# Tejasvanvekar/Sparse-optimal-control-of-Viscous-Chan-hilliard-via-Gradient-descent--1D-2D

Measured on AMD Instinct MI355X. Metric: PGD iterations/sec (fwd Newton + adjoint + prox), 2D 512^2 grid, higher is better.
Workload: dtype f64; 1 GPU; 2D 512x512, 1000 time steps, batch 8 trajectories per GPU (8 total), seeds 42+i, targets build_targets 1/1, u0 = 0; grid=512, batch_per_gpu=8, contexts_per_gpu=2, parallelism=batch-shard x1, collective=cabi-rccl

## Files before the change

sparse-optimal-control-of-viscous-chan-hilliard-via-gradient-descent--1d-2d_amd/csrc/vch_engine2d.hip:

```cpp
#include "vch_common.h"
#include "vch_kernels2d.h"
#include "vch_gemm.h"
#include "vch_fft.h"
#include <algorithm>
#include <atomic>
#include <chrono>
#include <cmath>

thread_local char g_vch_err[512] = "";

extern "C" const char *vch_last_error(void) { return g_vch_err; }
extern "C" int vch_abi_version(void) { return 3; }
extern "C" int vch_device_count(void) {
    int n = 0;
    if (hipGetDeviceCount(&n) != hipSuccess) return -1;
    return n;
}

constexpr int J_RING = 64;

struct GuessPolicy {
    static constexpr int PROBE_EVERY = 8;
    int order, probe, since, next_dir;
    bool climbing;
    double r_base;
    void reset() { order = 1; probe = 0; since = 0; next_dir = 1; climbing = true; r_base = 1e300; }
    int choose(int avail, int cap) const { return std::max(0, std::min(std::min(order + probe, cap), avail)); }
    void report(double r, int used, int cap) {
        if (used < 1) return;
        if (climbing) {
            if (r > 0.7) {
                order = std::max(1, used - 1);
                r_base = 1e300;
                if (used > 1) climbing = false;
                return;
            }
            if (r_base < 1e299 && r > 0.5 * r_base) {
                order = std::max(1, used - 1);
                climbing = false;
                return;
            }
            r_base = r;
            order = used;
            if (used >= cap) climbing = false;
            else order = used + 1;
            return;
        }
        if (probe == 0) {
            r_base = r;
            if (r > 0.7 && order > 1) { --order; since = 0; return; }
            if (++since >= PROBE_EVERY) {
                since = 0;
                probe = next_dir;
                next_dir = -next_dir;
                if (order + probe < 1 || order + probe > cap) probe = 0;
            }
            return;
        }
        if (probe > 0 ? r < 0.5 * r_base : r <= r_base) order = used;
        probe = 0;
    }
};

struct vch2d_ctx {
    vch2d_params prm;
    int B, Mmax, device;
    Geom G;
    Phys P;
    double hx, hy;
    hipStream_t stream;
    hipEvent_t ev0, ev1;
    dim3 grid;
    int nblk;
    long slot_stride;
    double *phi_s, *mu_s, *Rphi_s, *rhs_s, *D_s;
    double *w, *wnew, *mu0, *cphi, *cmu, *x, *r, *dmu, *t1, *t2;
    double *cg_p[2], *cg_v, *cg_q;
    double *cg_z2;
    double *xf;
    int cg_last;
    bool cheb_on;
    int spec_form[4];
    bool debug_guess;
    bool adj_guess_off, adj_safe;
    long redo_iters;
    bool fused_on;
    int fused_mode;
    unsigned *fin_counter;
    int cheb_enq, spec_chn[4], cheb_margin, cheb_max;
    double pgd_adj_tol;
    double eta1_factor;
    double cg_scale_ratio;
    double *dprev[GUESS_RING], *x0g;
    bool guess_on;
    int guess_wr, guess_step;
    int guess_max;
    std::vector<GuessPolicy> pol1, pol2;
    std::vector<int> used1, used2, run2;
    GuessPolicy pol1_all, pol2_all;
    int run2_all;
    GuessArgs gtab1, gtab2;
    unsigned gmask1, gmask2;
    double *dprev2[GUESS_RING];
    bool guess2_on;
    double *gpart2;
    double *gpart3;
    double *gpart;
    int gnblk;
    double *tmp[6];
    double *wts_mass, *W_cost;
    double *part;
    double *part_mass;
    bool post_fold;
    bool post_pending;
    double *post_hist;
    TrajState *st, *st_host;
    TrajState *st_pub;
    unsigned long long *seq_pub, seq_next;
    bool look_spin;
    int *frozen_dev;
    double *hist_dev, *hist_host;
    double *Q1f, *Q2f, *Q1s, *Q2s, *mf, *ms;
    bool use_fft;
    int cols_c;
    FftAxis fax, sax;
    FftAxis fax_h, sax_h;
    double2 *tw_fh = nullptr, *tw_sh = nullptr;
    bool half_f = false, half_s = false;
    double2 *tw_f, *tw_s;
    double *phi_hist, *u_hist, *u_trial, *phi_trial, *phiQ, *r_hist, *p_hist, *q_hist;
    double *phiT, *phi0;
    double *cost_part, *cost_lvl;
    double *cost_lvl_host;
    double *alpha_dev;
    int M_res;
    int u_rows_res;
    bool pgd_ready;
    bool ramp;
    double rampT;
    std::vector<double> t_hist, dt, xg, yg, tfrac;
    double *tfrac_dev;
    std::vector<vch_opt_params> opts;
    double *opt_tab, *seam_tab;
    std::vector<double> tab_host;
    bool pgd_r_valid;
    unsigned long long *kkt_dev;
    std::vector<double> pgd_cost, pgd_alpha_prev, pgd_J;
    std::vector<int> pgd_plateau, pgd_done, pgd_k;
    std::vector<std::vector<double>> pgd_cost_hist;
    std::vector<double> pgd_denQ2, pgd_denT2, pgd_trk, pgd_trm;
    double pgd_rms;
    int pgd_err_n;
    double *J_dev;
    double *J_ring_dev, *J_ring_host;
    std::atomic<long> pgd_iter_total;
    long tot_launch, tot_sync;
    bool prof_on;
    std::vector<hipEvent_t> prof_ev;
    std::vector<int> prof_cls;
    size_t prof_used;
    int lin_maxit;
    double lin_tol;
    double lin_eta;
    bool spec;
    int spec_slots, spec_cgb[4];
    long n_launch, n_sync;
};

enum { PC_SCHUR_P = 0, PC_GEMM = 1, PC_RESIDUAL = 2, PC_ADJ_Q = 3, PC_CG_UPDATE = 4, PC_ADJ_RHS = 5, PC_COST = 6,
       PC_PROX = 7, PC_DCT_R0 = 8, PC_DCT_C = 9, PC_DCT_R3 = 10, PC_SCHUR_P1 = 11, PC_CG_ROWS = 12, PC_CG_ROWS1 = 13,
       PC_NOOP = 14, PC_GUESS = 15, PC_ADJ_GUESS = 16, PC_CHEB_ROWS = 17, PC_CHEB_ROWS0 = 18, PC_RESIDUAL0 = 19,
       PC_NCLS = 20 };

__global__ void k_noop() {}

static bool launch_begin(vch2d_ctx *c, int cls) {
    const bool rec = cls >= 0 && c->prof_on && c->prof_used + 2 <= c->prof_ev.size();
    if (rec) hipEventRecord(c->prof_ev[c->prof_used], c->stream);
    return rec;
}
static void launch_end(vch2d_ctx *c, int cls, bool rec) {
    c->n_launch++;
    if (rec) {
        hipEventRecord(c->prof_ev[c->prof_used + 1], c->stream);
        c->prof_cls.push_back(cls);
        c->prof_used += 2;
    }
}
#define LAUNCHC(cls, kern, grid, block, ...) LAUNCH_LDS(cls, kern, grid, block, 0, __VA_ARGS__)

static int dalloc(double **p, size_t n, hipStream_t s) {
    *p = nullptr;
    HIPCHK(hipMalloc((void **)p, n * sizeof(double)));
    HIPCHK(hipMemsetAsync(*p, 0, n * sizeof(double), s));
    return 0;
}

static int h2d(vch2d_ctx *c, double *dev, const double *host, long nplanes) {
    HIPCHK(hipMemcpy2DAsync(dev, (size_t)c->G.pitch * 8, host, (size_t)c->G.nf * 8, (size_t)c->G.nf * 8,
                            (size_t)c->G.ns * nplanes, hipMemcpyHostToDevice, c->stream));
    return 0;
}
static int d2h(vch2d_ctx *c, double *host, const double *dev, long nplanes) {
    HIPCHK(hipMemcpy2DAsync(host, (size_t)c->G.nf * 8, dev, (size_t)c->G.pitch * 8, (size_t)c->G.nf * 8,
                            (size_t)c->G.ns * nplanes, hipMemcpyDeviceToHost, c->stream));
    HIPCHK(hipStreamSynchronize(c->stream));
    return 0;
}
static int h2d_hist(vch2d_ctx *c, double *dev, const double *host, int rows) {
    const long hs = (long)(c->Mmax + 1) * c->G.plane;
    for (int b = 0; b < c->B; ++b)
        VCHCHK(h2d(c, dev + b * hs, host + (long)b * rows * c->G.nf * c->G.ns, rows));
    return 0;
}
static int d2h_hist(vch2d_ctx *c, double *host, const double *dev, int rows) {
    const long hs = (long)(c->Mmax + 1) * c->G.plane;
    for (int b = 0; b < c->B; ++b) {
        HIPCHK(hipMemcpy2DAsync(host + (long)b * rows * c->G.nf * c->G.ns, (size_t)c->G.nf * 8, dev + b * hs,
                                (size_t)c->G.pitch * 8, (size_t)c->G.nf * 8, (size_t)c->G.ns * rows,
                                hipMemcpyDeviceToHost, c->stream));
    }
    HIPCHK(hipStreamSynchronize(c->stream));
    return 0;
}
static int ensure_hist(vch2d_ctx *c, double **p) {
    if (*p) return 0;
    size_t n = (size_t)c->B * (c->Mmax + 1) * c->G.plane;
    hipError_t e = hipMalloc((void **)p, n * sizeof(double));
    if (e != hipSuccess) {
        *p = nullptr;
        return vch_fail(VCH_ERR_NOMEM, "hipMalloc of a %.2f GB history failed: %s", n * 8e-9, hipGetErrorString(e));
    }
    HIPCHK(hipMemsetAsync(*p, 0, n * sizeof(double), c->stream));
    return 0;
}
static inline long hist_stride(const vch2d_ctx *c) { return (long)(c->Mmax + 1) * c->G.plane; }

__global__ void k_publish_state(const unsigned *__restrict__ st, int nwords, unsigned *__restrict__ dst,
                                unsigned long long *seq, unsigned long long val) {
    for (int i = threadIdx.x; i < nwords; i += blockDim.x) dst[i] = st[i];
    __threadfence_system();
    __syncthreads();
    if (threadIdx.x == 0) __hip_atomic_store(seq, val, __ATOMIC_RELEASE, __HIP_MEMORY_SCOPE_SYSTEM);
}

static int sync_state(vch2d_ctx *c, bool full = true) {
    c->n_sync++;
    if (full || !c->look_spin) {
        HIPCHK(hipMemcpyAsync(c->st_host, c->st, sizeof(TrajState) * c->B, hipMemcpyDeviceToHost, c->stream));
        HIPCHK(hipStreamSynchronize(c->stream));
        return 0;
    }
    const unsigned long long want = ++c->seq_next;
    static_assert(sizeof(TrajState) % 4 == 0, "TrajState is copied in 32-bit words");
    hipLaunchKernelGGL(k_publish_state, dim3(1), dim3(256), 0, c->stream, (const unsigned *)c->st,
                       (int)(sizeof(TrajState) / 4 * c->B), (unsigned *)c->st_pub, c->seq_pub, want);
    HIPCHK(hipGetLastError());
    const auto t0 = std::chrono::steady_clock::now();
    for (unsigned spins = 1; __atomic_load_n(c->seq_pub, __ATOMIC_ACQUIRE) != want; ++spins) {
        __builtin_ia32_pause();
        if ((spins & 0x3fff) == 0) {
            const hipError_t q = hipStreamQuery(c->stream);
            if (q != hipSuccess && q != hipErrorNotReady) return vch_fail(VCH_ERR_HIP, "sync_state: %s", hipGetErrorString(q));
            if (q == hipSuccess && __atomic_load_n(c->seq_pub, __ATOMIC_ACQUIRE) != want)
                return vch_fail(VCH_ERR_STATE, "sync_state: stream drained but the state was not published");
            if (std::chrono::steady_clock::now() - t0 > std::chrono::seconds(120))
                return vch_fail(VCH_ERR_STATE, "sync_state: no state from the device after 120 s");
        }
    }
    memcpy(c->st_host, c->st_pub, sizeof(TrajState) * c->B);
    return 0;
}

static void dct_tables(int N, double h, std::vector<double> &Q1, std::vector<double> &Q2, std::vector<double> &m) {
    const int n = N + 1;
    Q1.assign((size_t)n * n, 0.0);
    Q2.assign((size_t)n * n, 0.0);
    m.assign(n, 0.0);
    const long double pi = 3.14159265358979323846264338327950288L;
    const long double sc = sqrtl(2.0L / N), is2 = 1.0L / sqrtl(2.0L);
    for (int j = 0; j < n; ++j) {
        long double sj = (j == 0 || j == N) ? is2 : 1.0L;
        for (int k = 0; k < n; ++k) {
            long double sk = (k == 0 || k == N) ? is2 : 1.0L;
            long long jk = ((long long)j * k) % (2LL * N);
            long double cv = cosl(pi * (long double)jk / (long double)N);
            Q1[(size_t)j * n + k] = (double)(sc * sj * sj * sk * cv);
            Q2[(size_t)j * n + k] = (double)(sc * sj * cv);
        }
        m[j] = (double)((2.0L - 2.0L * cosl(pi * j / (long double)N)) / ((long double)h * h));
    }
}

extern "C" vch2d_ctx *vch2d_create(const vch2d_params *p, int batch, int max_steps, int device) {
    if (!p || p->Nx < 2 || p->Ny < 2 || batch < 1 || max_steps < 1 || !(p->Lx > 0) || !(p->Ly > 0)) {
        vch_fail(VCH_ERR_ARG, "vch2d_create: bad arguments (Nx,Ny >= 2, batch >= 1, max_steps >= 1)");
        return nullptr;
    }
    if (hipSetDevice(device) != hipSuccess) {
        (void)hipGetLastError();
        vch_fail(VCH_ERR_HIP, "hipSetDevice(%d) failed", device);
        return nullptr;
    }
    vch2d_ctx *c = new vch2d_ctx();
    c->prm = *p;
    c->B = batch;
    c->Mmax = max_steps;
    c->device = device;
    c->hx = p->Lx / p->Nx;
    c->hy = p->Ly / p->Ny;
    Geom &G = c->G;
    G.nf = p->Nx + 1;
    G.ns = p->Ny + 1;
    G.pitch = (G.nf + 7) / 8 * 8;
    G.plane = (long)G.ns * G.pitch;
    G.tiles_f = (G.nf + TX - 1) / TX;
    G.tiles_s = (G.ns + TY - 1) / TY;
    G.ax = 1.0 / (c->hx * c->hx);
    G.ay = 1.0 / (c->hy * c->hy);
    c->P = Phys{p->tau, p->gamma, p->c1, p->c2, p->kappa, p->Lx * p->Ly};
    c->grid = dim3(G.tiles_f, G.tiles_s, batch);
    c->nblk = G.tiles_f * G.tiles_s;
    c->slot_stride = (long)batch * G.plane;
    c->M_res = -1;
    c->u_rows_res = 0;
    c->pgd_ready = false;
    c->prof_on = false;
    c->prof_used = 0;
    c->lin_maxit = 4000;
    c->lin_tol = 1e-15;
    if (const char *e = getenv("VCH_LIN_TOL")) c->lin_tol = atof(e);
    c->lin_eta = 0.05 * NEWTON_TOL;
    if (const char *e = getenv("VCH_LIN_ETA")) c->lin_eta = atof(e);
    c->cols_c = 1024;
    if (const char *e = getenv("VCH_COLS_C")) c->cols_c = atoi(e);
    c->spec = getenv("VCH_NO_SPEC") == nullptr;
    c->spec_slots = 2;
    for (int &n : c->spec_cgb) n = 12;
    c->cheb_on = !(getenv("VCH_CHEB") && atoi(getenv("VCH_CHEB")) == 0);
    for (int &f : c->spec_form) f = 3;
    c->debug_guess = getenv("VCH_DEBUG_GUESS") != nullptr;
    c->adj_guess_off = c->adj_safe = false;
    c->redo_iters = 0;
    c->cheb_enq = -1;
    c->fused_mode = getenv("VCH_FUSED") ? atoi(getenv("VCH_FUSED")) : 2;
    c->fused_on = c->fused_mode != 0;
    c->post_fold = true;
    if (const char *e = getenv("VCH_POST_FOLD")) c->post_fold = atoi(e) != 0;
    c->post_pending = false;
    c->post_hist = nullptr;
    c->fin_counter = nullptr;
    for (int &n : c->spec_chn) n = 2;
    c->cheb_margin = 1;
    if (const char *e = getenv("VCH_CHEB_MARGIN")) c->cheb_margin = std::max(0, atoi(e));
    c->cheb_max = 6;
    if (const char *e = getenv("VCH_CHEB_MAX")) c->cheb_max = std::max(0, atoi(e));
    c->pgd_adj_tol = 1e-12;
    if (const char *e = getenv("VCH_ADJ_TOL")) c->pgd_adj_tol = atof(e);
    c->eta1_factor = 1e-2;
    if (const char *e = getenv("VCH_ETA1")) c->eta1_factor = atof(e);
    c->cg_scale_ratio = 4.0;
    if (const char *e = getenv("VCH_CG_SCALE")) c->cg_scale_ratio = atof(e);
    c->n_launch = c->n_sync = 0;
    auto fail = [&](const char *what) {
        vch_fail(VCH_ERR_HIP, "vch2d_create: %s failed: %s", what, hipGetErrorString(hipGetLastError()));
        return (vch2d_ctx *)nullptr;
    };
    if (hipStreamCreate(&c->stream) != hipSuccess) return fail("hipStreamCreate");
    hipEventCreate(&c->ev0);
    hipEventCreate(&c->ev1);
    const size_t bp = (size_t)batch * G.plane;
    double **two[] = {&c->phi_s, &c->mu_s, &c->Rphi_s, &c->rhs_s, &c->D_s};
    for (auto q : two)
        if (dalloc(q, 2 * bp, c->stream)) return fail("hipMalloc");
    double **one[] = {&c->w, &c->wnew, &c->mu0, &c->cphi, &c->cmu, &c->x, &c->r, &c->dmu, &c->t1, &c->t2,
                      &c->cg_p[0], &c->cg_p[1], &c->cg_v, &c->cg_q, &c->cg_z2, &c->xf, &c->dprev[0], &c->dprev[1], &c->dprev[2], &c->dprev[3], &c->dprev[4], &c->dprev[5], &c->dprev[6], &c->dprev[7], &c->dprev2[0], &c->dprev2[1], &c->dprev2[2], &c->dprev2[3], &c->dprev2[4], &c->dprev2[5], &c->dprev2[6], &c->dprev2[7], &c->x0g, &c->tmp[0], &c->tmp[1], &c->tmp[2], &c->tmp[3], &c->tmp[4], &c->tmp[5], &c->phiT, &c->phi0};
    for (auto q : one)
        if (dalloc(q, bp, c->stream)) return fail("hipMalloc");
    if (dalloc(&c->wts_mass, G.plane, c->stream) || dalloc(&c->W_cost, G.plane, c->stream)) return fail("hipMalloc");
    if (dalloc(&c->part, (size_t)batch * c->nblk * NPART, c->stream)) return fail("hipMalloc");
    if (dalloc(&c->part_mass, (size_t)batch * c->nblk * NPART, c->stream)) return fail("hipMalloc");
    c->gnblk = ((G.nf + GN - 1) / GN) * ((G.ns + GM - 1) / GM);
    if (dalloc(&c->gpart, 2 * (size_t)batch * (c->gnblk + G.ns), c->stream)) return fail("hipMalloc");
    c->gpart2 = c->gpart + (size_t)batch * (c->gnblk + G.ns);
    if (dalloc(&c->gpart3, 4 * (size_t)batch * (c->gnblk + G.ns), c->stream)) return fail("hipMalloc");
    if (dalloc(&c->hist_dev, (size_t)batch * HIST_CAP, c->stream)) return fail("hipMalloc");
    if (dalloc(&c->alpha_dev, batch, c->stream) || dalloc(&c->J_dev, 5 * (size_t)batch, c->stream)) return fail("hipMalloc");
    if (dalloc(&c->opt_tab, (size_t)OPT_STRIDE * batch, c->stream) || dalloc(&c->seam_tab, (size_t)OPT_STRIDE * batch, c->stream))
        return fail("hipMalloc");
    if (hipMalloc((void **)&c->kkt_dev, sizeof(unsigned long long) * 3 * batch * (max_steps + 2)) != hipSuccess)
        return fail("hipMalloc");
    c->pgd_r_valid = false;
    if (dalloc(&c->J_ring_dev, (size_t)J_RING * 5 * batch, c->stream)) return fail("hipMalloc");
    if (hipHostMalloc((void **)&c->J_ring_host, sizeof(double) * J_RING * 5 * batch) != hipSuccess) return fail("hipHostMalloc");
    c->pgd_iter_total = 0;
    c->tot_launch = c->tot_sync = 0;
    if (hipMalloc((void **)&c->st, sizeof(TrajState) * batch) != hipSuccess) return fail("hipMalloc");
    hipMemsetAsync(c->st, 0, sizeof(TrajState) * batch, c->stream);
    if (hipMalloc((void **)&c->frozen_dev, sizeof(int) * batch) != hipSuccess) return fail("hipMalloc");
    if (hipMalloc((void **)&c->fin_counter, sizeof(unsigned) * batch) != hipSuccess) return fail("hipMalloc");
    hipMemsetAsync(c->fin_counter, 0, sizeof(unsigned) * batch, c->stream);
    if (hipHostMalloc((void **)&c->st_host, sizeof(TrajState) * batch) != hipSuccess) return fail("hipHostMalloc");
    c->st_pub = nullptr;
    c->seq_pub = nullptr;
    c->seq_next = 0;
    c->look_spin = !(getenv("VCH_LOOK_SPIN") && atoi(getenv("VCH_LOOK_SPIN")) == 0);
    if (c->look_spin) {
        if (hipHostMalloc((void **)&c->st_pub, sizeof(TrajState) * batch, hipHostMallocMapped | hipHostMallocCoherent) != hipSuccess ||
            hipHostMalloc((void **)&c->seq_pub, 64, hipHostMallocMapped | hipHostMallocCoherent) != hipSuccess) {
            (void)hipGetLastError();
            if (c->st_pub) hipHostFree(c->st_pub);
            c->st_pub = nullptr;
            c->seq_pub = nullptr;
            c->look_spin = false;
        } else {
            *c->seq_pub = 0;
        }
    }
    if (hipHostMalloc((void **)&c->hist_host, sizeof(double) * batch * HIST_CAP) != hipSuccess) return fail("hipHostMalloc");
    c->phi_hist = c->u_hist = c->u_trial = c->phi_trial = c->phiQ = c->r_hist = c->p_hist = c->q_hist = nullptr;
    c->cost_part = c->cost_lvl = nullptr;
    c->cost_lvl_host = nullptr;
    c->tfrac_dev = nullptr;
    {
        std::vector<double> wm((size_t)G.plane, 0.0);
        const int nx1 = p->Nx + 1, ny1 = p->Ny + 1;
        for (int i = 0; i < nx1; ++i)
            for (int j = 0; j < ny1; ++j) {
                long f = (long)i * ny1 + j;
                double wi = (i == 0 || i == nx1 - 1) ? 0.5 : 1.0, wj = (j == 0 || j == ny1 - 1) ? 0.5 : 1.0;
                wm[(f / G.nf) * G.pitch + (f % G.nf)] = c->hx * c->hy * (wi * wj);
            }
        if (hipMemcpy(c->wts_mass, wm.data(), wm.size() * 8, hipMemcpyHostToDevice) != hipSuccess) return fail("hipMemcpy");
    }
    {
        std::vector<double> Q1, Q2, m;
        auto up = [&](double **d, const std::vector<double> &v) {
            if (hipMalloc((void **)d, v.size() * 8) != hipSuccess) return false;
            return hipMemcpy(*d, v.data(), v.size() * 8, hipMemcpyHostToDevice) == hipSuccess;
        };
        dct_tables(p->Nx, c->hx, Q1, Q2, m);
        if (!up(&c->Q1f, Q1) || !up(&c->Q2f, Q2) || !up(&c->mf, m)) return fail("DCT table upload");
        dct_tables(p->Ny, c->hy, Q1, Q2, m);
        if (!up(&c->Q1s, Q1) || !up(&c->Q2s, Q2) || !up(&c->ms, m)) return fail("DCT table upload");
    }
    {
        auto pow2 = [](int n) { return n >= 16 && n <= 2048 && (n & (n - 1)) == 0; };
        c->use_fft = pow2(p->Nx) && pow2(p->Ny) && getenv("VCH_FORCE_GEMM_DCT") == nullptr;
        c->tw_f = c->tw_s = nullptr;
        if (c->use_fft) {
            auto mk = [&](int N, double2 **tw, FftAxis &ax) {
                const int L = 2 * N;
                std::vector<double2> t(L);
                const long double pi = 3.14159265358979323846264338327950288L;
                for (int m = 0; m < L; ++m) {
                    long double a = -2.0L * pi * m / L;
                    t[m] = make_double2((double)cosl(a), (double)sinl(a));
                }
                if (hipMalloc((void **)tw, sizeof(double2) * L) != hipSuccess) return false;
                if (hipMemcpy(*tw, t.data(), sizeof(double2) * L, hipMemcpyHostToDevice) != hipSuccess) return false;
                int lg = 0;
                while ((1 << lg) < L) ++lg;
                ax = FftAxis{N, L, lg, *tw};
                return true;
            };
            if (!mk(p->Nx, &c->tw_f, c->fax) || !mk(p->Ny, &c->tw_s, c->sax)) return fail("FFT twiddle upload");
            const bool want_half = getenv("VCH_DCT_HALF") != nullptr;
            if (want_half && p->Nx == HN) {
                if (!mk(HN / 2, &c->tw_fh, c->fax_h)) return fail("FFT twiddle upload");
                c->half_f = true;
            }
            if (want_half && p->Ny == HN) {
                if (!mk(HN / 2, &c->tw_sh, c->sax_h)) return fail("FFT twiddle upload");
                c->half_s = true;
            }
            if (c->half_f) {
                c->gnblk = (G.ns + 3) / 4;
            } else {
                const int Cc = c->fax.L <= 1024 ? 1024 : c->fax.L;
                const int rpw = 2 * (Cc >> c->fax.logL);
                c->gnblk = (G.ns + rpw - 1) / rpw;
            }
        }
    }
    c->guess_on = c->use_fft && !c->half_f && !c->half_s && !(getenv("VCH_GUESS") && atoi(getenv("VCH_GUESS")) == 0);
    memset(&c->gtab1, 0, sizeof(c->gtab1));
    memset(&c->gtab2, 0, sizeof(c->gtab2));
    c->gmask1 = c->gmask2 = 0;
    c->pol1.resize(batch);
    c->pol2.resize(batch);
    c->used1.assign(batch, 0);
    c->used2.assign(batch, 0);
    c->run2.assign(batch, 0);
    c->run2_all = 0;
    c->guess2_on = !(getenv("VCH_GUESS2") && atoi(getenv("VCH_GUESS2")) == 0);
    c->guess_wr = -1;
    c->guess_step = 0;
    c->guess_max = 6;
    if (const char *e = getenv("VCH_GUESS_MAX")) c->guess_max = std::max(1, std::min(GUESS_ORD, atoi(e)));
    if (hipStreamSynchronize(c->stream) != hipSuccess) return fail("hipStreamSynchronize");
    return c;
}

extern "C" void vch2d_destroy(vch2d_ctx *c) {
    if (!c) return;
    hipSetDevice(c->device);
    hipStreamSynchronize(c->stream);
    double *all[] = {c->phi_s, c->mu_s, c->Rphi_s, c->rhs_s, c->D_s, c->w, c->wnew, c->mu0, c->cphi, c->cmu, c->x,
                     c->r, c->dmu, c->t1, c->t2, c->cg_p[0], c->cg_p[1], c->cg_v, c->cg_q, c->cg_z2, c->xf, c->dprev[0], c->dprev[1], c->dprev[2], c->dprev[3], c->dprev[4], c->dprev[5], c->dprev[6], c->dprev[7], c->dprev2[0], c->dprev2[1], c->dprev2[2], c->dprev2[3], c->dprev2[4], c->dprev2[5], c->dprev2[6], c->dprev2[7], c->x0g, c->gpart, c->gpart3, c->tmp[0], c->tmp[1], c->tmp[2], c->tmp[3], c->tmp[4], c->tmp[5],
                     c->phiT, c->phi0, c->wts_mass, c->W_cost, c->part, c->part_mass, c->hist_dev, c->alpha_dev, c->opt_tab, c->seam_tab, c->J_dev, c->Q1f,
                     c->Q2f, c->Q1s, c->Q2s, c->mf, c->ms, c->phi_hist, c->u_hist, c->u_trial, c->phi_trial, c->phiQ,
                     c->r_hist, c->p_hist, c->q_hist, c->cost_part, c->cost_lvl, c->tfrac_dev};
    for (double *q : all)
        if (q) hipFree(q);
    hipFree(c->st);
    hipFree(c->frozen_dev);
    if (c->kkt_dev) hipFree(c->kkt_dev);
    if (c->fin_counter) hipFree(c->fin_counter);
    if (c->tw_fh) hipFree(c->tw_fh);
    if (c->tw_sh) hipFree(c->tw_sh);
    if (c->tw_f) hipFree(c->tw_f);
    if (c->tw_s) hipFree(c->tw_s);
    hipHostFree(c->st_host);
    if (c->st_pub) hipHostFree(c->st_pub);
    if (c->seq_pub) hipHostFree(c->seq_pub);
    hipHostFree(c->hist_host);
    hipHostFree(c->J_ring_host);
    hipFree(c->J_ring_dev);
    if (c->cost_lvl_host) hipHostFree(c->cost_lvl_host);
    for (hipEvent_t e : c->prof_ev) hipEventDestroy(e);
    hipEventDestroy(c->ev0);
    hipEventDestroy(c->ev1);
    hipStreamDestroy(c->stream);
    delete c;
}

extern "C" int vch2d_batch(const vch2d_ctx *c) { return c ? c->B : VCH_ERR_ARG; }

template <class F>
static int with_plan(const FftAxis &ax, F &&f) {
    using std::integral_constant;
    if (ax.logL == 10) return f(integral_constant<int, 1024>(), integral_constant<int, 10>());
    if (ax.logL == 9) return f(integral_constant<int, 1024>(), integral_constant<int, 9>());
    if (ax.logL < 10) return f(integral_constant<int, 1024>(), integral_constant<int, 0>());
    if (ax.logL == 11) return f(integral_constant<int, 2048>(), integral_constant<int, 11>());
    return f(integral_constant<int, 4096>(), integral_constant<int, 0>());
}

template <int EPI>
static int dct_rows(vch2d_ctx *c, const double *in, long in_slot_stride, double *out, const SpecArgs &sp, int gate) {
    return with_plan(c->fax, [&](auto C, auto LG) {
        const int rpw = 2 * (C >> c->fax.logL);
        LAUNCHC(EPI >= 3 ? PC_DCT_R3 : PC_DCT_R0, (k_dct_rows<EPI, C, LG>), dim3((c->G.ns + rpw - 1) / rpw, 1, c->B),
                dim3(FftThreads<C, LG>::T), c->G, c->fax, in, in_slot_stride, out, 1.0, sp, c->st, gate);
        return 0;
    });
}

template <int C, int LOGL>
static int dct_cols_plan(vch2d_ctx *c, const SpecArgs &sp, double scale, int gate) {
    const int cpw = 2 * (C >> c->sax.logL);
    LAUNCHC(PC_DCT_C, (k_dct_cols<C, LOGL>), dim3((c->G.nf + cpw - 1) / cpw, 1, c->B), dim3(FftThreads<C, LOGL>::T), c->G,
            c->sax, (const double *)c->t1, c->t2, scale, sp, c->st, gate);
    return 0;
}
static int dct_cols(vch2d_ctx *c, const SpecArgs &sp, double scale, int gate) {
    const int wide = c->sax.logL == 10 ? c->cols_c : 0;
    if (wide == 4096) return dct_cols_plan<4096, 10>(c, sp, scale, gate);
    if (wide == 2048) return dct_cols_plan<2048, 10>(c, sp, scale, gate);
    return with_plan(c->sax, [&](auto C, auto LG) { return dct_cols_plan<C, LG>(c, sp, scale, gate); });
}

static int cg_rows(vch2d_ctx *c, const CgSweepArgs &a, bool first) {
    return with_plan(c->fax, [&](auto C, auto LG) {
        const int rpw = 2 * (C >> c->fax.logL);
        auto k_rows = first ? k_cg_rows_fwd<1, C, LG> : k_cg_rows_fwd<0, C, LG>;
        LAUNCHC(first ? PC_CG_ROWS1 : PC_CG_ROWS, k_rows, dim3((c->G.ns + rpw - 1) / rpw, 1, c->B), dim3(FftThreads<C, LG>::T),
                c->G, c->fax, a, c->t1, c->st);
        return 0;
    });
}

static int cheb_rows(vch2d_ctx *c, const ChebSweepArgs &a, bool first) {
    return with_plan(c->fax, [&](auto C, auto LG) {
        const int rpw = 2 * (C >> c->fax.logL);
        auto k_rows = first ? k_cheb_rows<C, LG, 1> : k_cheb_rows<C, LG, 0>;
        LAUNCHC(first ? PC_CHEB_ROWS0 : PC_CHEB_ROWS, k_rows, dim3((c->G.ns + rpw - 1) / rpw, 1, c->B), dim3(FftThreads<C, LG>::T),
                c->G, c->fax, a, (const double *)c->t2, c->t1, (const TrajState *)c->st);
        return 0;
    });
}

static int adj_rows(vch2d_ctx *c, const AdjSweepArgs &a, bool first) {
    return with_plan(c->fax, [&](auto C, auto LG) {
        const int rpw = 2 * (C >> c->fax.logL);
        auto k_rows = first ? k_adj_rows_fwd<1, C, LG> : k_adj_rows_fwd<0, C, LG>;
        LAUNCHC(PC_ADJ_Q, k_rows, dim3((c->G.ns + rpw - 1) / rpw, 1, c->B), dim3(FftThreads<C, LG>::T), c->G, c->fax, a, c->t1,
                c->st);
        return 0;
    });
}

static int precond(vch2d_ctx *c, const double *in, long in_slot_stride, double *out, int last, const double *other,
                   double c0, double c1a, double c1b, double c2, int gate) {
    const Geom &G = c->G;
    const int ns = G.ns, nf = G.nf;
    dim3 g((nf + GN - 1) / GN, (ns + GM - 1) / GM, c->B);
    SpecArgs sp{c0, c1a, c1b, c2, c->ms, c->mf, other, c->D_s, c->slot_stride, c->gpart, c->gpart2, 0};
    if (c->use_fft) {
        const double scale = 1.0 / (4.0 * (double)c->fax.N * (double)c->sax.N);
#define DCTH_ROWS(EPI_, in_, iss_, out_)                                                                        \
    LAUNCHC(((EPI_) == 3 ? PC_DCT_R3 : PC_DCT_R0), (k_dcth_rows<EPI_>), dim3((ns + 3) / 4, 1, c->B), dim3(HT), G, c->fax, c->fax_h, in_, iss_, out_, 1.0, sp, \
            c->st, gate)
        if (c->half_f) DCTH_ROWS(0, in, in_slot_stride, c->t1);
        else VCHCHK(dct_rows<0>(c, in, in_slot_stride, c->t1, sp, gate));
        if (c->half_s)
            LAUNCHC(PC_DCT_C, k_dcth_cols, dim3((nf + 3) / 4, 1, c->B), dim3(HT), G, c->sax, c->sax_h, (const double *)c->t1, c->t2,
                    scale, sp, c->st, gate);
        else VCHCHK(dct_cols(c, sp, scale, gate));
        if (c->half_f) {
            if (last == 3) DCTH_ROWS(3, (const double *)c->t2, 0L, out);
            else DCTH_ROWS(0, (const double *)c->t2, 0L, out);
        } else if (last == 3) VCHCHK(dct_rows<3>(c, c->t2, 0L, out, sp, gate));
        else if (last == 4) VCHCHK(dct_rows<4>(c, c->t2, 0L, out, sp, gate));
        else VCHCHK(dct_rows<0>(c, c->t2, 0L, out, sp, gate));
        return 0;
    }
    LAUNCHC(PC_GEMM, (k_gemm<false, 0>), g, dim3(256), ns, nf, nf, in, (long)G.pitch, G.plane, in_slot_stride, c->Q1f, (long)nf, 0L,
           c->t1, (long)G.pitch, G.plane, sp, c->st, gate);
    LAUNCHC(PC_GEMM, (k_gemm<true, 1>), g, dim3(256), ns, nf, ns, c->Q1s, (long)ns, 0L, 0L, c->t1, (long)G.pitch, G.plane, c->t2,
           (long)G.pitch, G.plane, sp, c->st, gate);
    LAUNCHC(PC_GEMM, (k_gemm<true, 0>), g, dim3(256), ns, nf, ns, c->Q2s, (long)ns, 0L, 0L, c->t2, (long)G.pitch, G.plane, c->t1,
           (long)G.pitch, G.plane, sp, c->st, gate);
    if (last == 3)
        LAUNCHC(PC_GEMM, (k_gemm<false, 3>), g, dim3(256), ns, nf, nf, c->t1, (long)G.pitch, G.plane, 0L, c->Q2f, (long)nf, 0L, out,
               (long)G.pitch, G.plane, sp, c->st, gate);
    else
        LAUNCHC(PC_GEMM, (k_gemm<false, 0>), g, dim3(256), ns, nf, nf, c->t1, (long)G.pitch, G.plane, 0L, c->Q2f, (long)nf, 0L, out,
               (long)G.pitch, G.plane, sp, c->st, gate);
    return 0;
}

static int sweep_tail(vch2d_ctx *c, const double *p, double *q, double c0, double c2, int gate) {
    const SpecArgs sp{c0, 0.0, 1.0, c2, c->ms, c->mf, p, c->D_s, c->slot_stride, c->gpart, c->gpart2, 1};
    VCHCHK(dct_cols(c, sp, 1.0 / (4.0 * (double)c->fax.N * (double)c->sax.N), gate));
    return dct_rows<4>(c, c->t2, 0L, q, sp, gate);
}

static int cg_budget(const vch2d_ctx *c, bool only_newton_active) {
    int n = 0;
    for (int b = 0; b < c->B; ++b) {
        const TrajState &S = c->st_host[b];
        if (!S.lin_active) continue;
        if (only_newton_active && !S.newton_active) continue;
        n = std::max(n, S.lin_budget);
    }
    return std::min(n, c->lin_maxit);
}
static bool any_lin_active(const vch2d_ctx *c) {
    for (int b = 0; b < c->B; ++b)
        if (c->st_host[b].lin_active) return true;
    return false;
}
constexpr int CG_CHUNK = 24;

static int schur_solve(vch2d_ctx *c, double dt, int budget, bool look) {
    c->cg_last = -1;
    if (budget <= 0) return 0;
    const double c0 = 1.0 / dt, c2 = 0.5 * c->P.kappa;
    double *zb[2] = {c->r, c->cg_z2};
    VCHCHK(precond(c, c->rhs_s, c->slot_stride, zb[0], 3, nullptr, c0, 0.0, 1.0, c2, 5));
    const bool spectral = c->use_fft && !c->half_f && !c->half_s;
    if (!spectral) LAUNCH(k_fin_cg_init, dim3(c->B), dim3(64), c->st, c->gpart, c->gnblk);
    int done = 0;
    while (done < budget) {
        const int chunk = look ? std::min(budget - done, CG_CHUNK) : budget - done;
        for (int j = 0; j < chunk; ++j, ++done) {
            double *pn = c->cg_p[done & 1], *po = c->cg_p[(done + 1) & 1];
            if (spectral) {
                CgSweepArgs a{done == 0 ? zb[0] : zb[(done + 1) & 1], c->cg_q, po, c->x, zb[done & 1], pn, c->D_s, c->slot_stride,
                              c->gpart, c->gpart2, c->gpart3, done, c->lin_maxit, c->B, c->x0g};
                VCHCHK(cg_rows(c, a, done == 0));
                VCHCHK(sweep_tail(c, pn, c->cg_q, c0, c2, 2 + (done & 1)));
                continue;
            }
            if (done == 0) {
                LAUNCHC(PC_SCHUR_P1, (k_schur_p<1>), c->grid, dim3(NTH), c->G, c->P, c->st, c->slot_stride, zb[0], c->cg_q, po, c->D_s, dt,
                        c->x, zb[1], pn, c->cg_v, c->part, (const double *)c->gpart, (const double *)c->gpart2, c->gnblk, 0,
                        c->lin_tol, c->lin_maxit);
            } else {
                LAUNCHC(PC_SCHUR_P, (k_schur_p<0>), c->grid, dim3(NTH), c->G, c->P, c->st, c->slot_stride, zb[(done + 1) & 1], c->cg_q, po,
                        c->D_s, dt, c->x, zb[done & 1], pn, c->cg_v, c->part, (const double *)c->gpart, (const double *)c->gpart2,
                        c->gnblk, done, c->lin_tol, c->lin_maxit);
            }
            VCHCHK(precond(c, c->cg_v, 0, c->cg_q, 3, pn, c0, 0.0, 1.0, c2, 2 + (done & 1)));
        }
        if (done < budget) {
            LAUNCH(k_cg_publish, dim3((c->B + 63) / 64), dim3(64), c->st, (done - 1) & 1, c->B);
            VCHCHK(sync_state(c, false));
            if (!any_lin_active(c)) break;
        }
    }
    c->cg_last = done - 1;
    if (!spectral) {
        LAUNCH(k_fin_cg_step, dim3(c->B), dim3(192), c->st, c->gpart, c->gpart2, c->gnblk, c->part, c->nblk, (done - 1) & 1,
               done - 1 >= 1 ? 1 : 0, (done - 1) & 1, (done - 1) & 1, c->lin_tol, c->lin_maxit);
        LAUNCHC(PC_CG_UPDATE, k_cg_finish, c->grid, dim3(NTH), c->G, c->st, c->cg_p[0], c->cg_p[1], c->x);
    }
    return 0;
}

static int cheb_solve(vch2d_ctx *c, double dt, int n_enq) {
    c->cheb_enq = n_enq;
    const double c0 = 1.0 / dt, c2 = 0.5 * c->P.kappa;
    const double scale = 1.0 / (4.0 * (double)c->fax.N * (double)c->sax.N);
    {
        const SpecArgs sp{c0, 0.0, 1.0, c2, c->ms, c->mf, nullptr, c->D_s, c->slot_stride, c->gpart, c->gpart2, 0};
        VCHCHK(dct_rows<0>(c, c->rhs_s, c->slot_stride, c->t1, sp, 8));
        VCHCHK(dct_cols(c, sp, 1.0, 8));
    }
    for (int j = 0; j <= n_enq; ++j) {
        ChebSweepArgs a{c->r, c->r, c->cg_p[j & 1], c->cg_p[(j + 1) & 1], c->cg_p[(j + 1) & 1], c->xf, c->x0g, c->D_s, c->slot_stride,
                        j == 0 ? c->gpart : c->gpart2, j, scale, c->phi_s, c->gpart3,
                        c->guess_wr >= 0 ? c->dprev[c->guess_wr] : (double *)nullptr,
                        (c->guess_wr >= 0 && c->guess2_on) ? c->dprev2[c->guess_wr] : (double *)nullptr};
        VCHCHK(cheb_rows(c, a, j == 0));
        if (j < n_enq) {
            const SpecArgs sp{c0, 0.0, 1.0, c2, c->ms, c->mf, nullptr, c->D_s, c->slot_stride, c->gpart, c->gpart2, 1};
            VCHCHK(dct_cols(c, sp, 1.0, 16 + j + 1));
        }
    }
    return 0;
}

static int dmu_ceiling(vch2d_ctx *c, int strict) {
    const bool spectral = c->use_fft && !c->half_f && !c->half_s;
    const ChebFin nocheb{-1, 0, nullptr, nullptr, nullptr};
    if (spectral && c->cheb_enq >= 0) {
        LAUNCH(k_fin_ceiling, dim3(c->B), dim3(64), c->st, c->part, c->nblk, strict, -1,
               ChebFin{c->cheb_enq, c->gnblk, c->gpart, c->gpart2, c->gpart3});
    }
    if (spectral && c->cg_last >= 0) {
        const int last = c->cg_last, rd = last & 1;
        FinSolveArgs f{c->gpart, c->gpart2, c->gpart3 + (size_t)rd * c->B * c->gnblk, c->gnblk, last >= 1 ? 1 : 0, rd, c->lin_maxit,
                       c->cg_p[last & 1], -1};
        LAUNCH(k_dmu_ceiling_fin, c->grid, dim3(NTH), c->G, c->P, c->st, c->slot_stride, (const double *)c->x, f, (const double *)c->phi_s,
               (const double *)c->D_s, (const double *)c->Rphi_s, c->dmu, c->xf, c->part,
               c->guess_wr >= 0 ? c->dprev[c->guess_wr] : (double *)nullptr,
               (c->guess_wr >= 0 && c->guess2_on) ? c->dprev2[c->guess_wr] : (double *)nullptr);
        LAUNCH(k_fin_ceiling, dim3(c->B), dim3(64), c->st, c->part, c->nblk, strict, rd ^ 1, nocheb);
    } else if (!spectral) {
        LAUNCH(k_dmu_ceiling, c->grid, dim3(NTH), c->G, c->P, c->st, c->slot_stride, c->x, c->phi_s, c->D_s, c->Rphi_s, c->dmu, c->xf,
               c->part);
        LAUNCH(k_fin_ceiling, dim3(c->B), dim3(64), c->st, c->part, c->nblk, strict, -1, nocheb);
    }
    c->cg_last = -1;
    c->cheb_enq = -1;
    return 0;
}

static int residual_trial(vch2d_ctx *c, double dt, bool inline_dmu, bool fused, bool fin_inside, bool guess, double eta,
                          const SolveOpts &so, const EvalFin &efin) {
    if (inline_dmu && fused) {
        GuessArgs gt = c->gtab2;
        if (!guess) memset(gt.c, 0, sizeof(gt.c));
        auto k_trial = fin_inside ? k_eval<2, true> : k_eval<2, false>;
        LAUNCHC(PC_RESIDUAL, k_trial, c->grid, dim3(NTH), c->G, c->P, c->st, c->slot_stride, c->phi_s, c->mu_s, c->Rphi_s, c->rhs_s,
                c->D_s, (const double *)c->xf, c->cphi, c->cmu, dt, c->part, (const double *)nullptr, (const double *)nullptr,
                (const double *)nullptr, 0L, (double *)nullptr, gt, c->x0g, efin, PostArgs{nullptr, nullptr, 0});
        if (!fin_inside)
            LAUNCH((k_fin_residual<1>), dim3(c->B), dim3(64), c->st, c->part, c->nblk, c->hist_dev, c->P.kappa, dt, c->lin_tol, eta,
                   guess ? (int)c->gmask2 : 0, so);
        return 0;
    }
    if (inline_dmu)
        LAUNCHC(PC_RESIDUAL, k_residual2, c->grid, dim3(NTH), c->G, c->P, c->st, c->slot_stride, c->phi_s, c->mu_s, c->Rphi_s,
                c->rhs_s, c->D_s, (const double *)c->xf, c->cphi, c->cmu, dt, c->part);
    else
        LAUNCHC(PC_RESIDUAL, (k_residual<1>), c->grid, dim3(NTH), c->G, c->P, c->st, c->slot_stride, c->phi_s, c->mu_s, c->Rphi_s,
                c->rhs_s, c->D_s, c->mu0, c->xf, c->dmu, c->cphi, c->cmu, dt, c->part);
    if (guess)
        LAUNCHC(PC_GUESS, k_guess, c->grid, dim3(NTH), c->G, c->P, c->st, c->slot_stride, c->gtab2, (const double *)c->D_s, dt,
                c->rhs_s, c->x0g, c->part, 1);
    LAUNCH((k_fin_residual<1>), dim3(c->B), dim3(64), c->st, c->part, c->nblk, c->hist_dev, c->P.kappa, dt, c->lin_tol, eta,
           guess ? (int)c->gmask2 : 0, so);
    return 0;
}

static int newton_level(vch2d_ctx *c, double dt, const double *un, const double *unp1, long u_stride,
                        const double *wnew_in, bool in_march) {
    const double eta_ = in_march ? c->lin_eta : 0.0;
    const bool spectral = c->use_fft && !c->half_f && !c->half_s;
    const bool fused = in_march && c->fused_on && spectral && !wnew_in;
    const bool inline_dmu = in_march && spectral;
    const int cheb_max_ = (in_march && spectral && c->cheb_on && eta_ > 0.0) ? c->cheb_max : -1;
    const bool fin_inside = c->fused_mode == 1;
    const SolveOpts so_{cheb_max_, spectral ? c->cg_scale_ratio : 0.0, in_march ? c->eta1_factor : 0.0};
    const EvalFin efin_{fin_inside ? c->fin_counter : (unsigned *)nullptr, c->hist_dev, c->P.kappa, c->lin_tol, eta_, so_};
    const bool guess = in_march && c->guess_on && c->gmask1 != 0;
    const bool guess2 = in_march && c->guess_on && c->guess2_on && c->gmask2 != 0;
    if (fused) {
        GuessArgs g1_ = c->gtab1;
        if (!guess) memset(g1_.c, 0, sizeof(g1_.c));
        const PostArgs post_{c->post_pending ? (const double *)c->part_mass : (const double *)nullptr, c->post_hist, hist_stride(c)};
        c->post_pending = false;
        auto k_start = fin_inside ? k_eval<0, true> : k_eval<0, false>;
        LAUNCHC(PC_RESIDUAL0, k_start, c->grid, dim3(NTH), c->G, c->P, c->st, c->slot_stride, c->phi_s, c->mu_s, c->Rphi_s, c->rhs_s,
                c->D_s, (const double *)nullptr, c->cphi, c->cmu, dt, c->part, (const double *)c->w, un, unp1, u_stride, c->wnew, g1_,
                c->x0g, efin_, post_);
        if (!fin_inside)
            LAUNCH((k_fin_residual<2>), dim3(c->B), dim3(64), c->st, c->part, c->nblk, c->hist_dev, c->P.kappa, dt, c->lin_tol, eta_,
                   guess ? (int)c->gmask1 : 0, so_);
    } else {
        LAUNCH(k_prepare, c->grid, dim3(NTH), c->G, c->P, c->st, c->slot_stride, c->phi_s, c->mu_s, c->w, un, unp1, u_stride,
               wnew_in, dt, c->wnew, c->mu0, c->cphi, c->cmu);
        LAUNCHC(PC_RESIDUAL0, (k_residual<0>), c->grid, dim3(NTH), c->G, c->P, c->st, c->slot_stride, c->phi_s, c->mu_s, c->Rphi_s, c->rhs_s,
               c->D_s, c->mu0, c->x, c->dmu, c->cphi, c->cmu, dt, c->part);
        if (guess)
            LAUNCHC(PC_GUESS, k_guess, c->grid, dim3(NTH), c->G, c->P, c->st, c->slot_stride, c->gtab1, (const double *)c->D_s, dt, c->rhs_s,
                   c->x0g, c->part, 0);
        LAUNCH((k_fin_residual<0>), dim3(c->B), dim3(64), c->st, c->part, c->nblk, c->hist_dev, c->P.kappa, dt, c->lin_tol, eta_,
               guess ? (int)c->gmask1 : 0, so_);
    }
    if (c->spec) {
        for (int s = 0; s < c->spec_slots; ++s) {
            if (cheb_max_ >= 0 && (c->spec_form[s] & 1)) VCHCHK(cheb_solve(c, dt, c->spec_chn[s]));
            if (cheb_max_ < 0 || (c->spec_form[s] & 2)) VCHCHK(schur_solve(c, dt, c->spec_cgb[s], false));
            VCHCHK(dmu_ceiling(c, 1));
            VCHCHK(residual_trial(c, dt, inline_dmu, fused, fin_inside, guess2, eta_, so_, efin_));
        }
    }
    VCHCHK(sync_state(c, false));
    auto any_active = [&]() {
        for (int b = 0; b < c->B; ++b)
            if (c->st_host[b].newton_active) return true;
        return false;
    };
    auto any_trial = [&]() {
        for (int b = 0; b < c->B; ++b)
            if (c->st_host[b].newton_active && c->st_host[b].need_trial) return true;
        return false;
    };
    if (c->debug_guess) {
        const TrajState &S = c->st_host[0];
        fprintf(stderr, "guess order %d / %d (run %d) | traj 0: ratio %.3e / %.3e solves %d sweeps %d %d %d normR %.3e active %d "
                "tol %.3e %.3e %.3e kT %.6f %.6f %.6f form %d %d %d | norms %d total sweeps %ld newton %ld trials %d lastform %d lastn %d R %.3e %.3e %.3e r0 %.3e\n",
                c->used1[0], c->used2[0], c->run2[0], S.guess_ratio, S.guess_ratio2, S.step_solves, S.step_lin[0],
                S.step_lin[1], S.step_lin[2], S.normR, S.newton_active, S.step_tol[0], S.step_tol[1], S.step_tol[2],
                S.step_kT[0], S.step_kT[1], S.step_kT[2], S.step_form[0], S.step_form[1], S.step_form[2], S.iters, S.lin_total,
                S.newton_total, S.ntrials, S.use_cheb, S.cheb_n, S.step_R[0], S.step_R[1], S.step_R[2], S.lin_r0);
    }
    int guard = 0;
    while (any_active()) {
        if (++guard > NEWTON_MAXIT + 2) return vch_fail(VCH_ERR_STATE, "newton_level: state machine did not terminate");
        int need = -1, budget = 0;
        for (int b = 0; b < c->B; ++b) {
            const TrajState &S = c->st_host[b];
            if (!S.newton_active || !S.lin_active) continue;
            if (S.use_cheb) need = std::max(need, S.cheb_n);
            else budget = std::max(budget, S.lin_budget);
        }
        if (need >= 0) VCHCHK(cheb_solve(c, dt, need));
        if (budget > 0) VCHCHK(schur_solve(c, dt, std::min(budget, c->lin_maxit), true));
        VCHCHK(dmu_ceiling(c, 0));
        int tguard = 0;
        do {
            VCHCHK(residual_trial(c, dt, inline_dmu, fused, fin_inside, guess2, eta_, so_, efin_));
            VCHCHK(sync_state(c, false));
            if (++tguard > ARMIJO_TRIALS + 2) return vch_fail(VCH_ERR_STATE, "newton_level: Armijo loop did not terminate");
        } while (any_trial());
    }
    {
        int solves = 1, sweeps[4] = {1, 1, 1, 1}, chn[4] = {0, 0, 0, 0}, form[4] = {0, 0, 0, 0}, longest = 1, bound = 1, chmax = 0,
            form_any = 0;
        for (int b = 0; b < c->B; ++b) {
            const TrajState &S = c->st_host[b];
            if (S.frozen) continue;
            solves = std::max(solves, S.step_solves);
            bound = std::max(bound, S.lin_budget);
            for (int s = 0; s < 4 && s < S.step_solves; ++s) {
                if (S.step_form[s]) {
                    chn[s] = std::max(chn[s], S.step_chn[s]);
                    chmax = std::max(chmax, S.step_chn[s]);
                    form[s] |= 1;
                } else {
                    sweeps[s] = std::max(sweeps[s], S.step_lin[s]);
                    longest = std::max(longest, S.step_lin[s]);
                    form[s] |= 2;
                }
                form_any |= form[s];
            }
        }
        if (!form_any) form_any = cheb_max_ >= 0 ? 1 : 2;
        c->spec_slots = std::min(solves, 4);
        for (int s = 0; s < 4; ++s) {
            const bool seen = s < solves && form[s] != 0;
            c->spec_form[s] = seen ? form[s] : form_any;
            const int want = ((seen && (form[s] & 2)) ? sweeps[s] : longest) + 1;
            c->spec_cgb[s] = std::max(2, std::min(std::min(want, bound), 64));
            c->spec_chn[s] = ((seen && (form[s] & 1)) ? chn[s] : chmax) + c->cheb_margin;
        }
    }
    return 0;
}

static void fill_stats(vch2d_ctx *c, vch_stats *s, float ms) {
    if (!s) return;
    memset(s, 0, sizeof(*s));
    for (int b = 0; b < c->B; ++b) {
        const TrajState &S = c->st_host[b];
        s->newton_iters += S.newton_total;
        s->linear_solves += S.nsolves;
        s->linear_iters += S.lin_total;
        s->armijo_trials += S.ntrials;
        s->max_lin_relres = std::max(s->max_lin_relres, S.lin_maxrel);
        s->max_lin_absres = std::max(s->max_lin_absres, S.lin_maxabs);
        s->unconverged_solves += S.lin_unconv;
    }
    s->linear_iters += c->redo_iters;
    s->host_syncs += 0;
    s->host_syncs = c->n_sync;
    s->launches = c->n_launch;
    s->seconds = ms * 1e-3;
}

static int reset_counters(vch2d_ctx *c) {
    HIPCHK(hipMemsetAsync(c->st, 0, sizeof(TrajState) * c->B, c->stream));
    c->tot_launch += c->n_launch;
    c->tot_sync += c->n_sync;
    c->n_launch = c->n_sync = 0;
    return 0;
}

static int freeze(vch2d_ctx *c, const std::vector<int> &flags) {
    HIPCHK(hipMemcpyAsync(c->frozen_dev, flags.data(), sizeof(int) * c->B, hipMemcpyHostToDevice, c->stream));
    LAUNCH(k_set_frozen, dim3((c->B + 63) / 64), dim3(64), c->st, (const int *)c->frozen_dev, c->B);
    return 0;
}

extern "C" int vch2d_apply_laplacian(vch2d_ctx *c, const double *v, double *out) {
    CTXCHK(c);
    ARGCHK(v && out, "NULL array");
    VCHCHK(h2d(c, c->tmp[0], v, c->B));
    LAUNCH(k_lap, c->grid, dim3(NTH), c->G, c->tmp[0], c->tmp[1]);
    return d2h(c, out, c->tmp[1], c->B);
}

extern "C" int vch2d_initialize_mu(vch2d_ctx *c, const double *phi, const double *w, double *mu_out) {
    CTXCHK(c);
    ARGCHK(phi && w && mu_out, "NULL array");
    VCHCHK(h2d(c, c->tmp[0], phi, c->B));
    VCHCHK(h2d(c, c->tmp[1], w, c->B));
    LAUNCH(k_init_mu, c->grid, dim3(NTH), c->G, c->P, c->tmp[0], c->tmp[1], c->tmp[2]);
    return d2h(c, mu_out, c->tmp[2], c->B);
}

extern "C" int vch2d_solve_w(vch2d_ctx *c, const double *w_old, double dt, const double *u_n, const double *u_np1,
                             double *w_out) {
    CTXCHK(c);
    ARGCHK(w_old && w_out && dt > 0, "NULL array or dt <= 0");
    VCHCHK(h2d(c, c->tmp[0], w_old, c->B));
    if (u_n) VCHCHK(h2d(c, c->tmp[1], u_n, c->B));
    if (u_np1) VCHCHK(h2d(c, c->tmp[2], u_np1, c->B));
    LAUNCH(k_solve_w, c->grid, dim3(NTH), c->G, c->tmp[0], u_n ? c->tmp[1] : nullptr, u_np1 ? c->tmp[2] : nullptr,
           c->P.gamma / dt, c->tmp[3]);
    return d2h(c, w_out, c->tmp[3], c->B);
}

static int read_norms(vch2d_ctx *c, int slot, double *norm_out) {
    std::vector<double> hp((size_t)c->B * c->nblk * NPART);
    HIPCHK(hipMemcpyAsync(hp.data(), c->part, hp.size() * 8, hipMemcpyDeviceToHost, c->stream));
    HIPCHK(hipStreamSynchronize(c->stream));
    for (int b = 0; b < c->B; ++b) {
        double s = 0.0;
        for (int t = 0; t < c->nblk; ++t) s += hp[((size_t)b * c->nblk + t) * NPART + slot];
        norm_out[b] = std::sqrt(s);
    }
    return 0;
}

extern "C" int vch2d_residuals(vch2d_ctx *c, const double *pn, const double *po, const double *mn, const double *mo,
                               const double *wn, const double *wo, double dt, double *Rp, double *Rm, double *norm_out) {
    CTXCHK(c);
    ARGCHK(pn && po && mn && mo && wn && wo && Rp && Rm && dt > 0, "NULL array or dt <= 0");
    const double *src[6] = {pn, po, mn, mo, wn, wo};
    for (int k = 0; k < 6; ++k) VCHCHK(h2d(c, c->tmp[k], src[k], c->B));
    LAUNCH(k_residual_plain, c->grid, dim3(NTH), c->G, c->P, c->tmp[0], c->tmp[1], c->tmp[2], c->tmp[3], c->tmp[4],
           c->tmp[5], dt, c->t1, c->t2, c->part);
    VCHCHK(d2h(c, Rp, c->t1, c->B));
    VCHCHK(d2h(c, Rm, c->t2, c->B));
    if (norm_out) VCHCHK(read_norms(c, 0, norm_out));
    return 0;
}

extern "C" int vch2d_jacobian_apply(vch2d_ctx *c, const double *phi_new, double dt, const double *dphi, const double *dmu,
                                    double *out_phi, double *out_mu) {
    CTXCHK(c);
    ARGCHK(phi_new && dphi && dmu && out_phi && out_mu && dt > 0, "NULL array or dt <= 0");
    VCHCHK(h2d(c, c->tmp[0], phi_new, c->B));
    VCHCHK(h2d(c, c->tmp[1], dphi, c->B));
    VCHCHK(h2d(c, c->tmp[2], dmu, c->B));
    LAUNCH(k_jac_apply, c->grid, dim3(NTH), c->G, c->P, c->tmp[0], c->tmp[1], c->tmp[2], dt, c->tmp[3], c->tmp[4]);
    VCHCHK(d2h(c, out_phi, c->tmp[3], c->B));
    return d2h(c, out_mu, c->tmp[4], c->B);
}

extern "C" int vch2d_schur_apply(vch2d_ctx *c, const double *phi_new, double dt, const double *x, double *out) {
    CTXCHK(c);
    ARGCHK(phi_new && x && out && dt > 0, "NULL array or dt <= 0");
    VCHCHK(reset_counters(c));
    VCHCHK(h2d(c, c->tmp[0], phi_new, c->B));
    VCHCHK(h2d(c, c->tmp[1], x, c->B));
    LAUNCH(k_solve_setup, c->grid, dim3(NTH), c->G, c->P, c->tmp[1], c->tmp[1], c->tmp[0], dt, c->Rphi_s, c->rhs_s, c->D_s,
           c->part);
    LAUNCH(k_schur, c->grid, dim3(NTH), c->G, c->P, (const TrajState *)nullptr, c->slot_stride, c->tmp[1], c->D_s, dt, c->tmp[2]);
    return d2h(c, out, c->tmp[2], c->B);
}

extern "C" int vch2d_spectral_solve(vch2d_ctx *c, double c0, double c1, double c2, const double *v, double *out) {
    CTXCHK(c);
    ARGCHK(v && out, "NULL array");
    VCHCHK(h2d(c, c->tmp[0], v, c->B));
    VCHCHK(precond(c, c->tmp[0], 0, c->tmp[1], 0, nullptr, c0, c1, 0.0, c2, 0));
    return d2h(c, out, c->tmp[1], c->B);
// ... 11 lines not shown
    HIPCHK(hipMemcpyAsync(c->phi_s, c->tmp[0], sizeof(double) * c->B * c->G.plane, hipMemcpyDeviceToDevice, c->stream));
    LAUNCH(k_solve_setup, c->grid, dim3(NTH), c->G, c->P, c->tmp[1], c->tmp[2], c->tmp[0], dt, c->Rphi_s, c->rhs_s, c->D_s,
           c->part);
    LAUNCH(k_fin_lin_begin, dim3(c->B), dim3(64), c->st, c->part, c->nblk, 2, c->P.tau, c->P.kappa, dt, c->lin_tol);
    VCHCHK(sync_state(c));
    VCHCHK(schur_solve(c, dt, cg_budget(c, false), true));
    HIPCHK(hipStreamSynchronize(c->stream));
    {
        std::vector<TrajState> tmp(c->B);
        HIPCHK(hipMemcpy(tmp.data(), c->st, sizeof(TrajState) * c->B, hipMemcpyDeviceToHost));
        for (auto &S : tmp) { S.newton_active = 1; S.need_trial = 0; }
        HIPCHK(hipMemcpy(c->st, tmp.data(), sizeof(TrajState) * c->B, hipMemcpyHostToDevice));
    }
    VCHCHK(dmu_ceiling(c, 0));
    HIPCHK(hipEventRecord(c->ev1, c->stream));
    VCHCHK(d2h(c, dphi, c->xf, c->B));
    VCHCHK(d2h(c, dmu, c->dmu, c->B));
    VCHCHK(sync_state(c));
    float ms = 0;
    hipEventElapsedTime(&ms, c->ev0, c->ev1);
    fill_stats(c, stats, ms);
    return 0;
}

static int adjoint_solve_cg(vch2d_ctx *c, double dt, int budget, bool look) {
    const bool spectral = c->use_fft && !c->half_f && !c->half_s;
    LAUNCH((k_adj_op<1>), c->grid, dim3(NTH), c->G, c->P, c->st, c->x, c->cmu, c->cphi, dt, c->r, c->part);
    if (spectral) {
        if (budget <= 0) return 0;
        const double cadj = 0.5 * dt;
        double *rb[2] = {c->r, c->cg_z2}, *y = c->cg_v;
        int done = 0;
        while (done < budget) {
            const int chunk = look ? std::min(budget - done, CG_CHUNK) : budget - done;
            for (int j = 0; j < chunk; ++j, ++done) {
                double *pn = c->cg_p[done & 1], *po = c->cg_p[(done + 1) & 1];
                AdjSweepArgs a{done == 0 ? rb[0] : rb[(done + 1) & 1], c->cg_q, po, y, rb[done & 1], pn, c->cmu,
                               c->gpart, c->gpart2, c->gpart3, done, c->lin_maxit, c->B, c->part, c->nblk, c->lin_tol};
                VCHCHK(adj_rows(c, a, done == 0));
                const SpecArgs sp{1.0, c->P.tau, cadj, cadj, c->ms, c->mf, pn, c->cmu, 0L, c->gpart, c->gpart2, 1, cadj};
                const int gate = 2 + (done & 1);
                VCHCHK(dct_cols(c, sp, 1.0 / (4.0 * (double)c->fax.N * (double)c->sax.N), gate));
                VCHCHK(dct_rows<5>(c, c->t2, 0L, c->cg_q, sp, gate));
            }
            if (done < budget) {
                LAUNCH(k_cg_publish, dim3((c->B + 63) / 64), dim3(64), c->st, (done - 1) & 1, c->B);
                VCHCHK(sync_state(c, false));
                if (!any_lin_active(c)) break;
            }
        }
        LAUNCH(k_fin_adj_step, dim3(c->B), dim3(192), c->st, (const double *)c->gpart, (const double *)c->gpart2,
               (const double *)(c->gpart3 + (size_t)((done - 1) & 1) * c->B * c->gnblk * 2), c->gnblk, done - 1 >= 1 ? 1 : 0,
               (done - 1) & 1, (done - 1) & 1, c->lin_maxit);
        LAUNCHC(PC_CG_UPDATE, k_cg_finish, c->grid, dim3(NTH), c->G, c->st, c->cg_p[0], c->cg_p[1], y);
        VCHCHK(precond(c, y, 0, c->x, 4, c->x, 1.0, c->P.tau, cadj, cadj, 4));
        return 0;
    }
    double *ph = c->cg_p[0], *pv = c->cg_p[1], *q = c->cg_q;
    LAUNCH(k_fin_cg_beta, dim3(c->B), dim3(64), c->st, c->part, c->nblk, 1, c->lin_tol, c->lin_maxit, 1);
    int done = 0;
    while (done < budget) {
        const int chunk = std::min(budget - done, CG_CHUNK);
        for (int j = 0; j < chunk; ++j, ++done) {
            if (done == 0) LAUNCH((k_cg_dir<1>), c->grid, dim3(NTH), c->G, c->st, c->r, ph);
            else LAUNCH((k_cg_dir<0>), c->grid, dim3(NTH), c->G, c->st, c->r, ph);
            VCHCHK(precond(c, ph, 0, pv, 0, nullptr, 1.0, c->P.tau, 0.5 * dt, 0.5 * dt, 1));
            LAUNCHC(PC_ADJ_Q, k_adj_q, c->grid, dim3(NTH), c->G, c->P, c->st, pv, c->cmu, ph, dt, q, c->part);
            LAUNCH(k_fin_cg_alpha, dim3(c->B), dim3(64), c->st, c->part, c->nblk, NPART, 0);
            LAUNCHC(PC_CG_UPDATE, k_cg_update_adj, c->grid, dim3(NTH), c->G, c->st, pv, q, c->cmu, c->x, c->r, c->part);
            LAUNCH(k_fin_cg_beta, dim3(c->B), dim3(64), c->st, c->part, c->nblk, 1, c->lin_tol, c->lin_maxit, 0);
        }
        if (done < budget && look) {
            VCHCHK(sync_state(c, false));
            if (!any_lin_active(c)) break;
        }
    }
    return 0;
}

extern "C" int vch2d_adjoint_apply(vch2d_ctx *c, int which, const double *phi, double dt, const double *v, double *out) {
    CTXCHK(c);
    ARGCHK(phi && v && out && (which == 0 || which == 1), "NULL array or which not in {0,1}");
    VCHCHK(h2d(c, c->tmp[0], phi, c->B));
    VCHCHK(h2d(c, c->tmp[1], v, c->B));
    LAUNCH(k_adj_setup, c->grid, dim3(NTH), c->G, c->P, c->tmp[0], (const double *)nullptr, c->cmu, c->part);
    if (which == 0)
        LAUNCH((k_adj_op<0>), c->grid, dim3(NTH), c->G, c->P, c->st, c->tmp[1], c->cmu, c->cphi, dt, c->tmp[2], c->part);
    else
        LAUNCH((k_adj_op<2>), c->grid, dim3(NTH), c->G, c->P, c->st, c->tmp[1], c->cmu, c->cphi, dt, c->tmp[2], c->part);
    return d2h(c, out, c->tmp[2], c->B);
}

extern "C" int vch2d_adjoint_solve(vch2d_ctx *c, const double *phi_n, double dt, const double *rhs, double *p_out,
                                   vch_stats *stats) {
    CTXCHK(c);
    ARGCHK(rhs && p_out && dt >= 0 && (phi_n || dt == 0), "NULL array or dt < 0");
    VCHCHK(reset_counters(c));
    HIPCHK(hipEventRecord(c->ev0, c->stream));
    if (phi_n) VCHCHK(h2d(c, c->tmp[0], phi_n, c->B));
    VCHCHK(h2d(c, c->cphi, rhs, c->B));
    LAUNCH(k_adj_setup, c->grid, dim3(NTH), c->G, c->P, (dt > 0 ? c->tmp[0] : (const double *)nullptr), c->cphi, c->cmu,
           c->part);
    LAUNCH(k_fin_lin_begin, dim3(c->B), dim3(64), c->st, c->part, c->nblk, 0, c->P.tau, c->P.kappa, dt, c->lin_tol);
    LAUNCH(k_fill, c->grid, dim3(NTH), c->G, c->x, 0.0);
    VCHCHK(sync_state(c));
    VCHCHK(adjoint_solve_cg(c, dt, cg_budget(c, false), true));
    HIPCHK(hipEventRecord(c->ev1, c->stream));
    VCHCHK(d2h(c, p_out, c->x, c->B));
    VCHCHK(sync_state(c));
    float ms = 0;
    hipEventElapsedTime(&ms, c->ev0, c->ev1);
    fill_stats(c, stats, ms);
    return 0;
}

extern "C" int vch2d_newton_raphson(vch2d_ctx *c, const double *phi_old, const double *mu_old, const double *w_old,
                                    const double *w_new, double dt, double *phi_new, double *mu_new, double *hist,
                                    int hist_cap, int32_t *n_hist, vch_stats *stats) {
    CTXCHK(c);
    ARGCHK(phi_old && mu_old && w_old && w_new && phi_new && mu_new && dt > 0, "NULL array or dt <= 0");
    VCHCHK(reset_counters(c));
    VCHCHK(h2d(c, c->phi_s, phi_old, c->B));
    VCHCHK(h2d(c, c->mu_s, mu_old, c->B));
    VCHCHK(h2d(c, c->w, w_old, c->B));
    VCHCHK(h2d(c, c->tmp[0], w_new, c->B));
    HIPCHK(hipEventRecord(c->ev0, c->stream));
    VCHCHK(newton_level(c, dt, nullptr, nullptr, 0, c->tmp[0], false));
    HIPCHK(hipEventRecord(c->ev1, c->stream));
    HIPCHK(hipStreamSynchronize(c->stream));
    for (int b = 0; b < c->B; ++b) {
        const int slot = c->st_host[b].slot;
        VCHCHK(d2h(c, phi_new + (long)b * c->G.nf * c->G.ns, c->phi_s + slot * c->slot_stride + b * c->G.plane, 1));
        VCHCHK(d2h(c, mu_new + (long)b * c->G.nf * c->G.ns, c->mu_s + slot * c->slot_stride + b * c->G.plane, 1));
    }
    if (hist || n_hist) {
        HIPCHK(hipMemcpy(c->hist_host, c->hist_dev, sizeof(double) * c->B * HIST_CAP, hipMemcpyDeviceToHost));
        for (int b = 0; b < c->B; ++b) {
            int n = std::min(c->st_host[b].iters, HIST_CAP);
            if (n_hist) n_hist[b] = n;
            if (hist)
                for (int k = 0; k < std::min(n, hist_cap); ++k) hist[(long)b * hist_cap + k] = c->hist_host[(long)b * HIST_CAP + k];
        }
    }
    float ms = 0;
    hipEventElapsedTime(&ms, c->ev0, c->ev1);
    fill_stats(c, stats, ms);
    return 0;
}

static int forward_core(vch2d_ctx *c, const double *u_dev, int u_rows, const double *dt, int M, double *hist_out) {
    const long hs = hist_stride(c);
    HIPCHK(hipMemsetAsync(c->w, 0, sizeof(double) * c->B * c->G.plane, c->stream));
    LAUNCH(k_init_mu, c->grid, dim3(NTH), c->G, c->P, c->phi_s, c->w, c->mu_s);
    LAUNCH(k_mass, c->grid, dim3(NTH), c->G, c->st, c->slot_stride, c->phi_s, c->wts_mass, 0, c->part);
    LAUNCH(k_fin_mass, dim3(c->B), dim3(64), c->st, c->part, c->nblk, 1);
    c->post_pending = false;
    const bool fold_post = c->post_fold && c->fused_on && c->use_fft && !c->half_f && !c->half_s;
    if (hist_out) LAUNCH(k_copy_plane, c->grid, dim3(NTH), c->G, c->phi_s, c->G.plane, hist_out, hs);
    const bool per_traj = c->B <= GUESS_BMAX;
    for (auto &q : c->pol1) q.reset();
    for (auto &q : c->pol2) q.reset();
    std::fill(c->run2.begin(), c->run2.end(), 0);
    c->pol1_all.reset();
    c->pol2_all.reset();
    c->run2_all = 0;
    for (int &f : c->spec_form) f = 3;
    for (int step = 0; step < M; ++step) {
        const double *un = nullptr, *unp1 = nullptr;
        if (u_dev && step < u_rows - 1) {
            un = u_dev + (long)step * c->G.plane;
            unp1 = u_dev + (long)(step + 1) * c->G.plane;
        }
        memset(c->gtab1.c, 0, sizeof(c->gtab1.c));
        memset(c->gtab2.c, 0, sizeof(c->gtab2.c));
        c->gtab1.per_traj = c->gtab2.per_traj = per_traj ? 1 : 0;
        c->gmask1 = c->gmask2 = 0;
        c->guess_wr = -1;
        c->guess_step = step;
        if (c->guess_on) {
            c->guess_wr = step & (GUESS_RING - 1);
            for (int j = 0; j < GUESS_ORD; ++j) {
                c->gtab1.d[j] = c->dprev[(step - 1 - j) & (GUESS_RING - 1)];
                c->gtab2.d[j] = c->dprev2[(step - 1 - j) & (GUESS_RING - 1)];
            }
            auto weights = [&](int m, double *cf) -> int {
                for (; m >= 1; --m) {
                    double mid[GUESS_ORD + 1];
                    mid[0] = 0.5 * dt[step];
                    double t0 = 0.0, mag = 0.0;
                    for (int j = 1; j <= m; ++j) {
                        t0 -= dt[step - j];
                        mid[j] = t0 + 0.5 * dt[step - j];
                    }
                    for (int j = 0; j < GUESS_ORD; ++j) cf[j] = 0.0;
                    for (int j = 1; j <= m; ++j) {
                        double w = 1.0;
                        for (int k = 1; k <= m; ++k)
                            if (k != j) w *= (mid[0] - mid[k]) / (mid[j] - mid[k]);
                        cf[j - 1] = w * dt[step] / dt[step - j];
                        mag += std::fabs(cf[j - 1]);
                    }
                    if (std::isfinite(mag) && mag <= 64.0) return m;
                }
                for (int j = 0; j < GUESS_ORD; ++j) cf[j] = 0.0;
                return 0;
            };
            if (per_traj) {
                for (int b = 0; b < c->B; ++b) {
                    c->used1[b] = weights(c->pol1[b].choose(step, c->guess_max), c->gtab1.c[b]);
                    c->used2[b] = weights(c->guess2_on ? c->pol2[b].choose(std::min(step, c->run2[b]), c->guess_max) : 0, c->gtab2.c[b]);
                    if (c->used1[b] >= 1) c->gmask1 |= 1u << b;
                    if (c->used2[b] >= 1) c->gmask2 |= 1u << b;
                }
            } else {
                const int u1 = weights(c->pol1_all.choose(step, c->guess_max), c->gtab1.c[0]);
                const int u2 = weights(c->guess2_on ? c->pol2_all.choose(std::min(step, c->run2_all), c->guess_max) : 0, c->gtab2.c[0]);
                std::fill(c->used1.begin(), c->used1.end(), u1);
                std::fill(c->used2.begin(), c->used2.end(), u2);
                c->gmask1 = u1 >= 1 ? ~0u : 0u;
                c->gmask2 = u2 >= 1 ? ~0u : 0u;
            }
        }
        VCHCHK(newton_level(c, dt[step], un, unp1, hs, nullptr, true));
        LAUNCH(k_mass, c->grid, dim3(NTH), c->G, c->st, c->slot_stride, c->phi_s, c->wts_mass, 1, c->part_mass);
        double *const lvl = hist_out ? hist_out + (long)(step + 1) * c->G.plane : (double *)nullptr;
        if (fold_post && step + 1 < M) {
            c->post_pending = true;
            c->post_hist = lvl;
        } else {
            LAUNCH(k_post, c->grid, dim3(NTH), c->G, c->P, c->st, c->slot_stride, c->phi_s, lvl, hs, (const double *)c->part_mass);
        }
        std::swap(c->w, c->wnew);
        if (c->guess_on) {
            auto fin = [](double r) { return std::isfinite(r) ? r : 1e300; };
            if (per_traj) {
                for (int b = 0; b < c->B; ++b) {
                    const TrajState &S = c->st_host[b];
                    if (S.frozen) continue;
                    if (c->used1[b] >= 1 && S.step_solves >= 1) c->pol1[b].report(fin(S.guess_ratio), c->used1[b], c->guess_max);
                    if (!c->guess2_on) continue;
                    if (S.step_solves >= 2) {
                        c->run2[b]++;
                        if (c->used2[b] >= 1) c->pol2[b].report(fin(S.guess_ratio2), c->used2[b], c->guess_max);
                    } else {
                        c->run2[b] = 0;
                        c->pol2[b].reset();
                    }
                }
            } else {
                double worst = 0.0, worst2 = 0.0;
                bool any = false, anyb = false, all2 = true;
                for (int b = 0; b < c->B; ++b) {
                    const TrajState &S = c->st_host[b];
                    if (S.frozen) continue;
                    anyb = true;
                    if (S.step_solves >= 1) { any = true; worst = std::max(worst, fin(S.guess_ratio)); }
                    if (S.step_solves < 2) all2 = false;
                    worst2 = std::max(worst2, fin(S.guess_ratio2));
                }
                if (any && c->used1[0] >= 1) c->pol1_all.report(worst, c->used1[0], c->guess_max);
                if (c->guess2_on) {
                    if (anyb && all2) {
                        c->run2_all++;
                        if (c->used2[0] >= 1) c->pol2_all.report(worst2, c->used2[0], c->guess_max);
                    } else {
                        c->run2_all = 0;
                        c->pol2_all.reset();
                    }
                }
            }
        }
    }
    memset(c->gtab1.c, 0, sizeof(c->gtab1.c));
    memset(c->gtab2.c, 0, sizeof(c->gtab2.c));
    c->gmask1 = c->gmask2 = 0;
    c->guess_wr = -1;
    return 0;
}

extern "C" int vch2d_forward(vch2d_ctx *c, const double *phi0, const double *u, int u_rows, const double *dt, int M,
                             double *phi_hist_out, vch_stats *stats) {
    CTXCHK(c);
    ARGCHK(phi0 && dt && M >= 1 && M <= c->Mmax, "NULL array or M out of range (1..max_steps)");
    for (int k = 0; k < M; ++k) ARGCHK(dt[k] > 0, "dt must be positive");
    VCHCHK(ensure_hist(c, &c->phi_hist));
    const double *u_dev = nullptr;
    if (u == VCH_RESIDENT) {
        ARGCHK(c->u_hist && c->u_rows_res > 0, "no resident control");
        u_dev = c->u_hist;
        u_rows = c->u_rows_res;
    } else if (u) {
        ARGCHK(u_rows >= 1 && u_rows <= c->Mmax + 1, "control rows out of range (1..max_steps+1)");
        VCHCHK(ensure_hist(c, &c->u_hist));
        VCHCHK(h2d_hist(c, c->u_hist, u, u_rows));
        c->u_rows_res = u_rows;
        u_dev = c->u_hist;
    }
    VCHCHK(reset_counters(c));
    VCHCHK(h2d(c, c->phi_s, phi0, c->B));
    HIPCHK(hipEventRecord(c->ev0, c->stream));
    VCHCHK(forward_core(c, u_dev, u_rows, dt, M, c->phi_hist));
    HIPCHK(hipEventRecord(c->ev1, c->stream));
    VCHCHK(sync_state(c));
    c->M_res = M;
    if (phi_hist_out) VCHCHK(d2h_hist(c, phi_hist_out, c->phi_hist, M + 1));
    float ms = 0;
    hipEventElapsedTime(&ms, c->ev0, c->ev1);
    fill_stats(c, stats, ms);
    return 0;
}

static int write_opt_tab(vch2d_ctx *c, double *tab_dev, const vch_opt_params *o, int n_o) {
    c->tab_host.assign((size_t)OPT_STRIDE * c->B, 0.0);
    for (int b = 0; b < c->B; ++b) {
        const vch_opt_params &s = o[n_o == 1 ? 0 : b];
        double *t = c->tab_host.data() + (size_t)OPT_STRIDE * b;
        t[OPT_B1] = s.b1; t[OPT_B2] = s.b2; t[OPT_B3] = s.b3;
        t[OPT_KS] = s.kappa_sparsity; t[OPT_UMIN] = s.u_min; t[OPT_UMAX] = s.u_max;
    }
    HIPCHK(hipMemcpyAsync(tab_dev, c->tab_host.data(), sizeof(double) * OPT_STRIDE * c->B, hipMemcpyHostToDevice, c->stream));
    return 0;
}

constexpr int ADJ_LOOK = 8, ADJ_SETTLE = 16;
static int backward_pass(vch2d_ctx *c, const double *phi_hist_dev, int M, const double *t_hist, const double *opt_tab,
                         const double *phiQ_dev, const double *phiT_dev, double *r_out, double *p_out, double *q_out, bool safe) {
    const long hs = hist_stride(c);
    const Geom &G = c->G;
    double *rhs = c->cphi, *Dn = c->cmu, *rcur = c->wnew;
    double *qa = c->mu0, *qb = c->dmu;
    LAUNCH(k_scaled_diff, c->grid, dim3(NTH), G, phi_hist_dev + (long)M * G.plane, hs, phiT_dev, G.plane, opt_tab + OPT_B2, OPT_STRIDE, rhs,
           c->part);
    LAUNCH(k_adj_setup, c->grid, dim3(NTH), G, c->P, (const double *)nullptr, (const double *)rhs, Dn, c->part);
    LAUNCH(k_fin_lin_begin, dim3(c->B), dim3(64), c->st, c->part, c->nblk, 0, c->P.tau, c->P.kappa, 0.0, c->lin_tol);
    LAUNCH(k_fill, c->grid, dim3(NTH), G, c->x, 0.0);
    VCHCHK(adjoint_solve_cg(c, 0.0, 3, false));
    int sweeps = -1, steps_since_look = 0;
    bool first_solve = true;
    const bool guess = c->guess_on && !safe && !c->adj_guess_off;
    const bool per_traj = c->B <= GUESS_BMAX;
    std::vector<int> order(per_traj ? c->B : 1, 1);
    int kept = 0;
    LAUNCH(k_adj_finish, c->grid, dim3(NTH), G, c->x, (const double *)nullptr, qa, rcur, 0.0, 0.0,
           r_out ? r_out + (long)M * G.plane : (double *)nullptr, p_out ? p_out + (long)M * G.plane : (double *)nullptr,
           q_out ? q_out + (long)M * G.plane : (double *)nullptr, hs);
    for (int n = M - 1; n >= 0; --n) {
        const double dtn = t_hist[n + 1] - t_hist[n];
        double *rl = r_out ? r_out + (long)n * G.plane : nullptr;
        double *pl = p_out ? p_out + (long)n * G.plane : nullptr;
        double *ql = q_out ? q_out + (long)n * G.plane : nullptr;
        if (dtn <= 1e-14) {
            if (rl) LAUNCH(k_copy_plane, c->grid, dim3(NTH), G, r_out + (long)(n + 1) * G.plane, hs, rl, hs);
            if (pl) LAUNCH(k_copy_plane, c->grid, dim3(NTH), G, p_out + (long)(n + 1) * G.plane, hs, pl, hs);
            if (ql) LAUNCH(k_copy_plane, c->grid, dim3(NTH), G, q_out + (long)(n + 1) * G.plane, hs, ql, hs);
            kept = 0;
            continue;
        }
        LAUNCHC(PC_ADJ_RHS, k_adj_rhs, c->grid, dim3(NTH), G, c->P, c->x, qa, phi_hist_dev + (long)n * G.plane,
               phi_hist_dev + (long)(n + 1) * G.plane, phiQ_dev ? phiQ_dev + (long)n * G.plane : (const double *)nullptr,
               phiQ_dev ? phiQ_dev + (long)(n + 1) * G.plane : (const double *)nullptr, hs, dtn, opt_tab, rhs, Dn, c->part);
        LAUNCH(k_fin_lin_begin, dim3(c->B), dim3(64), c->st, c->part, c->nblk, 0, c->P.tau, c->P.kappa, dtn, c->lin_tol);
        if (safe || steps_since_look >= ((guess && M - 1 - n < ADJ_SETTLE) ? 1 : ADJ_LOOK) || sweeps < 0) {
            VCHCHK(sync_state(c, false));
            steps_since_look = 0;
            int longest = 0;
            for (int b = 0; b < c->B; ++b) longest = std::max(longest, c->st_host[b].step_lin_max);
            const int bound = cg_budget(c, false);
            int margin = 1;
            if (guess && !first_solve) {
                bool changed = false;
                auto adapt = [&](int &ord, double ratio) {
                    const int before = ord;
                    if (ratio < 0.25) ord = std::min(ord + 1, GUESS_ORD / 2);
                    else if (ratio > 0.7) ord = std::max(ord - 1, 1);
                    changed |= ord != before;
                };
                auto fin = [](double r) { return std::isfinite(r) ? r : 1e300; };
// ... 719 lines not shown
```

sparse-optimal-control-of-viscous-chan-hilliard-via-gradient-descent--1d-2d_amd/csrc/vch_fft.h:

```cpp
#pragma once
#include "vch_common.h"
#include "vch_kernels2d.h"
#include "vch_gemm.h"

struct FftAxis {
    int N, L, logL;
    const double2 *tw;
};


__device__ __forceinline__ double2 cmul(double2 a, double2 b) {
    return make_double2(a.x * b.x - a.y * b.y, a.x * b.y + a.y * b.x);
}

struct SpecArgs;
template <class SP>
__device__ __forceinline__ void spec_mult2(const SP &sp, double c1, double scale, double ma, double mb, double &fa, double &fb,
                                           int mode) {
    const double pa = sp.c0 + ma * (c1 + sp.c2 * ma), pb = sp.c0 + mb * (c1 + sp.c2 * mb);
    const double na = scale * (mode == 2 ? -(sp.c0 + sp.c2 * ma * ma) : (mode ? ma : 1.0));
    const double nb = scale * (mode == 2 ? -(sp.c0 + sp.c2 * mb * mb) : (mode ? mb : 1.0));
    const double d = pa * pb;
    double r = __builtin_amdgcn_rcp(d);
    r = fma(fma(-d, r, 1.0), r, r);
// ... 422 lines not shown
            if (active)
                for (int t = tid; t < (int)gridDim.x; t += 64) g += a.gpart[(long)b * gridDim.x + t];
            g = wave_sum(g);
            if (tid == 0) {
                TrajState &S = st[b];
                S.cg_pending = 0;
                if (!active) {
                    S.ci_active[0] = 0;
                } else {
                    S.cg_gamma = S.cg_gamma0 = g;
                    S.cg_beta = 0.0;
                    S.lin_it = 0;
                    S.lin_rel = 1.0;
                    S.ci_active[0] = 1;
                    S.ci_it[0] = 0;
                    S.ci_gamma[0] = g;
                }
            }
        }
        if (!active) return;
    } else {
        if (!st[b].ci_active[rd]) {
            if (blockIdx.x == 0 && tid == 0) {
                st[b].ci_active[wr] = 0;
                st[b].ci_it[wr] = st[b].ci_it[rd];
                st[b].ci_gamma[wr] = st[b].ci_gamma[rd];
            }
            return;
        }
        const double gamma0 = st[b].cg_gamma0, gamma_old = st[b].ci_gamma[rd], tol = st[b].lin_reltol;
        const int it_old = st[b].ci_it[rd], n = gridDim.x;
        cg_sums3<T>(a.gpart, a.gpart2, a.it >= 2 ? a.gpart3 + (long)rd * a.nbatch * n : nullptr, n, b, s3);
        const CgNext nx = cg_next(s3[0], s3[1], a.it >= 2 ? s3[2] : gamma_old, gamma0, it_old, tol, a.maxit);
        if (blockIdx.x == 0 && tid == 0) cg_record(st[b], nx, wr);
        alpha = nx.alpha;
        beta = nx.beta;
        if (!nx.active) {
            if (!nx.breakdown)
                for (int idx = tid; idx < 2 * nfft * n1; idx += T) {
                    const int rr = idx / n1, k = idx - rr * n1, row = row0 + rr;
                    if (row < G.ns) {
                        const long o = pb + (long)row * G.pitch + k;
                        a.x[o] += alpha * a.p_old[o];
                    }
                }
            return;
        }
    }
    const double dbar = st[b].dbar;
    const int scaled = st[b].scaled;
    const double *Dp = a.Dslot + st[b].slot * a.d_slot_stride + pb;
    const bool primed = FIRST && a.x0 && st[b].x_primed;
    double acc = 0.0;
    auto node = [&](int row, int m, bool owner) -> double {
        if (row >= G.ns) return 0.0;
        const long o = (long)row * G.pitch + m;
        const double dl = cg_weight(Dp[o], dbar, scaled);
        double pn;
        if (FIRST) {
            pn = a.z[pb + o];
            if (owner) {
                a.x[pb + o] = primed ? (scaled ? a.x0[pb + o] * (Dp[o] / dbar) : a.x0[pb + o]) : 0.0;
                a.p_new[pb + o] = pn;
            }
        } else {
            const double po = a.p_old[pb + o];
            const double zn = a.z[pb + o] - alpha * a.q[pb + o];
            pn = zn + beta * po;
            if (owner) {
                a.x[pb + o] += alpha * po;
                a.z_new[pb + o] = zn;
                a.p_new[pb + o] = pn;
                acc += wdev(row, m, G) * dl * (zn * zn);
            }
        }
        return dl * pn;
    };
    double *ob = out + pb;
    auto put = [&](int row, int k, double e) { ob[(long)row * G.pitch + k] = e; };
    constexpr bool DIRECT = LOGL >= 9 && LOGL <= 11;
    if (DIRECT) {
        struct Emit {
            enum { ACTIVE = 1, TO_LDS = 0 };
            decltype(put) &put_;
            int row0_, ns_;
            __device__ __forceinline__ void operator()(int idx, double2 v) const {
                constexpr int LL = 1 << (LOGL ? LOGL : 1);
                const int f = idx >> (LOGL ? LOGL : 1), k = idx & (LL - 1);
                if (k <= LL / 2) {
                    const int ra = row0_ + 2 * f;
                    if (ra < ns_) put_(ra, k, v.x);
                    if (ra + 1 < ns_) put_(ra + 1, k, v.y);
                }
            }
        };
        for (int idx = tid; idx < nfft * n1; idx += T) {
            const int f = nfft == 1 ? 0 : idx / n1, j = idx - f * n1;
            const int ra = row0 + 2 * f;
            const double2 v = make_double2(node(ra, j, true), node(ra + 1, j, true));
            buf[swz<LOGL>(f * L + j)] = v;
            if (j > 0 && j < N) buf[swz<LOGL>(f * L + L - j)] = v;
        }
        __syncthreads();
        fft_lds<C, LOGL>(buf, ax, Emit{put, row0, G.ns});
    } else {
        const float inv_n1 = 1.0f / (float)n1;
        for (int idx = tid; idx < nfft * n1; idx += T) {
            const int f = nfft == 1 ? 0 : (int)(((float)idx + 0.5f) * inv_n1), j = idx - f * n1;
            const int ra = row0 + 2 * f;
            const double2 v = make_double2(node(ra, j, true), node(ra + 1, j, true));
            buf[swz<LOGL>(f * L + j)] = v;
            if (j > 0 && j < N) buf[swz<LOGL>(f * L + L - j)] = v;
        }
        __syncthreads();
        fft_lds<C, LOGL>(buf, ax);
        for (int idx = tid; idx < 2 * nfft * n1; idx += T) {
            const int rr = nfft == 1 ? (idx >= n1 ? 1 : 0) : (int)(((float)idx + 0.5f) * inv_n1), k = idx - rr * n1;
            const int row = row0 + rr;
            if (row < G.ns) {
                const double2 c = buf[swz<LOGL>((rr >> 1) * L + k)];
                put(row, k, (rr & 1) ? c.y : c.x);
            }
        }
    }
    if (!FIRST) {
        acc = wave_sum(acc);
        __syncthreads();
        double *sred = reinterpret_cast<double *>(buf);
        if ((tid & 63) == 0) sred[tid >> 6] = acc;
        __syncthreads();
        if (tid == 0) {
            double tot = 0.0;
            for (int w = 0; w < T / 64; ++w) tot += sred[w];
            a.gpart3[((long)wr * a.nbatch + b) * gridDim.x + blockIdx.x] = tot;
        }
    }
}

struct ChebSweepArgs {
    const double *bt_in;
    double *bt_out;
    const double *y_cur, *y_prev;
    double *y_new;
    double *x_out;
    const double *x0;
    const double *Dslot;
    long d_slot_stride;
    double *gpart;
    int j;
    double scale;
    const double *phi_s;
    double *cmin;
    double *keep1, *keep2;
};

#ifndef CHEB_MINW
#define CHEB_MINW 1
#endif
template <int C, int LOGL, int FIRST>
__global__ __launch_bounds__((FftThreads<C, LOGL>::T), CHEB_MINW) void k_cheb_rows(Geom G, FftAxis ax, ChebSweepArgs a_, const double *__restrict__ in,
                                                                       double *__restrict__ out, const TrajState *__restrict__ st) {
    const int b = blockIdx.z;
    ChebSweepArgs a = a_;
    if (FIRST) a.j = 0;
    if (!st[b].lin_active || !st[b].use_cheb || a.j > st[b].cheb_n) return;
    const bool last = a.j == st[b].cheb_n;
    __shared__ double2 buf[C];
    constexpr int T = FftThreads<C, LOGL>::T;
    const int tid = threadIdx.x;
    const int logL = LOGL ? LOGL : ax.logL, L = 1 << logL, N = L >> 1, nfft = C >> logL;
    const int row0 = blockIdx.x * 2 * nfft, n1 = N + 1;
    const long pb = b * G.plane;
    const double theta = st[b].cheb_theta, delta = st[b].cheb_delta;
    double cj = 0.0, ej = 1.0 / theta;
    {
        double rho_prev = delta / theta;
        for (int i = 1; i <= a.j; ++i) {
            ej = 2.0 / (2.0 * theta - delta * rho_prev);
            const double rho = 0.5 * delta * ej;
            cj = rho * rho_prev;
            rho_prev = rho;
        }
    }
    const double dbar = st[b].dbar;
    const double *Dp = a.Dslot + st[b].slot * a.d_slot_stride + pb;
    const bool primed = a.x0 && st[b].x_primed;
    const bool need_norm = !(last && a.j == 0);
    double acc = 0.0, cmin = 1e300;
    const double *php = a.phi_s + st[b].slot * a.d_slot_stride + pb;
    double *const keepp = st[b].iters == 1 ? a.keep1 : (st[b].iters == 2 ? a.keep2 : nullptr);
    auto upd = [&](int row, int k, double g) -> double {
        const long o = (long)row * G.pitch + k;
        const double gg = a.scale * g;
        double z, yn, dl = 0.0;
        if (need_norm || !last) dl = Dp[o] - dbar;
        if (a.j == 0) {
            z = gg;
            yn = ej * z;
            if (!last) a.bt_out[pb + o] = gg;
        } else {
            const double yc = a.y_cur[pb + o], yp = a.j >= 2 ? a.y_prev[pb + o] : 0.0;
            z = a.bt_in[pb + o] - yc - gg;
            yn = yc + cj * (yc - yp) + ej * z;
        }
        if (need_norm) acc += wdev(row, k, G) * dl * (z * z);
        if (last) {
            const double d = primed ? a.x0[pb + o] + yn : yn, ph = php[o];
            a.x_out[pb + o] = d;
            if (keepp) keepp[pb + o] = d;
            if (d > 0.0) cmin = fmin(cmin, (1.0 - DELTA_SEP - ph) / d);
            else if (d < 0.0) cmin = fmin(cmin, (-1.0 + DELTA_SEP - ph) / d);
        } else {
            a.y_new[pb + o] = yn;
        }
        return dl * yn;
    };
    const double *ib = in + pb;
    double *ob = out + pb;
    auto put = [&](int row, int k, double e) { ob[(long)row * G.pitch + k] = e; };
    constexpr bool DIRECT = LOGL >= 9 && LOGL <= 11;
    if (DIRECT) {
        constexpr int LL = 1 << (LOGL ? LOGL : 1), LG = LOGL ? LOGL : 1;
        struct RowIngest {
            enum { ACTIVE = 1 };
            const double *ib_;
            long pitch_;
            int row0_, ns_;
            __device__ __forceinline__ double2 operator()(int idx) const {
                const int f = idx >> LG, i = idx & (LL - 1), m = i <= LL / 2 ? i : LL - i;
                const int ra = row0_ + 2 * f;
                const double *p = ib_ + (long)ra * pitch_ + m;
                return make_double2(ra < ns_ ? p[0] : 0.0, ra + 1 < ns_ ? p[pitch_] : 0.0);
            }
        };
        struct UpdEmit {
            enum { ACTIVE = 1, TO_LDS = 1 };
            decltype(upd) &upd_;
            double2 *buf_;
            int row0_, ns_;
            bool last_;
            __device__ __forceinline__ void operator()(int idx, double2 v) const {
                const int f = idx >> LG, k = idx & (LL - 1);
                if (k > LL / 2) return;
                const int ra = row0_ + 2 * f;
                double2 w = make_double2(0.0, 0.0);
                if (ra < ns_) w.x = upd_(ra, k, v.x);
                if (ra + 1 < ns_) w.y = upd_(ra + 1, k, v.y);
                if (!last_) {
                    buf_[swz<LOGL>(idx)] = w;
                    if (k > 0 && k < LL / 2) buf_[swz<LOGL>(f * LL + LL - k)] = w;
                }
            }
        };
        struct RowEmit {
            enum { ACTIVE = 1, TO_LDS = 0 };
            decltype(put) &put_;
            int row0_, ns_;
            __device__ __forceinline__ void operator()(int idx, double2 v) const {
                const int f = idx >> LG, k = idx & (LL - 1);
                if (k <= LL / 2) {
                    const int ra = row0_ + 2 * f;
                    if (ra < ns_) put_(ra, k, v.x);
                    if (ra + 1 < ns_) put_(ra + 1, k, v.y);
                }
            }
        };
        fft_lds<C, LOGL>(buf, ax, UpdEmit{upd, buf, row0, G.ns, last}, RowIngest{ib, (long)G.pitch, row0, G.ns});
        if (!last) fft_lds<C, LOGL>(buf, ax, RowEmit{put, row0, G.ns});
    } else {
        const float inv_n1 = 1.0f / (float)n1;
        for (int idx = tid; idx < nfft * n1; idx += T) {
            const int f = nfft == 1 ? 0 : (int)(((float)idx + 0.5f) * inv_n1), j = idx - f * n1;
            const int ra = row0 + 2 * f;
            const double2 v = make_double2(ra < G.ns ? ib[(long)ra * G.pitch + j] : 0.0,
                                           ra + 1 < G.ns ? ib[(long)(ra + 1) * G.pitch + j] : 0.0);
            buf[swz<LOGL>(f * L + j)] = v;
            if (j > 0 && j < N) buf[swz<LOGL>(f * L + L - j)] = v;
        }
        __syncthreads();
        fft_lds<C, LOGL>(buf, ax);
        for (int idx = tid; idx < nfft * n1; idx += T) {
            const int f = nfft == 1 ? 0 : (int)(((float)idx + 0.5f) * inv_n1), k = idx - f * n1;
            const int ra = row0 + 2 * f;
            const double2 v = buf[swz<LOGL>(f * L + k)];
            double2 w = make_double2(0.0, 0.0);
            if (ra < G.ns) w.x = upd(ra, k, v.x);
            if (ra + 1 < G.ns) w.y = upd(ra + 1, k, v.y);
            if (!last) {
                buf[swz<LOGL>(f * L + k)] = w;
                if (k > 0 && k < N) buf[swz<LOGL>(f * L + L - k)] = w;
            }
        }
        if (!last) {
            __syncthreads();
            fft_lds<C, LOGL>(buf, ax);
            for (int idx = tid; idx < 2 * nfft * n1; idx += T) {
                const int rr = nfft == 1 ? (idx >= n1 ? 1 : 0) : (int)(((float)idx + 0.5f) * inv_n1), k = idx - rr * n1;
                const int row = row0 + rr;
                if (row < G.ns) {
                    const double2 c = buf[swz<LOGL>((rr >> 1) * L + k)];
                    put(row, k, (rr & 1) ? c.y : c.x);
                }
            }
        }
    }
    if (need_norm || last) {
        acc = wave_sum(acc);
        cmin = wave_min(cmin);
        __syncthreads();
        double *sred = reinterpret_cast<double *>(buf);
        if ((tid & 63) == 0) {
            sred[tid >> 6] = acc;
            sred[T / 64 + (tid >> 6)] = cmin;
        }
        __syncthreads();
        if (tid == 0) {
            double tot = 0.0, mn = 1e300;
            for (int w = 0; w < T / 64; ++w) {
                tot += sred[w];
                mn = fmin(mn, sred[T / 64 + w]);
            }
            if (need_norm) a.gpart[(long)b * gridDim.x + blockIdx.x] = tot;
            if (last) a.cmin[(long)b * gridDim.x + blockIdx.x] = mn;
        }
    }
}

struct AdjSweepArgs {
    const double *r, *q, *p_old;
    double *y, *r_new, *p_new;
    const double *Dn;
    const double *gpart, *gpart2;
    double *gpart3;
    int it, maxit, nbatch;
    const double *part;
    int nblk;
    double tol;
};

struct CgNextAdj {
    int active, breakdown, it;
    double alpha, beta, gamma, rel;
};
__device__ __forceinline__ CgNextAdj cg_next_adj(double pq, double qq, double gamma, double r2, double rhs_norm, int it_old,
                                                 double tol, int maxit) {
    CgNextAdj n;
    n.it = it_old;
    const double rel_now = rhs_norm > 0.0 ? sqrt(fmax(r2, 0.0)) / rhs_norm : 0.0;
    if (!(pq > 0.0) || !(gamma > 0.0)) {
        n.active = 0; n.breakdown = 1; n.alpha = 0.0; n.beta = 0.0; n.gamma = fmax(gamma, 0.0); n.rel = rel_now;
        return n;
    }
    n.breakdown = 0;
    n.alpha = gamma / pq;
    double gn = n.alpha * n.alpha * qq - gamma;
    if (gn > 1e-13 * gamma) {
        n.beta = gn / gamma;
    } else {
        gn = 1e-13 * gamma;
        n.beta = 0.0;
    }
    n.gamma = gn;
    n.it = it_old + 1;
    n.rel = sqrt(gn / gamma) * rel_now;
    n.active = (n.rel > tol && n.it < maxit) ? 1 : 0;
    return n;
}
__device__ __forceinline__ void adj_record(TrajState &S, const CgNextAdj &n, int wr) {
    S.cg_alpha = n.alpha;
    S.cg_beta = n.beta;
    S.cg_gamma = n.gamma;
    S.lin_rel = n.rel;
    if (!n.breakdown) {
        S.lin_it = n.it;
        S.lin_total++;
    }
    if (!n.active && n.rel > S.lin_maxrel) S.lin_maxrel = n.rel;
    S.ci_active[wr] = n.active;
    S.ci_it[wr] = n.it;
    S.ci_gamma[wr] = n.gamma;
}

template <int T>
__device__ __forceinline__ void adj_sums4(const double *__restrict__ g1, const double *__restrict__ g2,
                                          const double *__restrict__ g3, int n, int b, double *s4) {
    const int wv = threadIdx.x >> 6, lane = threadIdx.x & 63;
    for (int k = wv; k < 4; k += T / 64) {
        double a = 0.0;
        if (k < 2) {
            const double *src = k == 0 ? g1 : g2;
            for (int t = lane; t < n; t += 64) a += src[(long)b * n + t];
        } else if (g3) {
            for (int t = lane; t < n; t += 64) a += g3[((long)b * n + t) * 2 + (k - 2)];
        }
        a = wave_sum(a);
        if (lane == 0) s4[k] = a;
    }
    __syncthreads();
}

__global__ void k_fin_adj_step(TrajState *st, const double *__restrict__ gpart, const double *__restrict__ gpart2,
                               const double *__restrict__ gpart3_rd, int gnblk, int direct, int pbuf, int rd, int maxit) {
    const int b = blockIdx.x;
    TrajState &S = st[b];
    __shared__ double s4[4];
    if (!S.lin_active) return;
    if (!S.ci_active[rd]) {
        if (threadIdx.x == 0) { S.lin_active = 0; S.cg_pending = 0; }
        return;
    }
    adj_sums4<192>(gpart, gpart2, direct ? gpart3_rd : nullptr, gnblk, b, s4);
    if (threadIdx.x != 0) return;
    const CgNextAdj n = cg_next_adj(s4[0], s4[1], direct ? s4[2] : S.ci_gamma[rd], direct ? s4[3] : S.aux[0], S.lin_r0,
                                    S.ci_it[rd], S.lin_reltol, maxit);
    adj_record(S, n, rd ^ 1);
    if (n.it > S.step_lin_max) S.step_lin_max = n.it;
    S.cg_pending = n.breakdown ? 0 : 1;
    S.cg_pbuf = pbuf;
    S.lin_active = n.active;
}

template <int FIRST, int C, int LOGL>
__global__ __launch_bounds__((FftThreads<C, LOGL>::T)) void k_adj_rows_fwd(Geom G, FftAxis ax, AdjSweepArgs a, double *__restrict__ out,
                                                                          TrajState *__restrict__ st) {
    const int b = blockIdx.z;
    __shared__ double2 buf[C];
    __shared__ double s4[4];
    constexpr int T = FftThreads<C, LOGL>::T;
    const int tid = threadIdx.x;
    const int logL = LOGL ? LOGL : ax.logL, L = 1 << logL, N = L >> 1, nfft = C >> logL;
    const int row0 = blockIdx.x * 2 * nfft, n1 = N + 1;
    const int rd = (a.it + 1) & 1, wr = a.it & 1;
    const long pb = b * G.plane;
    double alpha = 0.0, beta = 0.0;
    if (FIRST) {
        const int pending = st[b].lin_active;
        const double rhsn = st[b].lin_r0;
        double g = 0.0, r2 = 0.0;
        if (pending) {
            if (tid < 64) {
                for (int t = tid; t < a.nblk; t += 64) {
                    g += a.part[((long)b * a.nblk + t) * NPART];
                    r2 += a.part[((long)b * a.nblk + t) * NPART + 1];
                }
                g = wave_sum(g);
                r2 = wave_sum(r2);
                if (tid == 0) {
                    s4[0] = g;
                    s4[1] = r2;
                }
            }
            __syncthreads();
            g = s4[0];
            r2 = s4[1];
        }
        const double rel = rhsn > 0.0 ? sqrt(r2) / rhsn : 0.0;
        const int start = pending && (rel > a.tol) && (g > 0.0);
        if (blockIdx.x == 0 && tid == 0) {
            TrajState &S = st[b];
            S.cg_pending = 0;
            if (pending) {
                S.cg_gamma = S.cg_gamma0 = g;
                S.cg_beta = 0.0;
                S.lin_it = 0;
                S.lin_reltol = a.tol;
                S.aux[0] = r2;
                S.lin_rel = rel;
                S.guess_ratio = rel;
                if (!start) {
                    S.lin_active = 0;
                    if (rel > S.lin_maxrel) S.lin_maxrel = rel;
                }
                S.ci_it[0] = 0;
                S.ci_gamma[0] = g;
            }
            S.ci_active[0] = start;
// ... 454 lines not shown
```

sparse-optimal-control-of-viscous-chan-hilliard-via-gradient-descent--1d-2d_amd/csrc/vch_kernels2d.h:

```cpp
#pragma once
#include "vch_common.h"

struct TrajState {
    int slot;
    int newton_active;
    int need_trial;
    int trial_no;
    int force_accept;
    int iters;
    int nsolves;
    int ntrials;
    int stuck;
    int frozen;
    double normR;
    double alpha;
    double best_norm, best_alpha;
    double Dmin, Dmax, dbar;
    double rho;
    double kT;
    long newton_total;
    int lin_active, lin_it;
    long lin_total;
    double lin_r0, lin_prev, lin_rel, lin_maxrel;
    double cg_gamma, cg_gamma0, cg_alpha, cg_beta;
// ... 418 lines not shown
__host__ __device__ inline unsigned guess_bit(unsigned mask, int b) { return (mask >> (b & 31)) & 1u; }
__global__ __launch_bounds__(NTH) void k_guess(Geom G, Phys P, const TrajState *__restrict__ st, long slot_stride,
                                               GuessArgs ga, const double *__restrict__ D_s, double dt,
                                               double *__restrict__ rhs_s, double *__restrict__ x0, double *__restrict__ part,
                                               int which) {
    TILE_COORDS;
    const TrajState S = st[b];
    if (!S.newton_active || !S.need_trial) return;
    if (which == 1 && S.iters != 1) return;
    const double *gcf = ga.row(b);
    if (gcf[0] == 0.0) return;
    const int slot = which == 1 ? 1 - S.slot : S.slot;
    __shared__ double sx[(TY + 4) * (TX + 4)];
    __shared__ double stt[(TY + 2) * (TX + 2)];
    __shared__ double sred[4];
    constexpr int W2 = TX + 4, W1 = TX + 2;
    const long pb = b * G.plane;
    for (int e = threadIdx.x; e < W2 * (TY + 4); e += NTH) {
        int ly = e / W2, lxx = e - ly * W2;
        int gr = refl(r0 - 2 + ly, G.ns), gc = refl(c0 - 2 + lxx, G.nf);
        long o = pb + (long)gr * G.pitch + gc;
        double v = gcf[0] * ga.d[0][o];
#pragma unroll
        for (int j = 1; j < GUESS_ORD; ++j)
            if (gcf[j] != 0.0) v += gcf[j] * ga.d[j][o];
        sx[e] = isfinite(v) ? v : 0.0;
    }
    __syncthreads();
    const double *Dp = D_s + slot * slot_stride + pb;
    for (int e = threadIdx.x; e < (TY + 2) * W1; e += NTH) {
        int ly = e / W1, lxx = e - ly * W1;
        int gr = refl(r0 - 1 + ly, G.ns), gc = refl(c0 - 1 + lxx, G.nf);
        int p2 = (ly + 1) * W2 + lxx + 1;
        stt[e] = -0.5 * P.kappa * lap_at<W2>(sx, p2, G.ax, G.ay) + Dp[(long)gr * G.pitch + gc] * sx[p2];
    }
    __syncthreads();
    const double idt = 1.0 / dt;
    double acc = 0.0;
    for (int k = 0; k < TY / 4; ++k) {
        int ly = ly0 + 4 * k, r = r0 + ly, c = c0 + lx;
        if (r < G.ns && c < G.nf) {
            int p1 = (ly + 1) * W1 + lx + 1, p2 = (ly + 2) * W2 + lx + 2;
            long o = pb + (long)r * G.pitch + c, os = slot * slot_stride + o;
            const double rh = rhs_s[os] - (sx[p2] * idt - lap_at<W1>(stt, p1, G.ax, G.ay));
            rhs_s[os] = rh;
            x0[o] = sx[p2];
            acc += rh * rh;
        }
    }
    acc = wave_sum(acc);
    if ((threadIdx.x & 63) == 0) sred[threadIdx.x >> 6] = acc;
    __syncthreads();
    if (threadIdx.x == 0) {
        double *pp = part + ((long)b * nblk + blk) * NPART;
        pp[4] = pp[1];
        pp[1] = (sred[0] + sred[1]) + (sred[2] + sred[3]);
    }
}

__global__ __launch_bounds__(NTH) void k_dmu_ceiling(Geom G, Phys P, const TrajState *__restrict__ st,
                                                     long slot_stride, const double *__restrict__ x,
                                                     const double *__restrict__ phi_s,
                                                     const double *__restrict__ D_s,
                                                     const double *__restrict__ Rphi_s, double *__restrict__ dmu,
                                                     double *__restrict__ x_out, double *__restrict__ part) {
    TILE_COORDS;
    const TrajState S = st[b];
    if (!S.newton_active || S.need_trial) return;
    __shared__ double sx[(TY + 2) * (TX + 2)];
    __shared__ double sred[NPART * 4];
    constexpr int W = TX + 2;
    const long pb = b * G.plane;
    load_tile<1>(sx, x + pb, G, c0, r0);
    __syncthreads();
    double acc[1] = {1e300};
    for (int k = 0; k < TY / 4; ++k) {
        int ly = ly0 + 4 * k, r = r0 + ly, c = c0 + lx;
        if (r < G.ns && c < G.nf) {
            int p = (ly + 1) * W + lx + 1;
            long o = pb + (long)r * G.pitch + c, os = S.slot * slot_stride + o;
            double d = sx[p];
            x_out[o] = d;
            dmu[o] = 2.0 * ((-0.5 * P.kappa * lap_at<W>(sx, p, G.ax, G.ay) + D_s[os] * d) + Rphi_s[os]);
            double ph = phi_s[os];
            if (d > 0.0) acc[0] = fmin(acc[0], (1.0 - DELTA_SEP - ph) / d);
            else if (d < 0.0) acc[0] = fmin(acc[0], (-1.0 + DELTA_SEP - ph) / d);
        }
    }
    const int op[1] = {1};
    block_reduce_store<1>(acc, op, sred, part + ((long)b * nblk + blk) * NPART);
}

__global__ __launch_bounds__(NTH) void k_jac_apply(Geom G, Phys P, const double *__restrict__ phi,
                                                   const double *__restrict__ dphi, const double *__restrict__ dmu,
                                                   double dt, double *__restrict__ op_, double *__restrict__ om_) {
    TILE_COORDS;
    __shared__ double sa[(TY + 2) * (TX + 2)];
    __shared__ double sb[(TY + 2) * (TX + 2)];
    constexpr int W = TX + 2;
    const long pb = b * G.plane;
    load_tile<1>(sa, dphi + pb, G, c0, r0);
    load_tile<1>(sb, dmu + pb, G, c0, r0);
    __syncthreads();
    for (int k = 0; k < TY / 4; ++k) {
        int ly = ly0 + 4 * k, r = r0 + ly, c = c0 + lx;
        if (r < G.ns && c < G.nf) {
            int p = (ly + 1) * W + lx + 1;
            long o = pb + (long)r * G.pitch + c;
            double d = jac_diag(phi[o], P.tau / dt, P.c1);
            op_[o] = -0.5 * P.kappa * lap_at<W>(sa, p, G.ax, G.ay) + d * sa[p] - 0.5 * sb[p];
            om_[o] = sa[p] / dt - 0.5 * lap_at<W>(sb, p, G.ax, G.ay);
        }
    }
}

__global__ __launch_bounds__(NTH) void k_residual_plain(Geom G, Phys P, const double *__restrict__ pn,
                                                        const double *__restrict__ po, const double *__restrict__ mn,
                                                        const double *__restrict__ mo, const double *__restrict__ wn,
                                                        const double *__restrict__ wo, double dt,
                                                        double *__restrict__ Rp, double *__restrict__ Rm,
                                                        double *__restrict__ part) {
    TILE_COORDS;
    __shared__ double s[4][(TY + 2) * (TX + 2)];
    __shared__ double sred[NPART * 4];
    constexpr int W = TX + 2;
    const long pb = b * G.plane;
    load_tile<1>(s[0], pn + pb, G, c0, r0);
    load_tile<1>(s[1], po + pb, G, c0, r0);
    load_tile<1>(s[2], mn + pb, G, c0, r0);
    load_tile<1>(s[3], mo + pb, G, c0, r0);
    __syncthreads();
    double acc[1] = {0.0};
    for (int k = 0; k < TY / 4; ++k) {
        int ly = ly0 + 4 * k, r = r0 + ly, c = c0 + lx;
        if (r < G.ns && c < G.nf) {
            int p = (ly + 1) * W + lx + 1;
            long o = pb + (long)r * G.pitch + c;
            double rp = (P.tau * (s[0][p] - s[1][p]) / dt) -
                        0.5 * P.kappa * (lap_at<W>(s[0], p, G.ax, G.ay) + lap_at<W>(s[1], p, G.ax, G.ay)) +
                        (P.c1 * reglog(s[0][p]) + (-2.0 * P.c2 * s[1][p])) - 0.5 * (s[2][p] + s[3][p]) -
                        0.5 * (wn[o] + wo[o]);
            double rm = (s[0][p] - s[1][p]) / dt - 0.5 * (lap_at<W>(s[2], p, G.ax, G.ay) + lap_at<W>(s[3], p, G.ax, G.ay));
            Rp[o] = rp;
            Rm[o] = rm;
            acc[0] += rp * rp + rm * rm;
        }
    }
    const int op[1] = {0};
    block_reduce_store<1>(acc, op, sred, part + ((long)b * nblk + blk) * NPART);
}

__global__ __launch_bounds__(NTH) void k_mass(Geom G, const TrajState *__restrict__ st, long slot_stride,
                                              const double *__restrict__ phi_s, const double *__restrict__ wts,
                                              int do_clip, double *__restrict__ part) {
    TILE_COORDS;
    __shared__ double sred[NPART * 4];
    if (st[b].frozen) return;
    const int slot = st[b].slot;
    const double hi = 1.0 - DELTA_SEP;
    double acc[2] = {0.0, 0.0};
    for (int k = 0; k < TY / 4; ++k) {
        int r = r0 + ly0 + 4 * k, c = c0 + lx;
        if (r < G.ns && c < G.nf) {
            long o = (long)r * G.pitch + c;
            double ph = phi_s[slot * slot_stride + b * G.plane + o];
            if (do_clip) ph = fmin(fmax(ph, -hi), hi);
            double w = wts[o];
            acc[0] += w * ph;
            if (fabs(ph) < hi - 5e-3) acc[1] += w;
        }
    }
    const int op[2] = {0, 0};
    block_reduce_store<2>(acc, op, sred, part + ((long)b * nblk + blk) * NPART);
}

__device__ __forceinline__ void post_sums(const double *__restrict__ part, int nblk, int b, double *sm2) {
    if (threadIdx.x < 64) {
        double a0 = 0.0, a1 = 0.0;
        for (int t = threadIdx.x; t < nblk; t += 64) {
            a0 += part[((long)b * nblk + t) * NPART];
            a1 += part[((long)b * nblk + t) * NPART + 1];
        }
        a0 = wave_sum(a0);
        a1 = wave_sum(a1);
        if (threadIdx.x == 0) {
            sm2[0] = a0;
            sm2[1] = a1;
        }
    }
}
struct PostFix {
    double shift, hi;
    bool fix, interior_ok;
    __device__ __forceinline__ PostFix(const double *sm2, double mass0, double LxLy) {
        const double mass_err = sm2[0] - mass0, Wint = sm2[1];
        hi = 1.0 - DELTA_SEP;
        fix = fabs(mass_err) > 1e-16;
        interior_ok = Wint > 0.0;
        shift = fix ? (interior_ok ? mass_err / Wint : mass_err / LxLy) : 0.0;
    }
    __device__ __forceinline__ double apply(double v) const {
        double ph = fmin(fmax(v, -hi), hi);
        if (fix) {
            if (interior_ok) {
                if (fabs(ph) < hi - 5e-3) ph -= shift;
            } else {
                ph = fmin(fmax(ph - shift, -hi), hi);
            }
        }
        return ph;
    }
};
struct PostArgs {
    const double *part;
    double *hist;
    long hist_stride;
};

__global__ __launch_bounds__(NTH) void k_post(Geom G, Phys P, const TrajState *__restrict__ st, long slot_stride,
                                              double *__restrict__ phi_s, double *__restrict__ hist_level,
                                              long hist_stride, const double *__restrict__ part) {
    TILE_COORDS;
    const TrajState S = st[b];
    if (S.frozen) return;
    __shared__ double sm[2];
    post_sums(part, nblk, b, sm);
    __syncthreads();
    const PostFix pf(sm, S.mass0, P.LxLy);
    for (int k = 0; k < TY / 4; ++k) {
        int r = r0 + ly0 + 4 * k, c = c0 + lx;
        if (r < G.ns && c < G.nf) {
            long o = (long)r * G.pitch + c;
            long os = S.slot * slot_stride + b * G.plane + o;
            const double ph = pf.apply(phi_s[os]);
            phi_s[os] = ph;
            if (hist_level) hist_level[b * hist_stride + o] = ph;
        }
    }
}

constexpr int OPT_STRIDE = 8;
enum { OPT_B1 = 0, OPT_B2 = 1, OPT_B3 = 2, OPT_KS = 3, OPT_UMIN = 4, OPT_UMAX = 5 };

__global__ __launch_bounds__(NTH) void k_adj_rhs(Geom G, Phys P, const double *__restrict__ p,
                                                 const double *__restrict__ q, const double *__restrict__ phin,
                                                 const double *__restrict__ phin1, const double *__restrict__ qn,
                                                 const double *__restrict__ qn1, long hist_stride, double dt,
                                                 const double *__restrict__ opt_tab, double *__restrict__ rhs,
                                                 double *__restrict__ Dn, double *__restrict__ part) {
    TILE_COORDS;
    const double b1 = opt_tab[b * OPT_STRIDE + OPT_B1];
    __shared__ double sq[(TY + 2) * (TX + 2)];
    __shared__ double sred[NPART * 4];
    constexpr int W = TX + 2;
    const long pb = b * G.plane;
    load_tile<1>(sq, q + pb, G, c0, r0);
    __syncthreads();
    double acc[3] = {1e300, -1e300, 0.0};
    for (int k = 0; k < TY / 4; ++k) {
        int ly = ly0 + 4 * k, r = r0 + ly, c = c0 + lx;
        if (r < G.ns && c < G.nf) {
            int pp = (ly + 1) * W + lx + 1;
            long o = (long)r * G.pitch + c, oh = b * hist_stride + o;
            double f0 = phin[oh], f1 = phin1[oh];
            double t0 = qn ? qn[oh] : 0.0, t1 = qn1 ? qn1[oh] : 0.0;
            double src = 0.5 * dt * b1 * ((f0 - t0) + (f1 - t1));
            double dplus = fpp_log(f1, P.c1, P.c2), dn = fpp_log(f0, P.c1, P.c2);
            double v = p[pb + o] + (P.tau - 0.5 * dt * dplus) * sq[pp] + 0.5 * dt * lap_at<W>(sq, pp, G.ax, G.ay) + src;
            rhs[pb + o] = v;
            Dn[pb + o] = dn;
            acc[0] = fmin(acc[0], dn);
            acc[1] = fmax(acc[1], dn);
            acc[2] += v * v;
        }
    }
    const int op[3] = {1, 2, 0};
    block_reduce_store<3>(acc, op, sred, part + ((long)b * nblk + blk) * NPART);
}

template <int MODE>
__global__ __launch_bounds__(NTH) void k_adj_op(Geom G, Phys P, const TrajState *__restrict__ st,
                                                const double *__restrict__ x, const double *__restrict__ Dn,
                                                const double *__restrict__ rhs, double dt,
                                                double *__restrict__ out, double *__restrict__ part) {
    TILE_COORDS;
    if (MODE == 1 && !st[b].lin_active) return;
    const double dbar = MODE == 1 ? st[b].dbar : 0.0;
    __shared__ double sx[(TY + 4) * (TX + 4)];
    __shared__ double stt[(TY + 2) * (TX + 2)];
    __shared__ double sred[NPART * 4];
    constexpr int W2 = TX + 4, W1 = TX + 2;
    const long pb = b * G.plane;
    load_tile<2>(sx, x + pb, G, c0, r0);
    __syncthreads();
    for (int e = threadIdx.x; e < (TY + 2) * W1; e += NTH) {
        int ly = e / W1, lxx = e - ly * W1;
        stt[e] = -lap_at<W2>(sx, (ly + 1) * W2 + lxx + 1, G.ax, G.ay);
    }
    __syncthreads();
    double acc[2] = {0.0, 0.0};
    const double sgn = MODE == 2 ? -1.0 : 1.0;
    for (int k = 0; k < TY / 4; ++k) {
        int ly = ly0 + 4 * k, r = r0 + ly, c = c0 + lx;
        if (r < G.ns && c < G.nf) {
            int p1 = (ly + 1) * W1 + lx + 1, p2 = (ly + 2) * W2 + lx + 2;
            long o = pb + (long)r * G.pitch + c;
            double t = stt[p1], mt = -lap_at<W1>(stt, p1, G.ax, G.ay);
            double ax_ = sx[p2] + (P.tau + sgn * 0.5 * dt * Dn[o]) * t + sgn * 0.5 * dt * mt;
            if (MODE == 1) {
                double rr = rhs[o] - ax_;
// ... 151 lines not shown
__global__ __launch_bounds__(NTH) void k_grad_prox(Geom G, int tiles_f, const double *__restrict__ u,
                                                   const double *__restrict__ r, long hist_stride,
                                                   const double *__restrict__ alpha,
                                                   const double *__restrict__ opt_tab, double *__restrict__ uout,
                                                   double *__restrict__ part) {
    const int b = blockIdx.z, lvl = blockIdx.y;
    const double *ot = opt_tab + b * OPT_STRIDE;
    const double b3 = ot[OPT_B3], ks = ot[OPT_KS], umin = ot[OPT_UMIN], umax = ot[OPT_UMAX];
    const int tf = blockIdx.x % tiles_f, ts = blockIdx.x / tiles_f;
    const int c0 = tf * TX, r0 = ts * TY;
    const int lx = threadIdx.x & 63, ly0 = threadIdx.x >> 6;
    __shared__ double sred[NPART * 4];
    const double al = alpha[b];
    const long lb = b * hist_stride + (long)lvl * G.plane;
    double acc[2] = {0.0, 0.0};
    for (int k = 0; k < TY / 4; ++k) {
        int rr = r0 + ly0 + 4 * k, c = c0 + lx;
        if (rr < G.ns && c < G.nf) {
            long o = lb + (long)rr * G.pitch + c;
            double uu = u[o];
            double v = uu - al * (r[o] + b3 * uu);
            double sgn = v > 0.0 ? 1.0 : (v < 0.0 ? -1.0 : 0.0);
            double s = sgn * fmax(fabs(v) - al * ks, 0.0);
            double un = fmin(fmax(s, umin), umax);
            uout[o] = un;
            acc[0] += (un - uu) * (un - uu);
            acc[1] += uu * uu;
        }
    }
    if (part) {
        const int op[2] = {0, 0};
        block_reduce_store<2>(acc, op, sred, part + (((long)b * gridDim.y + lvl) * gridDim.x + blockIdx.x) * 4);
    }
}

__global__ __launch_bounds__(NTH) void k_kkt_count(Geom G, int tiles_f, const double *__restrict__ u,
                                                   const double *__restrict__ r, long hist_stride,
                                                   const double *__restrict__ opt_tab, double tol,
                                                   unsigned long long *__restrict__ part) {
    const int b = blockIdx.z, lvl = blockIdx.y;
    const int tf = blockIdx.x % tiles_f, ts = blockIdx.x / tiles_f;
    const int c0 = tf * TX, r0 = ts * TY;
    const int lx = threadIdx.x & 63, ly0 = threadIdx.x >> 6;
    const double ks = opt_tab[b * OPT_STRIDE + OPT_KS];
    const long lb = b * hist_stride + (long)lvl * G.plane;
    unsigned nz = 0, nsm = 0, nm = 0;
    for (int k = 0; k < TY / 4; ++k) {
        const int rr = r0 + ly0 + 4 * k, c = c0 + lx;
        const bool in = rr < G.ns && c < G.nf;
        bool zero = false, small = false;
        if (in) {
            const long o = lb + (long)rr * G.pitch + c;
            zero = fabs(u[o]) < tol;
            small = fabs(r[o]) <= ks;
        }
        nz += __popcll(__ballot(zero));
        nsm += __popcll(__ballot(small));
        nm += __popcll(__ballot(in && zero == small));
    }
    __shared__ unsigned sc[NTH / 64][3];
    if (lx == 0) {
        sc[ly0][0] = nz;
        sc[ly0][1] = nsm;
        sc[ly0][2] = nm;
    }
    __syncthreads();
    if (threadIdx.x < 3) {
        unsigned v = 0;
        for (int w = 0; w < NTH / 64; ++w) v += sc[w][threadIdx.x];
        if (v) atomicAdd(part + ((long)b * gridDim.y + lvl) * 3 + threadIdx.x, (unsigned long long)v);
    }
}

__global__ void k_kkt_fin(int levels, const unsigned long long *__restrict__ part, unsigned long long *__restrict__ counts) {
    const int b = blockIdx.x;
    __shared__ unsigned long long tot[3];
    if (threadIdx.x < 3) tot[threadIdx.x] = 0;
    __syncthreads();
    unsigned long long a[3] = {0, 0, 0};
    for (int l = threadIdx.x; l < levels; l += 64)
        for (int k = 0; k < 3; ++k) a[k] += part[((long)b * levels + l) * 3 + k];
    for (int k = 0; k < 3; ++k)
        if (a[k]) atomicAdd(&tot[k], a[k]);
    __syncthreads();
    if (threadIdx.x < 3) counts[3 * b + threadIdx.x] = tot[threadIdx.x];
}

__device__ __forceinline__ void fin_reduce(const double *part, int nblk, int b, double (&out)[NPART],
                                           const int (&op)[NPART], int n) {
    double a[NPART];
#pragma unroll
    for (int k = 0; k < NPART; ++k) a[k] = op[k] == 0 ? 0.0 : (op[k] == 1 ? 1e300 : -1e300);
    for (int t = threadIdx.x; t < nblk; t += 64) {
        const double *p = part + ((long)b * nblk + t) * NPART;
#pragma unroll
        for (int k = 0; k < NPART; ++k)
            if (k < n) {
                const double v = p[k];
                a[k] = op[k] == 0 ? a[k] + v : (op[k] == 1 ? fmin(a[k], v) : fmax(a[k], v));
            }
    }
#pragma unroll
    for (int k = 0; k < NPART; ++k)
        if (k < n) out[k] = op[k] == 0 ? wave_sum(a[k]) : (op[k] == 1 ? wave_min(a[k]) : wave_max(a[k]));
}

__device__ __forceinline__ void traj_copy_in(TrajState &dst, const TrajState *src) {
    const unsigned *s = reinterpret_cast<const unsigned *>(src);
    unsigned *d = reinterpret_cast<unsigned *>(&dst);
    for (int i = threadIdx.x; i < (int)(sizeof(TrajState) / 4); i += 64) d[i] = s[i];
    __syncthreads();
}
__device__ __forceinline__ void traj_copy_out(TrajState *dst, const TrajState &src) {
    __syncthreads();
    const unsigned *s = reinterpret_cast<const unsigned *>(&src);
    unsigned *d = reinterpret_cast<unsigned *>(dst);
    for (int i = threadIdx.x; i < (int)(sizeof(TrajState) / 4); i += 64) d[i] = s[i];
}

constexpr int HIST_CAP = 512;
constexpr double NEWTON_TOL = 1e-6;
constexpr int NEWTON_MAXIT = 500;
constexpr double ARMIJO_ETA = 1e-4;
constexpr int ARMIJO_TRIALS = 12;

__global__ void k_set_frozen(TrajState *st, const int *__restrict__ flags, int B) {
    int b = blockIdx.x * blockDim.x + threadIdx.x;
    if (b < B) st[b].frozen = flags[b];
}

__device__ __forceinline__ void cg_setup(TrajState &S, double g0, double cscale, double tol) {
    const double range = S.Dmax - S.Dmin;
    S.dbar = S.Dmin - fmax(1e-12, 0.05 * fmin(range, fabs(S.Dmin) + 1.0));
    const double den = cscale * S.dbar + g0;
    double kT = den > 0.0 ? 1.0 + cscale * (S.Dmax - S.dbar) / den : 1e12;
    const double sq = sqrt(kT);
    const double rate = (sq - 1.0) / (sq + 1.0);
    S.kT = kT;
    S.rho = rate;
    double k = rate > 1e-300 ? log(2.0 / tol) / -log(rate) : 1.0;
    S.lin_budget = (int)fmin(4000.0, ceil(k) + 2.0);
}

__device__ __forceinline__ double newton_lin_tol(double r0, double lin_tol, double eta) {
    if (!(eta > 0.0) || !(r0 > 0.0)) return lin_tol;
    if (r0 > 1e8) return fmax(lin_tol, 1e-12);
    return fmin(fmax(lin_tol, eta / r0), 0.5);
}

struct SolveOpts {
    int cheb_max;
    double scale_ratio;
    double eta1_factor;
};

__device__ __forceinline__ double cg_weight(double D, double dbar, int scaled) {
    const double dl = D - dbar;
    return scaled ? dl / D : dl;
}

constexpr int CHEB_NCAP = 200;
__device__ __forceinline__ void cheb_plan(TrajState &S, double tol) {
    const double kT = S.kT > 1.0 ? S.kT : 1.0;
    S.cheb_theta = 0.5 * (kT + 1.0);
    S.cheb_delta = 0.5 * (kT - 1.0);
    int n = 0;
    if (S.cheb_delta > 0.0) {
        const double sigma = S.cheb_theta / S.cheb_delta;
        double tkm1 = 1.0, tk = sigma;
        while (n < CHEB_NCAP && !(1.0 / tk <= tol)) {
            const double tn = 2.0 * sigma * tk - tkm1;
            tkm1 = tk;
            tk = tn;
            ++n;
        }
    }
    S.cheb_n = n;
}
__device__ __forceinline__ double cheb_last_factor(double theta, double delta, int n) {
    if (!(delta > 0.0)) return 0.0;
    const double sigma = theta / delta;
    double tkm1 = 1.0, tk = sigma;
    for (int k = 0; k < n; ++k) {
        const double tn = 2.0 * sigma * tk - tkm1;
        tkm1 = tk;
        tk = tn;
        if (!(tk < 1e280)) return 1.0 / (2.0 * sigma);
    }
    return tkm1 / tk;
}

template <int MODE>
__device__ __forceinline__ void fin_residual_update(TrajState &S, const double (&v)[NPART], bool primed, double *__restrict__ hist,
                                                    double kappa, double dt, double lin_tol, double eta, SolveOpts so);

template <int MODE>
__global__ void k_fin_residual(TrajState *st, const double *__restrict__ part, int nblk,
                               double *__restrict__ hist, double kappa, double dt, double lin_tol, double eta, int guess,
                               SolveOpts so) {
    const int b = blockIdx.x;
    __shared__ TrajState S;
    traj_copy_in(S, st + b);
    if (MODE == 2) {
        if (S.frozen) return;
        if (threadIdx.x == 0) {
            newton_begin(S);
            S.slot = 1 - S.slot;
        }
        __syncthreads();
    }
    if (!S.newton_active || !S.need_trial) return;
    double v[NPART];
    const int op[NPART] = {0, 0, 1, 2, 0, 0};
    const bool primed = guess_bit((unsigned)guess, b) && (MODE != 1 || S.iters == 1);
    fin_reduce(part, nblk, b, v, op, primed ? 5 : 4);
    if (threadIdx.x == 0)
        fin_residual_update<(MODE == 1 ? 1 : 0)>(S, v, primed, hist + (long)b * HIST_CAP, kappa, dt, lin_tol, eta, so);
    traj_copy_out(st + b, S);
}

template <int MODE>
__device__ __forceinline__ void fin_residual_update(TrajState &S, const double (&v)[NPART], bool primed, double *__restrict__ hist,
                                                    double kappa, double dt, double lin_tol, double eta, SolveOpts so) {
    const double nt = sqrt(v[0]);
    bool accept;
    if (MODE == 0) {
        accept = true;
    } else {
        S.ntrials++;
        if (S.force_accept) {
            accept = true;
        } else {
            if (nt < S.best_norm) { S.best_norm = nt; S.best_alpha = S.alpha; }
            accept = nt <= (1.0 - ARMIJO_ETA * S.alpha) * S.normR;
        }
    }
    if (accept) {
        if (MODE == 1) S.slot = 1 - S.slot;
        S.normR = nt;
        S.need_trial = 0;
        S.force_accept = 0;
        if (S.iters < HIST_CAP) hist[S.iters] = nt;
        if (S.iters < 4) S.step_R[S.iters] = nt;
        if (S.iters == 1) {
            S.R1_hist[2] = S.R1_hist[1];
            S.R1_hist[1] = S.R1_hist[0];
            S.R1_hist[0] = nt;
        }
        S.iters++;
        S.newton_total++;
        if (!(nt >= NEWTON_TOL) || S.iters > NEWTON_MAXIT) {
            if (S.iters > NEWTON_MAXIT) S.iters = NEWTON_MAXIT;
            S.newton_active = 0;
            return;
        }
        S.Dmin = v[2];
        S.Dmax = v[3];
        S.lin_r0 = sqrt(v[1]);
        S.x_primed = primed ? 1 : 0;
        S.lin_rscale = (primed && v[4] > 0.0) ? fmin(1.0, sqrt(v[1] / v[4])) : 1.0;
        if (MODE == 0) S.guess_ratio = (primed && v[4] > 0.0) ? sqrt(v[1] / v[4]) : 1.0;
        else if (primed) S.guess_ratio2 = v[4] > 0.0 ? sqrt(v[1] / v[4]) : 1.0;
        double eta_eff = eta;
        if (MODE == 0 && eta > 0.0 && so.eta1_factor > 0.0 && S.R1_hist[0] > 0.0 && S.R1_hist[1] > 0.0 && S.R1_hist[2] > 0.0)
            eta_eff = fmax(eta, so.eta1_factor * fmin(S.R1_hist[0], fmin(S.R1_hist[1], S.R1_hist[2])));
        S.lin_reltol = newton_lin_tol(S.lin_r0, lin_tol, eta_eff);
        cg_setup(S, 2.0 * sqrt(0.5 * kappa / dt), 1.0, S.lin_reltol);
        cheb_plan(S, S.lin_reltol);
        S.use_cheb = (so.cheb_max >= 0 && S.cheb_n <= so.cheb_max) ? 1 : 0;
        S.scaled = (!S.use_cheb && so.scale_ratio > 0.0 && S.Dmax > so.scale_ratio * S.Dmin) ? 1 : 0;
        S.lin_active = 1;
        S.lin_it = 0;
        S.lin_prev = 1e300;
        S.lin_rel = 1.0;
        S.nsolves++;
        S.step_solves++;
        if (S.step_solves <= 4) {
            S.step_tol[S.step_solves - 1] = S.lin_reltol;
            S.step_kT[S.step_solves - 1] = S.kT;
            S.step_chn[S.step_solves - 1] = S.cheb_n;
            S.step_form[S.step_solves - 1] = S.use_cheb;
        }
    } else {
        S.alpha *= 0.5;
        S.trial_no++;
        if (S.trial_no >= ARMIJO_TRIALS) {
            if (S.best_norm < S.normR) {
                S.alpha = S.best_alpha;
                S.force_accept = 1;
            } else {
                S.stuck = 1;
                S.need_trial = 0;
                while (S.iters < NEWTON_MAXIT) {
                    if (S.iters < HIST_CAP) hist[S.iters] = S.normR;
                    S.iters++;
                }
                S.newton_active = 0;
            }
        }
    }
}

struct EvalFin {
    unsigned *counter;
    double *hist;
    double kappa, lin_tol, eta;
    SolveOpts so;
};

__device__ __forceinline__ void store_agent(double *p, double v) { __hip_atomic_store(p, v, __ATOMIC_RELAXED, __HIP_MEMORY_SCOPE_AGENT); }
__device__ __forceinline__ double load_agent(const double *p) {
    return __hip_atomic_load(p, __ATOMIC_RELAXED, __HIP_MEMORY_SCOPE_AGENT);
}

__device__ __forceinline__ void fin_reduce_agent(const double *part, int nblk, int b, double (&out)[NPART], const int (&op)[NPART], int n) {
    double a[NPART];
#pragma unroll
    for (int k = 0; k < NPART; ++k) a[k] = op[k] == 0 ? 0.0 : (op[k] == 1 ? 1e300 : -1e300);
    for (int t = threadIdx.x; t < nblk; t += 64) {
        const double *p = part + ((long)b * nblk + t) * NPART;
#pragma unroll
        for (int k = 0; k < NPART; ++k)
            if (k < n) {
                const double v = load_agent(p + k);
                a[k] = op[k] == 0 ? a[k] + v : (op[k] == 1 ? fmin(a[k], v) : fmax(a[k], v));
            }
    }
#pragma unroll
    for (int k = 0; k < NPART; ++k)
        if (k < n) out[k] = op[k] == 0 ? wave_sum(a[k]) : (op[k] == 1 ? wave_min(a[k]) : wave_max(a[k]));
}

#ifndef EVAL_MINBLK
#define EVAL_MINBLK 5
#endif
template <int MODE, bool FIN_INSIDE>
__global__ __launch_bounds__(NTH, EVAL_MINBLK) void k_eval(Geom G, Phys P, TrajState *st, long slot_stride, double *phi_s, double *mu_s,
                                              double *Rphi_s, double *rhs_s, double *D_s, const double *dphi, double *cphi,
                                              double *cmu, double dt, double *part, const double *w, const double *un,
                                              const double *unp1, long u_stride, double *wnew, GuessArgs ga, double *x0,
                                              EvalFin fin, PostArgs post) {
    TILE_COORDS;
    const int S_slot = st[b].slot, S_iters = MODE == 0 ? 0 : st[b].iters;
    const double S_alpha = MODE == 0 ? 0.0 : st[b].alpha;
    if (MODE == 0) {
        if (st[b].frozen) {
            if (blk == 0 && threadIdx.x == 0) st[b].newton_active = st[b].need_trial = st[b].lin_active = 0;
            return;
        }
    } else {
        if (!st[b].newton_active || !st[b].need_trial) return;
    }
    __shared__ double sp[(TY + 4) * (TX + 4)];
    __shared__ double sd[MODE == 2 ? (TY + 4) * (TX + 4) : 1];
    __shared__ double sm[(TY + 2) * (TX + 2)];
    __shared__ double sr[MODE == 0 ? (TY + 2) * (TX + 2) : 1];
    __shared__ double sred[NPART * 4];
    __shared__ int s_last;
    constexpr int W2 = TX + 4, W1 = TX + 2;
    const long pb = b * G.plane;
    const int src = S_slot, dst = 1 - S_slot;
    const double tdt = P.tau / dt;
    const double *gcf = ga.row(b);
    const bool do_guess = gcf[0] != 0.0 && (MODE == 0 || S_iters == 1);
    double rm[TY / 4], rh[TY / 4];
    double acc[5] = {0.0, 0.0, 1e300, -1e300, 0.0};
    if (MODE == 0) {
        constexpr int N1 = (TY + 2) * W1, I1 = (N1 + NTH - 1) / NTH;
        if (post.part) {
            __shared__ double s_post[2];
            constexpr int I2 = (W2 * (TY + 4) + NTH - 1) / NTH;
            double raw[I2];
#pragma unroll
            for (int i = 0; i < I2; ++i) {
                const int e = threadIdx.x + i * NTH;
                raw[i] = 0.0;
                if (e < W2 * (TY + 4)) {
                    int ly = e / W2, lxx = e - ly * W2;
                    int gr = refl(r0 - 2 + ly, G.ns), gc = refl(c0 - 2 + lxx, G.nf);
                    raw[i] = phi_s[src * slot_stride + pb + (long)gr * G.pitch + gc];
                }
            }
            post_sums(post.part, nblk, (int)b, s_post);
            __syncthreads();
            const PostFix pf(s_post, st[b].mass0, P.LxLy);
#pragma unroll
            for (int i = 0; i < I2; ++i) {
                const int e = threadIdx.x + i * NTH;
                if (e < W2 * (TY + 4)) sp[e] = pf.apply(raw[i]);
            }
        } else {
            load_tile<2>(sp, phi_s + src * slot_stride + pb, G, c0, r0);
        }
        load_tile<1>(sm, mu_s + src * slot_stride + pb, G, c0, r0);
        double vW[I1], vU0[I1], vU1[I1];
#pragma unroll
        for (int i = 0; i < I1; ++i) {
            const int e = threadIdx.x + i * NTH;
            vW[i] = vU0[i] = vU1[i] = 0.0;
            if (e < N1) {
                int ly = e / W1, lxx = e - ly * W1;
                int gr = refl(r0 - 1 + ly, G.ns), gc = refl(c0 - 1 + lxx, G.nf);
                long o = (long)gr * G.pitch + gc;
                vW[i] = w[pb + o];
                vU0[i] = un ? un[b * u_stride + o] : 0.0;
                vU1[i] = unp1 ? unp1[b * u_stride + o] : 0.0;
            }
        }
        __syncthreads();
        for (int k = 0; k < TY / 4; ++k) {
            int ly = ly0 + 4 * k, r = r0 + ly, c = c0 + lx;
            rm[k] = 0.0;
            if (r < G.ns && c < G.nf) {
                int p1 = (ly + 1) * W1 + lx + 1, p2 = (ly + 2) * W2 + lx + 2;
                const double cm = -sp[p2] / dt - 0.5 * lap_at<W1>(sm, p1, G.ax, G.ay);
                cmu[pb + (long)r * G.pitch + c] = cm;
                rm[k] = cm;
            }
        }
        __syncthreads();
        const double gdt = P.gamma / dt;
#pragma unroll
        for (int i = 0; i < I1; ++i) {
            const int e = threadIdx.x + i * NTH;
            if (e >= N1) continue;
            int ly = e / W1, lxx = e - ly * W1;
            int rr = r0 - 1 + ly, cc = c0 - 1 + lxx;
            int gr = refl(rr, G.ns), gc = refl(cc, G.nf);
            int p2 = (ly + 1) * W2 + lxx + 1;
            long o = (long)gr * G.pitch + gc, ob = pb + o;
            const double u0 = vU0[i], u1 = vU1[i], wo = vW[i];
            const double wn = ((gdt - 0.5) * wo + 0.5 * (u1 + u0)) / (gdt + 0.5);
            const double ph = sp[p2], lp = lap_at<W2>(sp, p2, G.ax, G.ay);
            const double m0 = -P.kappa * lp + (P.c1 * reglog(ph) - 2.0 * P.c2 * ph) - wn;
            const double cp = -(P.tau / dt) * ph - 0.5 * P.kappa * lp - 2.0 * P.c2 * ph - 0.5 * sm[e] - 0.5 * (wn + wo);
            sr[e] = tdt * ph - 0.5 * P.kappa * lp + P.c1 * reglog(ph) - 0.5 * m0 + cp;
            sm[e] = m0;
            if (ly >= 1 && ly <= TY && lxx >= 1 && lxx <= TX && rr < G.ns && cc < G.nf) {
                wnew[ob] = wn;
                cphi[ob] = cp;
            }
        }
        __syncthreads();
        for (int k = 0; k < TY / 4; ++k) {
            int ly = ly0 + 4 * k, r = r0 + ly, c = c0 + lx;
            rh[k] = 0.0;
            if (r < G.ns && c < G.nf) {
                int p1 = (ly + 1) * W1 + lx + 1, p2 = (ly + 2) * W2 + lx + 2;
                long od = dst * slot_stride + pb + (long)r * G.pitch + c;
                const double ph = sp[p2], rp = sr[p1];
                const double rmv = ph / dt - 0.5 * lap_at<W1>(sm, p1, G.ax, G.ay) + rm[k];
                const double rhv = -rmv + lap_at<W1>(sr, p1, G.ax, G.ay);
                const double d = jac_diag(ph, tdt, P.c1);
                phi_s[od] = ph;
                if (post.part && post.hist) post.hist[b * post.hist_stride + (long)r * G.pitch + c] = ph;
                mu_s[od] = sm[p1];
                Rphi_s[od] = rp;
                D_s[od] = d;
                rh[k] = rhv;
                acc[0] += rp * rp + rmv * rmv;
                acc[2] = fmin(acc[2], d);
                acc[3] = fmax(acc[3], d);
            }
        }
    } else {
        const double *phi_o = phi_s + src * slot_stride + pb, *mu_o = mu_s + src * slot_stride + pb;
        const double *D_o = D_s + src * slot_stride + pb, *R_o = Rphi_s + src * slot_stride + pb;
        constexpr int N1 = (TY + 2) * W1, I1 = (N1 + NTH - 1) / NTH;
        double pd[(W2 * (TY + 4) + NTH - 1) / NTH], pp[(W2 * (TY + 4) + NTH - 1) / NTH];
        {
            int i = 0;
#pragma unroll
            for (int e = threadIdx.x; e < W2 * (TY + 4); e += NTH, ++i) {
                int ly = e / W2, lxx = e - ly * W2;
                int gr = refl(r0 - 2 + ly, G.ns), gc = refl(c0 - 2 + lxx, G.nf);
                long o = (long)gr * G.pitch + gc;
                pd[i] = dphi[pb + o];
                pp[i] = phi_o[o];
            }
        }
        double vD[I1], vR[I1], vM[I1], vC[I1], vcm[TY / 4];
#pragma unroll
        for (int i = 0; i < I1; ++i) {
            const int e = threadIdx.x + i * NTH;
            vD[i] = vR[i] = vM[i] = vC[i] = 0.0;
            if (e < N1) {
                int ly = e / W1, lxx = e - ly * W1;
                int gr = refl(r0 - 1 + ly, G.ns), gc = refl(c0 - 1 + lxx, G.nf);
                long o = (long)gr * G.pitch + gc;
                vD[i] = D_o[o];
                vR[i] = R_o[o];
                vM[i] = mu_o[o];
                vC[i] = cphi[pb + o];
            }
        }
#pragma unroll
        for (int k = 0; k < TY / 4; ++k) {
            int r = r0 + ly0 + 4 * k, c = c0 + lx;
            vcm[k] = (r < G.ns && c < G.nf) ? cmu[pb + (long)r * G.pitch + c] : 0.0;
        }
        {
            int i = 0;
#pragma unroll
            for (int e = threadIdx.x; e < W2 * (TY + 4); e += NTH, ++i) {
// ... 2 lines not shown
            }
        }
        __syncthreads();
#pragma unroll
        for (int i = 0; i < I1; ++i) {
            const int e = threadIdx.x + i * NTH;
            if (e < N1) {
                int ly = e / W1, lxx = e - ly * W1;
                int p2 = (ly + 1) * W2 + lxx + 1;
                const double Dv = vD[i], Rv = vR[i], Mv = vM[i];
                const double dm = 2.0 * ((-0.5 * P.kappa * lap_at<W2>(sd, p2, G.ax, G.ay) + Dv * sd[p2]) + Rv);
                sm[e] = Mv + S_alpha * dm;
            }
        }
        __syncthreads();
        double mt[TY / 4];
        for (int k = 0; k < TY / 4; ++k) {
            int ly = ly0 + 4 * k, r = r0 + ly, c = c0 + lx;
            rm[k] = mt[k] = 0.0;
            if (r < G.ns && c < G.nf) {
                int p1 = (ly + 1) * W1 + lx + 1, p2 = (ly + 2) * W2 + lx + 2;
                const double cm = vcm[k];
                rm[k] = sp[p2] / dt - 0.5 * lap_at<W1>(sm, p1, G.ax, G.ay) + cm;
                mt[k] = sm[p1];
            }
        }
        __syncthreads();
#pragma unroll
        for (int i = 0; i < I1; ++i) {
            const int e = threadIdx.x + i * NTH;
            if (e < N1) {
                int ly = e / W1, lxx = e - ly * W1;
                int p2 = (ly + 1) * W2 + lxx + 1;
                const double cp = vC[i];
                double ph = sp[p2];
                sm[e] = tdt * ph - 0.5 * P.kappa * lap_at<W2>(sp, p2, G.ax, G.ay) + P.c1 * reglog(ph) - 0.5 * sm[e] + cp;
            }
        }
        __syncthreads();
        for (int k = 0; k < TY / 4; ++k) {
            int ly = ly0 + 4 * k, r = r0 + ly, c = c0 + lx;
            rh[k] = 0.0;
            if (r < G.ns && c < G.nf) {
                int p1 = (ly + 1) * W1 + lx + 1, p2 = (ly + 2) * W2 + lx + 2;
                long od = dst * slot_stride + pb + (long)r * G.pitch + c;
                double ph = sp[p2], rp = sm[p1];
                double rhv = -rm[k] + lap_at<W1>(sm, p1, G.ax, G.ay);
                double d = jac_diag(ph, tdt, P.c1);
                phi_s[od] = ph;
                mu_s[od] = mt[k];
                Rphi_s[od] = rp;
                D_s[od] = d;
                rh[k] = rhv;
                acc[0] += rp * rp + rm[k] * rm[k];
                acc[2] = fmin(acc[2], d);
                acc[3] = fmax(acc[3], d);
            }
        }
    }
    if (do_guess) {
        double *X = MODE == 0 ? sp : sd;
        double *STT = MODE == 0 ? sr : sp;
        __syncthreads();
        for (int e = threadIdx.x; e < (TY + 2) * W1; e += NTH) {
            int ly = e / W1, lxx = e - ly * W1;
            sm[e] = jac_diag(sp[(ly + 1) * W2 + lxx + 1], tdt, P.c1);
        }
        __syncthreads();
        for (int e = threadIdx.x; e < W2 * (TY + 4); e += NTH) {
            int ly = e / W2, lxx = e - ly * W2;
            int gr = refl(r0 - 2 + ly, G.ns), gc = refl(c0 - 2 + lxx, G.nf);
            long o = pb + (long)gr * G.pitch + gc;
            double v = gcf[0] * ga.d[0][o];
#pragma unroll
            for (int j = 1; j < GUESS_ORD; ++j)
                if (gcf[j] != 0.0) v += gcf[j] * ga.d[j][o];
            X[e] = isfinite(v) ? v : 0.0;
        }
        __syncthreads();
        for (int e = threadIdx.x; e < (TY + 2) * W1; e += NTH) {
            int ly = e / W1, lxx = e - ly * W1;
            int p2 = (ly + 1) * W2 + lxx + 1;
            STT[e] = -0.5 * P.kappa * lap_at<W2>(X, p2, G.ax, G.ay) + sm[e] * X[p2];
        }
        double xv[TY / 4];
        for (int k = 0; k < TY / 4; ++k) xv[k] = X[(ly0 + 4 * k + 2) * W2 + lx + 2];
        __syncthreads();
        const double idt = 1.0 / dt;
        for (int k = 0; k < TY / 4; ++k) {
            int ly = ly0 + 4 * k, r = r0 + ly, c = c0 + lx;
            if (r < G.ns && c < G.nf) {
                int p1 = (ly + 1) * W1 + lx + 1;
                const double full = rh[k];
                const double defl = full - (xv[k] * idt - lap_at<W1>(STT, p1, G.ax, G.ay));
                x0[pb + (long)r * G.pitch + c] = xv[k];
                acc[4] += full * full;
                rh[k] = defl;
            }
        }
    }
    for (int k = 0; k < TY / 4; ++k) {
        int r = r0 + ly0 + 4 * k, c = c0 + lx;
        if (r < G.ns && c < G.nf) {
            rhs_s[dst * slot_stride + pb + (long)r * G.pitch + c] = rh[k];
            acc[1] += rh[k] * rh[k];
        }
    }
    {
        const int lane = threadIdx.x & 63, wv = threadIdx.x >> 6;
        const int op5[5] = {0, 0, 1, 2, 0};
#pragma unroll
        for (int k = 0; k < 5; ++k) {
            double r_ = op5[k] == 0 ? wave_sum(acc[k]) : (op5[k] == 1 ? wave_min(acc[k]) : wave_max(acc[k]));
            if (lane == 0) sred[k * 4 + wv] = r_;
        }
        __syncthreads();
        if (threadIdx.x == 0) {
            double *pp = part + ((long)b * nblk + blk) * NPART;
#pragma unroll
            for (int k = 0; k < 5; ++k) {
                const double a = sred[k * 4], bb = sred[k * 4 + 1], cc = sred[k * 4 + 2], dd = sred[k * 4 + 3];
                const double v = op5[k] == 0 ? (a + bb) + (cc + dd)
                                             : (op5[k] == 1 ? fmin(fmin(a, bb), fmin(cc, dd)) : fmax(fmax(a, bb), fmax(cc, dd)));
                if (FIN_INSIDE) store_agent(pp + k, v);
                else pp[k] = v;
            }
            if (FIN_INSIDE) {
                asm volatile("s_waitcnt vmcnt(0)" ::: "memory");
                const unsigned old = __hip_atomic_fetch_add(fin.counter + b, 1u, __ATOMIC_RELAXED, __HIP_MEMORY_SCOPE_AGENT);
                s_last = old == (unsigned)(nblk - 1) ? 1 : 0;
            }
        }
        if (!FIN_INSIDE) return;
        __syncthreads();
        if (!s_last || threadIdx.x >= 64) return;
    }
    if (FIN_INSIDE) {
        double v[NPART];
        const int op[NPART] = {0, 0, 1, 2, 0, 0};
        fin_reduce_agent(part, nblk, b, v, op, do_guess ? 5 : 4);
        if (threadIdx.x != 0) return;
        __hip_atomic_store(fin.counter + b, 0u, __ATOMIC_RELAXED, __HIP_MEMORY_SCOPE_AGENT);
        TrajState S = st[b];
        if (MODE == 0) {
            newton_begin(S);
            S.slot = dst;
        }
        fin_residual_update<(MODE == 0 ? 0 : 1)>(S, v, do_guess, fin.hist + (long)b * HIST_CAP, fin.kappa, dt, fin.lin_tol, fin.eta,
                                                 fin.so);
        st[b] = S;
    }
}

__device__ __forceinline__ double fin_sum1(const double *part, int n, int b, int stride, int k) {
    double a = 0.0;
    for (int t = threadIdx.x; t < n; t += 64) a += part[((long)b * n + t) * stride + k];
    return wave_sum(a);
}

__global__ void k_fin_cg_init(TrajState *st, const double *__restrict__ gpart, int gnblk) {
    const int b = blockIdx.x;
    TrajState &S = st[b];
    if (threadIdx.x == 0) {
        S.cg_pending = 0;
        if (!S.lin_active) S.ci_active[0] = 0;
    }
    if (!S.lin_active) return;
    double g = fin_sum1(gpart, gnblk, b, 1, 0);
    if (threadIdx.x != 0) return;
    S.cg_gamma = S.cg_gamma0 = g;
    S.cg_beta = 0.0;
    S.lin_it = 0;
    S.lin_rel = 1.0;
    S.ci_active[0] = S.lin_active;
    S.ci_it[0] = 0;
    S.ci_gamma[0] = g;
}

struct CgNext {
    int active, breakdown, it;
    double alpha, beta, gamma, rel;
};
__device__ __forceinline__ CgNext cg_next(double pq, double qq, double gamma, double gamma0, int it_old, double tol,
                                          int maxit) {
    CgNext n;
    n.it = it_old;
    if (!(pq > 0.0) || !(gamma > 0.0)) {
        n.active = 0; n.breakdown = 1; n.alpha = 0.0; n.beta = 0.0; n.gamma = fmax(gamma, 0.0);
        n.rel = gamma0 > 0.0 ? sqrt(fmax(gamma, 0.0) / gamma0) : 0.0;
        return n;
    }
    n.breakdown = 0;
    n.alpha = gamma / pq;
    double gn = n.alpha * n.alpha * qq - gamma;
    if (gn > 1e-13 * gamma) {
        n.beta = gn / gamma;
    } else {
        gn = 1e-13 * gamma;
        n.beta = 0.0;
    }
    n.gamma = gn;
    n.it = it_old + 1;
    n.rel = sqrt(gn / gamma0);
    n.active = (n.rel > tol && n.it < maxit) ? 1 : 0;
    return n;
}

__device__ __forceinline__ void cg_sums(const double *__restrict__ gpart, const double *__restrict__ gpart2, int gnblk,
                                        const double *__restrict__ part, int nblk, int pslot, int direct, int b,
                                        double *s3 ) {
    const int wv = threadIdx.x >> 6, lane = threadIdx.x & 63;
    if (wv < 3) {
        const double *src = wv == 0 ? gpart : (wv == 1 ? gpart2 : part + pslot);
        const int n = wv == 2 ? nblk : gnblk, stride = wv == 2 ? NPART : 1;
        double a = 0.0;
        if (wv < 2 || direct)
            for (int t = lane; t < n; t += 64) a += src[((long)b * n + t) * stride];
        a = wave_sum(a);
        if (lane == 0) s3[wv] = a;
    }
    __syncthreads();
}

__device__ __forceinline__ void cg_record(TrajState &S, const CgNext &n, int wr) {
    S.cg_alpha = n.alpha;
    S.cg_beta = n.beta;
    S.cg_gamma = n.gamma;
    S.lin_rel = n.rel;
    if (!n.breakdown) {
        S.lin_it = n.it;
        S.lin_total++;
    }
    if (!n.active && n.rel * S.lin_rscale > S.lin_maxrel) S.lin_maxrel = n.rel * S.lin_rscale;
    if (!n.active) S.lin_maxabs = fmax(S.lin_maxabs, n.rel * S.lin_r0);
    if (n.it > S.step_lin_max) S.step_lin_max = n.it;
    if (S.step_solves >= 1 && S.step_solves <= 4 && n.it > S.step_lin[S.step_solves - 1]) S.step_lin[S.step_solves - 1] = n.it;
    S.ci_active[wr] = n.active;
    S.ci_it[wr] = n.it;
    S.ci_gamma[wr] = n.gamma;
}

__global__ void k_fin_cg_step(TrajState *st, const double *__restrict__ gpart, const double *__restrict__ gpart2,
                              int gnblk, const double *__restrict__ part, int nblk, int pslot, int direct, int pbuf,
                              int rd, double tol, int maxit) {
    const int b = blockIdx.x;
    TrajState &S = st[b];
    __shared__ double s3[3];
    if (!S.lin_active) return;
    if (!S.ci_active[rd]) {
        if (threadIdx.x == 0) { S.lin_active = 0; S.cg_pending = 0; }
        return;
    }
    cg_sums(gpart, gpart2, gnblk, part, nblk, pslot, direct, b, s3);
    if (threadIdx.x != 0) return;
    const CgNext n = cg_next(s3[0], s3[1], direct ? s3[2] : S.ci_gamma[rd], S.cg_gamma0, S.ci_it[rd], S.lin_reltol, maxit);
    cg_record(S, n, rd ^ 1);
    S.cg_pending = n.breakdown ? 0 : 1;
    S.cg_pbuf = pbuf;
    S.lin_active = n.active;
}

__global__ void k_cg_publish(TrajState *st, int rd, int B) {
    const int b = blockIdx.x * blockDim.x + threadIdx.x;
    if (b < B && st[b].lin_active && !st[b].ci_active[rd]) st[b].lin_active = 0;
}

__global__ void k_fin_cg_alpha(TrajState *st, const double *__restrict__ part, int n, int stride, int k) {
    const int b = blockIdx.x;
    TrajState &S = st[b];
    if (!S.lin_active) return;
    double pq = fin_sum1(part, n, b, stride, k);
    if (threadIdx.x != 0) return;
    if (!(pq > 0.0)) {
        S.lin_active = 0;
        S.cg_alpha = 0.0;
        if (S.lin_rel > S.lin_maxrel) S.lin_maxrel = S.lin_rel;
        return;
    }
    S.cg_alpha = S.cg_gamma / pq;
}

__global__ void k_fin_cg_beta(TrajState *st, const double *__restrict__ part, int nblk, int mode, double tol,
                              int maxit, int init) {
    const int b = blockIdx.x;
    TrajState &S = st[b];
    if (!S.lin_active) return;
    double gn = fin_sum1(part, nblk, b, NPART, 0);
    double rr = mode == 1 ? fin_sum1(part, nblk, b, NPART, 1) : 0.0;
    if (threadIdx.x != 0) return;
    if (init) {
        S.cg_gamma = S.cg_gamma0 = gn;
        S.cg_beta = 0.0;
        S.lin_it = 0;
    } else {
        S.cg_beta = S.cg_gamma > 0.0 ? gn / S.cg_gamma : 0.0;
        S.cg_gamma = gn;
        S.lin_it++;
        S.lin_total++;
    }
    S.lin_rel = mode == 1 ? (S.lin_r0 > 0.0 ? sqrt(rr) / S.lin_r0 : 0.0)
                          : (S.cg_gamma0 > 0.0 ? sqrt(gn / S.cg_gamma0) : 0.0);
    if (!(S.lin_rel > tol) || S.lin_it >= maxit) {
        S.lin_active = 0;
        if (S.lin_rel > S.lin_maxrel) S.lin_maxrel = S.lin_rel;
    }
}

struct ChebFin {
    int enq, gnblk;
    const double *g0, *gn;
    const double *cmin;
};
__global__ void k_fin_ceiling(TrajState *st, const double *__restrict__ part, int nblk, int strict, int fin_copy, ChebFin cheb) {
    const int b = blockIdx.x;
    __shared__ TrajState S;
    traj_copy_in(S, st + b);
    if (!S.newton_active || S.need_trial) return;
    if ((cheb.enq >= 0) != (S.use_cheb != 0)) return;
    int lin_active = S.lin_active;
    if (cheb.enq >= 0 && lin_active) {
        if (S.cheb_n > cheb.enq) return;
        double rel = 1.0;
        if (S.cheb_n >= 1) {
            const double g0 = fin_sum1(cheb.g0, cheb.gnblk, b, 1, 0), gn = fin_sum1(cheb.gn, cheb.gnblk, b, 1, 0);
            rel = g0 > 0.0 ? sqrt(fmax(gn, 0.0) / g0) : 0.0;
        }
        if (threadIdx.x == 0) {
            rel *= cheb_last_factor(S.cheb_theta, S.cheb_delta, S.cheb_n);
            S.lin_rel = rel;
            S.lin_it = S.cheb_n;
            S.lin_total += S.cheb_n;
            if (rel * S.lin_rscale > S.lin_maxrel) S.lin_maxrel = rel * S.lin_rscale;
            S.lin_maxabs = fmax(S.lin_maxabs, rel * S.lin_r0);
            if (S.cheb_n > S.step_lin_max) S.step_lin_max = S.cheb_n;
            if (S.step_solves >= 1 && S.step_solves <= 4) S.step_lin[S.step_solves - 1] = S.cheb_n;
        }
        lin_active = 0;
    }
    if (fin_copy >= 0 && lin_active) {
        lin_active = fin_copy == 0 ? S.ci_active[0] : S.ci_active[1];
        if (strict && lin_active) {
            if (threadIdx.x == 0) st[b].lin_active = lin_active;
            return;
        }
    }
    if (strict && lin_active) return;
    double v[NPART];
    const int op[NPART] = {1, 0, 0, 0, 0, 0};
    if (cheb.enq >= 0 && cheb.cmin) {
        double a = 1e300;
        for (int t = threadIdx.x; t < cheb.gnblk; t += 64) a = fmin(a, cheb.cmin[(long)b * cheb.gnblk + t]);
        v[0] = wave_min(a);
    } else {
        fin_reduce(part, nblk, b, v, op, 1);
    }
    if (threadIdx.x == 0) {
        double amax = 2.0;
        if (v[0] < 1e299) amax = fmin(amax, 0.9 * v[0]);
        if (!isfinite(amax) || amax <= 0.0) amax = 1.0;
        S.alpha = fmin(1.0, amax);
        if (lin_active && S.lin_rel > S.lin_maxrel) S.lin_maxrel = S.lin_rel;
        S.lin_active = 0;
        S.need_trial = 1;
        S.trial_no = 0;
        S.force_accept = 0;
        S.best_norm = 1e300;
        S.best_alpha = S.alpha;
    }
    traj_copy_out(st + b, S);
}

__global__ void k_fin_mass(TrajState *st, const double *__restrict__ part, int nblk, int init) {
    const int b = blockIdx.x;
    TrajState &S = st[b];
    if (S.frozen) return;
    double v[NPART];
    const int op[NPART] = {0, 0, 0, 0, 0, 0};
    fin_reduce(part, nblk, b, v, op, 2);
    if (threadIdx.x != 0) return;
    if (init) {
        S.mass0 = v[0];
        S.mass_err = 0.0;
    } else {
        S.mass_err = v[0] - S.mass0;
    }
    S.Wint = v[1];
}

__global__ void k_fin_lin_begin(TrajState *st, const double *__restrict__ part, int nblk, int mode,
                                double tau, double kappa, double dt, double lin_tol) {
    const int b = blockIdx.x;
    TrajState &S = st[b];
    if (threadIdx.x == 0 && S.lin_active) {
        S.lin_unconv++;
        if (S.lin_rel > S.lin_maxrel) S.lin_maxrel = S.lin_rel;
    }
    double v[NPART];
    const int op0[NPART] = {1, 2, 0, 0, 0, 0};
    const int op1[NPART] = {0, 0, 0, 0, 0, 0};
    const int op2[NPART] = {0, 0, 1, 2, 0, 0};
    if (mode == 0) fin_reduce(part, nblk, b, v, op0, 3);
    else if (mode == 1) fin_reduce(part, nblk, b, v, op1, 1);
    else fin_reduce(part, nblk, b, v, op2, 4);
    if (threadIdx.x != 0) return;
    double dmin = 0.0, dmax = 0.0, r0;
    if (mode == 0) { dmin = v[0]; dmax = v[1]; r0 = sqrt(v[2]); }
    else if (mode == 1) { r0 = sqrt(v[0]); }
    else { dmin = v[2]; dmax = v[3]; r0 = sqrt(v[1]); }
    S.Dmin = dmin;
    S.Dmax = dmax;
    if (mode == 2) cg_setup(S, 2.0 * sqrt(0.5 * kappa / dt), 1.0, lin_tol);
    else cg_setup(S, tau + 2.0 * sqrt(0.5 * dt), 0.5 * dt, lin_tol);
    S.lin_r0 = r0;
    S.lin_active = (mode == 2 || r0 > 0.0) ? 1 : 0;
    S.lin_it = 0;
    S.lin_prev = 1e300;
    S.lin_rel = 1.0;
    S.lin_reltol = lin_tol;
    S.use_cheb = 0;
    S.scaled = 0;
    S.nsolves++;
}

__global__ __launch_bounds__(NTH) void k_solve_setup(Geom G, Phys P, const double *__restrict__ a,
                                                     const double *__restrict__ bv, const double *__restrict__ phi,
                                                     double dt, double *__restrict__ Rphi, double *__restrict__ rhs,
                                                     double *__restrict__ D, double *__restrict__ part) {
    TILE_COORDS;
    __shared__ double s[(TY + 2) * (TX + 2)];
    __shared__ double sred[NPART * 4];
    constexpr int W = TX + 2;
    const long pb = b * G.plane;
    load_tile<1>(s, a + pb, G, c0, r0);
    __syncthreads();
    double acc[4] = {0.0, 0.0, 1e300, -1e300};
    for (int k = 0; k < TY / 4; ++k) {
        int ly = ly0 + 4 * k, r = r0 + ly, c = c0 + lx;
        if (r < G.ns && c < G.nf) {
            int p = (ly + 1) * W + lx + 1;
            long o = pb + (long)r * G.pitch + c;
            double rh = bv[o] - lap_at<W>(s, p, G.ax, G.ay);
            double d = jac_diag(phi[o], P.tau / dt, P.c1);
            Rphi[o] = -s[p];
            rhs[o] = rh;
            D[o] = d;
            acc[1] += rh * rh;
            acc[2] = fmin(acc[2], d);
            acc[3] = fmax(acc[3], d);
        }
    }
    const int op[4] = {0, 0, 1, 2};
    block_reduce_store<4>(acc, op, sred, part + ((long)b * nblk + blk) * NPART);
}

__global__ __launch_bounds__(NTH) void k_adj_setup(Geom G, Phys P, const double *__restrict__ phi,
                                                   const double *__restrict__ rhs, double *__restrict__ Dn,
                                                   double *__restrict__ part) {
    TILE_COORDS;
    __shared__ double sred[NPART * 4];
    double acc[3] = {1e300, -1e300, 0.0};
    for (int k = 0; k < TY / 4; ++k) {
        int r = r0 + ly0 + 4 * k, c = c0 + lx;
        if (r < G.ns && c < G.nf) {
            long o = b * G.plane + (long)r * G.pitch + c;
            double d = phi ? fpp_log(phi[o], P.c1, P.c2) : 0.0;
            Dn[o] = d;
            acc[0] = fmin(acc[0], d);
            acc[1] = fmax(acc[1], d);
            if (rhs) acc[2] += rhs[o] * rhs[o];
        }
    }
    const int op[3] = {1, 2, 0};
    block_reduce_store<3>(acc, op, sred, part + ((long)b * nblk + blk) * NPART);
}

__global__ __launch_bounds__(NTH) void k_solve_w(Geom G, const double *__restrict__ w, const double *__restrict__ un,
                                                 const double *__restrict__ unp1, double gdt, double *__restrict__ out) {
    TILE_COORDS;
    for (int k = 0; k < TY / 4; ++k) {
        int r = r0 + ly0 + 4 * k, c = c0 + lx;
        if (r < G.ns && c < G.nf) {
            long o = b * G.plane + (long)r * G.pitch + c;
            double u0 = un ? un[o] : 0.0, u1 = unp1 ? unp1[o] : 0.0;
            out[o] = ((gdt - 0.5) * w[o] + 0.5 * (u1 + u0)) / (gdt + 0.5);
        }
    }
}

__global__ __launch_bounds__(NTH) void k_adj_guess(Geom G, double *__restrict__ x, GuessArgs ga, double *__restrict__ keep) {
    TILE_COORDS;
    for (int k = 0; k < TY / 4; ++k) {
        int r = r0 + ly0 + 4 * k, c = c0 + lx;
        if (r < G.ns && c < G.nf) {
            const long o = b * G.plane + (long)r * G.pitch + c;
            const double p1 = x[o];
            const double *gcf = ga.row(b);
            double v = gcf[0] * p1;
#pragma unroll
            for (int j = 1; j < GUESS_ORD; ++j)
                if (gcf[j] != 0.0) v += gcf[j] * ga.d[j][o];
            keep[o] = p1;
            x[o] = isfinite(v) ? v : p1;
        }
    }
}

__global__ void k_reset_longest(TrajState *st, int B) {
    const int b = blockIdx.x * blockDim.x + threadIdx.x;
    if (b < B) st[b].step_lin_max = 0;
}

__global__ __launch_bounds__(NTH) void k_fill(Geom G, double *__restrict__ x, double v) {
    TILE_COORDS;
    for (int k = 0; k < TY / 4; ++k) {
        int r = r0 + ly0 + 4 * k, c = c0 + lx;
        if (r < G.ns && c < G.nf) x[b * G.plane + (long)r * G.pitch + c] = v;
    }
}

__global__ __launch_bounds__(NTH) void k_ramp(Geom G, int tiles_f, const double *__restrict__ phi0,
                                              const double *__restrict__ phiT, const double *__restrict__ tfrac,
// ... 200 lines not shown
```

Before: 5.239 PGD iterations/s.

## Fold Chebyshev ceiling into atomic cell, publish state from fin kernel, launch mass early

The Chebyshev sweep now folds the per-block step-ceiling minimum into a per-trajectory atomic cell. The trial eval kernel and k_fin_residual read that cell directly, so the separate k_fin_ceiling launch is dropped. k_fin_residual can also write the TrajState into host-mapped memory and set per-trajectory sequence flags, which removes the extra k_publish_state launch before the host spin-wait. The mass kernel is launched before the sync so it overlaps the host wait, and it is relaunched if Newton iterations continue. The cost is more state-machine coupling and per-trajectory seq polling on the host.

Result: faster. 5.332 PGD iterations/s (median of 6 runs) (+1.8%).

```diff
diff --git a/sparse-optimal-control-of-viscous-chan-hilliard-via-gradient-descent--1d-2d_amd/csrc/vch_engine2d.hip b/sparse-optimal-control-of-viscous-chan-hilliard-via-gradient-descent--1d-2d_amd/csrc/vch_engine2d.hip
--- a/sparse-optimal-control-of-viscous-chan-hilliard-via-gradient-descent--1d-2d_amd/csrc/vch_engine2d.hip
+++ b/sparse-optimal-control-of-viscous-chan-hilliard-via-gradient-descent--1d-2d_amd/csrc/vch_engine2d.hip
@@ -118,6 +118,12 @@
     TrajState *st_pub;
     unsigned long long *seq_pub, seq_next;
     bool look_spin;
+    bool mass_early, fin_publish, ceil_cell_on;
+    unsigned long long *ceil_cell;
+    bool cell_now;
+    int trial_enq;
+    unsigned long long pub_pending;
+    bool mass_done;
     int *frozen_dev;
     double *hist_dev, *hist_host;
     double *Q1f, *Q2f, *Q1s, *Q2s, *mf, *ms;
@@ -237,32 +243,42 @@
 static inline long hist_stride(const vch2d_ctx *c) { return (long)(c->Mmax + 1) * c->G.plane; }
 
 __global__ void k_publish_state(const unsigned *__restrict__ st, int nwords, unsigned *__restrict__ dst,
-                                unsigned long long *seq, unsigned long long val) {
+                                unsigned long long *seq, int nseq, unsigned long long val) {
     for (int i = threadIdx.x; i < nwords; i += blockDim.x) dst[i] = st[i];
     __threadfence_system();
     __syncthreads();
-    if (threadIdx.x == 0) __hip_atomic_store(seq, val, __ATOMIC_RELEASE, __HIP_MEMORY_SCOPE_SYSTEM);
+    for (int i = threadIdx.x; i < nseq; i += blockDim.x) __hip_atomic_store(seq + i, val, __ATOMIC_RELEASE, __HIP_MEMORY_SCOPE_SYSTEM);
 }
 
 static int sync_state(vch2d_ctx *c, bool full = true) {
     c->n_sync++;
     if (full || !c->look_spin) {
+        c->pub_pending = 0;
         HIPCHK(hipMemcpyAsync(c->st_host, c->st, sizeof(TrajState) * c->B, hipMemcpyDeviceToHost, c->stream));
         HIPCHK(hipStreamSynchronize(c->stream));
         return 0;
     }
-    const unsigned long long want = ++c->seq_next;
     static_assert(sizeof(TrajState) % 4 == 0, "TrajState is copied in 32-bit words");
-    hipLaunchKernelGGL(k_publish_state, dim3(1), dim3(256), 0, c->stream, (const unsigned *)c->st,
-                       (int)(sizeof(TrajState) / 4 * c->B), (unsigned *)c->st_pub, c->seq_pub, want);
-    HIPCHK(hipGetLastError());
+    unsigned long long want = c->pub_pending;
+    c->pub_pending = 0;
+    if (!want) {
+        want = ++c->seq_next;
+        hipLaunchKernelGGL(k_publish_state, dim3(1), dim3(256), 0, c->stream, (const unsigned *)c->st,
+                           (int)(sizeof(TrajState) / 4 * c->B), (unsigned *)c->st_pub, c->seq_pub, c->B, want);
+        HIPCHK(hipGetLastError());
+    }
+    auto arrived = [&]() {
+        for (int b = 0; b < c->B; ++b)
+            if (__atomic_load_n(c->seq_pub + b, __ATOMIC_ACQUIRE) != want) return false;
+        return true;
+    };
     const auto t0 = std::chrono::steady_clock::now();
-    for (unsigned spins = 1; __atomic_load_n(c->seq_pub, __ATOMIC_ACQUIRE) != want; ++spins) {
+    for (unsigned spins = 1; !arrived(); ++spins) {
         __builtin_ia32_pause();
         if ((spins & 0x3fff) == 0) {
             const hipError_t q = hipStreamQuery(c->stream);
             if (q != hipSuccess && q != hipErrorNotReady) return vch_fail(VCH_ERR_HIP, "sync_state: %s", hipGetErrorString(q));
-            if (q == hipSuccess && __atomic_load_n(c->seq_pub, __ATOMIC_ACQUIRE) != want)
+            if (q == hipSuccess && !arrived())
                 return vch_fail(VCH_ERR_STATE, "sync_state: stream drained but the state was not published");
             if (std::chrono::steady_clock::now() - t0 > std::chrono::seconds(120))
                 return vch_fail(VCH_ERR_STATE, "sync_state: no state from the device after 120 s");
@@ -350,6 +366,14 @@
     c->post_pending = false;
     c->post_hist = nullptr;
     c->fin_counter = nullptr;
+    auto env_on = [](const char *name) { const char *e = getenv(name); return !(e && atoi(e) == 0); };
+    c->mass_early = env_on("VCH_MASS_EARLY");
+    c->fin_publish = env_on("VCH_FIN_PUBLISH");
+    c->ceil_cell_on = env_on("VCH_CEIL_CELL");
+    c->ceil_cell = nullptr;
+    c->cell_now = c->mass_done = false;
+    c->trial_enq = -1;
+    c->pub_pending = 0;
     for (int &n : c->spec_chn) n = 2;
     c->cheb_margin = 1;
     if (const char *e = getenv("VCH_CHEB_MARGIN")) c->cheb_margin = std::max(0, atoi(e));
@@ -400,6 +424,8 @@
     if (hipMalloc((void **)&c->frozen_dev, sizeof(int) * batch) != hipSuccess) return fail("hipMalloc");
     if (hipMalloc((void **)&c->fin_counter, sizeof(unsigned) * batch) != hipSuccess) return fail("hipMalloc");
     hipMemsetAsync(c->fin_counter, 0, sizeof(unsigned) * batch, c->stream);
+    if (hipMalloc((void **)&c->ceil_cell, sizeof(unsigned long long) * CeilCell::STRIDE * batch) != hipSuccess) return fail("hipMalloc");
+    hipMemsetAsync(c->ceil_cell, 0, sizeof(unsigned long long) * CeilCell::STRIDE * batch, c->stream);
     if (hipHostMalloc((void **)&c->st_host, sizeof(TrajState) * batch) != hipSuccess) return fail("hipHostMalloc");
     c->st_pub = nullptr;
     c->seq_pub = nullptr;
@@ -407,14 +433,15 @@
     c->look_spin = !(getenv("VCH_LOOK_SPIN") && atoi(getenv("VCH_LOOK_SPIN")) == 0);
     if (c->look_spin) {
         if (hipHostMalloc((void **)&c->st_pub, sizeof(TrajState) * batch, hipHostMallocMapped | hipHostMallocCoherent) != hipSuccess ||
-            hipHostMalloc((void **)&c->seq_pub, 64, hipHostMallocMapped | hipHostMallocCoherent) != hipSuccess) {
+            hipHostMalloc((void **)&c->seq_pub, std::max<size_t>(64, sizeof(unsigned long long) * batch),
+                          hipHostMallocMapped | hipHostMallocCoherent) != hipSuccess) {
             (void)hipGetLastError();
             if (c->st_pub) hipHostFree(c->st_pub);
             c->st_pub = nullptr;
             c->seq_pub = nullptr;
             c->look_spin = false;
         } else {
-            *c->seq_pub = 0;
+            for (int b = 0; b < batch; ++b) c->seq_pub[b] = 0;
         }
     }
     if (hipHostMalloc((void **)&c->hist_host, sizeof(double) * batch * HIST_CAP) != hipSuccess) return fail("hipHostMalloc");
@@ -517,6 +544,7 @@
     hipFree(c->frozen_dev);
     if (c->kkt_dev) hipFree(c->kkt_dev);
     if (c->fin_counter) hipFree(c->fin_counter);
+    if (c->ceil_cell) hipFree(c->ceil_cell);
     if (c->tw_fh) hipFree(c->tw_fh);
     if (c->tw_sh) hipFree(c->tw_sh);
     if (c->tw_f) hipFree(c->tw_f);
@@ -723,7 +751,8 @@
         ChebSweepArgs a{c->r, c->r, c->cg_p[j & 1], c->cg_p[(j + 1) & 1], c->cg_p[(j + 1) & 1], c->xf, c->x0g, c->D_s, c->slot_stride,
                         j == 0 ? c->gpart : c->gpart2, j, scale, c->phi_s, c->gpart3,
                         c->guess_wr >= 0 ? c->dprev[c->guess_wr] : (double *)nullptr,
-                        (c->guess_wr >= 0 && c->guess2_on) ? c->dprev2[c->guess_wr] : (double *)nullptr};
+                        (c->guess_wr >= 0 && c->guess2_on) ? c->dprev2[c->guess_wr] : (double *)nullptr,
+                        c->cell_now ? c->ceil_cell : (unsigned long long *)nullptr};
         VCHCHK(cheb_rows(c, a, j == 0));
         if (j < n_enq) {
             const SpecArgs sp{c0, 0.0, 1.0, c2, c->ms, c->mf, nullptr, c->D_s, c->slot_stride, c->gpart, c->gpart2, 1};
@@ -737,8 +766,10 @@
     const bool spectral = c->use_fft && !c->half_f && !c->half_s;
     const ChebFin nocheb{-1, 0, nullptr, nullptr, nullptr};
     if (spectral && c->cheb_enq >= 0) {
-        LAUNCH(k_fin_ceiling, dim3(c->B), dim3(64), c->st, c->part, c->nblk, strict, -1,
-               ChebFin{c->cheb_enq, c->gnblk, c->gpart, c->gpart2, c->gpart3});
+        if (c->cell_now) c->trial_enq = c->cheb_enq;
+        else
+            LAUNCH(k_fin_ceiling, dim3(c->B), dim3(64), c->st, c->part, c->nblk, strict, -1,
+                   ChebFin{c->cheb_enq, c->gnblk, c->gpart, c->gpart2, c->gpart3});
     }
     if (spectral && c->cg_last >= 0) {
         const int last = c->cg_last, rd = last & 1;
@@ -759,18 +790,33 @@
     return 0;
 }
 
+static const FinTail NO_FIN_TAIL{ChebFin{-1, 0, nullptr, nullptr, nullptr}, nullptr, nullptr, 0};
+static FinTail publish_tail(vch2d_ctx *c, FinTail t) {
+    c->pub_pending = ++c->seq_next;
+    t.pub = c->st_pub;
+    t.seq = c->seq_pub;
+    t.val = c->pub_pending;
+    return t;
+}
+
 static int residual_trial(vch2d_ctx *c, double dt, bool inline_dmu, bool fused, bool fin_inside, bool guess, double eta,
-                          const SolveOpts &so, const EvalFin &efin) {
+                          const SolveOpts &so, const EvalFin &efin, bool publish) {
     if (inline_dmu && fused) {
         GuessArgs gt = c->gtab2;
         if (!guess) memset(gt.c, 0, sizeof(gt.c));
+        EvalFin ef = efin;
+        ef.cheb_enq = c->trial_enq;
+        c->trial_enq = -1;
         auto k_trial = fin_inside ? k_eval<2, true> : k_eval<2, false>;
         LAUNCHC(PC_RESIDUAL, k_trial, c->grid, dim3(NTH), c->G, c->P, c->st, c->slot_stride, c->phi_s, c->mu_s, c->Rphi_s, c->rhs_s,
                 c->D_s, (const double *)c->xf, c->cphi, c->cmu, dt, c->part, (const double *)nullptr, (const double *)nullptr,
-                (const double *)nullptr, 0L, (double *)nullptr, gt, c->x0g, efin, PostArgs{nullptr, nullptr, 0});
-        if (!fin_inside)
+                (const double *)nullptr, 0L, (double *)nullptr, gt, c->x0g, ef, PostArgs{nullptr, nullptr, 0});
+        if (!fin_inside) {
+            FinTail tail{ChebFin{ef.cheb_enq, c->gnblk, c->gpart, c->gpart2, nullptr}, nullptr, nullptr, 0};
+            if (publish) tail = publish_tail(c, tail);
             LAUNCH((k_fin_residual<1>), dim3(c->B), dim3(64), c->st, c->part, c->nblk, c->hist_dev, c->P.kappa, dt, c->lin_tol, eta,
-                   guess ? (int)c->gmask2 : 0, so);
+                   guess ? (int)c->gmask2 : 0, so, tail);
+        }
         return 0;
     }
     if (inline_dmu)
@@ -783,7 +829,7 @@
         LAUNCHC(PC_GUESS, k_guess, c->grid, dim3(NTH), c->G, c->P, c->st, c->slot_stride, c->gtab2, (const double *)c->D_s, dt,
                 c->rhs_s, c->x0g, c->part, 1);
     LAUNCH((k_fin_residual<1>), dim3(c->B), dim3(64), c->st, c->part, c->nblk, c->hist_dev, c->P.kappa, dt, c->lin_tol, eta,
-           guess ? (int)c->gmask2 : 0, so);
+           guess ? (int)c->gmask2 : 0, so, NO_FIN_TAIL);
     return 0;
 }
 
@@ -795,8 +841,13 @@
     const bool inline_dmu = in_march && spectral;
     const int cheb_max_ = (in_march && spectral && c->cheb_on && eta_ > 0.0) ? c->cheb_max : -1;
     const bool fin_inside = c->fused_mode == 1;
-    const SolveOpts so_{cheb_max_, spectral ? c->cg_scale_ratio : 0.0, in_march ? c->eta1_factor : 0.0};
-    const EvalFin efin_{fin_inside ? c->fin_counter : (unsigned *)nullptr, c->hist_dev, c->P.kappa, c->lin_tol, eta_, so_};
+    const bool chain = fused && !fin_inside && c->look_spin;
+    c->cell_now = chain && c->ceil_cell_on && cheb_max_ >= 0;
+    c->trial_enq = -1;
+    const bool fin_pub = chain && c->fin_publish;
+    const SolveOpts so_{cheb_max_, spectral ? c->cg_scale_ratio : 0.0, in_march ? c->eta1_factor : 0.0,
+                        c->cell_now ? c->ceil_cell : (unsigned long long *)nullptr};
+    const EvalFin efin_{fin_inside ? c->fin_counter : (unsigned *)nullptr, c->hist_dev, c->P.kappa, c->lin_tol, eta_, so_, -1};
     const bool guess = in_march && c->guess_on && c->gmask1 != 0;
     const bool guess2 = in_march && c->guess_on && c->guess2_on && c->gmask2 != 0;
     if (fused) {
@@ -810,7 +861,7 @@
                 c->x0g, efin_, post_);
         if (!fin_inside)
             LAUNCH((k_fin_residual<2>), dim3(c->B), dim3(64), c->st, c->part, c->nblk, c->hist_dev, c->P.kappa, dt, c->lin_tol, eta_,
-                   guess ? (int)c->gmask1 : 0, so_);
+                   guess ? (int)c->gmask1 : 0, so_, NO_FIN_TAIL);
     } else {
         LAUNCH(k_prepare, c->grid, dim3(NTH), c->G, c->P, c->st, c->slot_stride, c->phi_s, c->mu_s, c->w, un, unp1, u_stride,
                wnew_in, dt, c->wnew, c->mu0, c->cphi, c->cmu);
@@ -820,16 +871,19 @@
             LAUNCHC(PC_GUESS, k_guess, c->grid, dim3(NTH), c->G, c->P, c->st, c->slot_stride, c->gtab1, (const double *)c->D_s, dt, c->rhs_s,
                    c->x0g, c->part, 0);
         LAUNCH((k_fin_residual<0>), dim3(c->B), dim3(64), c->st, c->part, c->nblk, c->hist_dev, c->P.kappa, dt, c->lin_tol, eta_,
-               guess ? (int)c->gmask1 : 0, so_);
+               guess ? (int)c->gmask1 : 0, so_, NO_FIN_TAIL);
     }
     if (c->spec) {
         for (int s = 0; s < c->spec_slots; ++s) {
             if (cheb_max_ >= 0 && (c->spec_form[s] & 1)) VCHCHK(cheb_solve(c, dt, c->spec_chn[s]));
             if (cheb_max_ < 0 || (c->spec_form[s] & 2)) VCHCHK(schur_solve(c, dt, c->spec_cgb[s], false));
             VCHCHK(dmu_ceiling(c, 1));
-            VCHCHK(residual_trial(c, dt, inline_dmu, fused, fin_inside, guess2, eta_, so_, efin_));
-        }
-    }
+            VCHCHK(residual_trial(c, dt, inline_dmu, fused, fin_inside, guess2, eta_, so_, efin_,
+                                  fin_pub && s == c->spec_slots - 1));
+        }
+    }
+    c->mass_done = chain && c->mass_early;
+    if (c->mass_done) LAUNCH(k_mass, c->grid, dim3(NTH), c->G, c->st, c->slot_stride, c->phi_s, c->wts_mass, 1, c->part_mass, 1);
     VCHCHK(sync_state(c, false));
     auto any_active = [&]() {
         for (int b = 0; b < c->B; ++b)
@@ -851,6 +905,7 @@
                 S.newton_total, S.ntrials, S.use_cheb, S.cheb_n, S.step_R[0], S.step_R[1], S.step_R[2], S.lin_r0);
     }
     int guard = 0;
+    const bool unfit = any_active();
     while (any_active()) {
         if (++guard > NEWTON_MAXIT + 2) return vch_fail(VCH_ERR_STATE, "newton_level: state machine did not terminate");
         int need = -1, budget = 0;
@@ -865,11 +920,12 @@
         VCHCHK(dmu_ceiling(c, 0));
         int tguard = 0;
         do {
-            VCHCHK(residual_trial(c, dt, inline_dmu, fused, fin_inside, guess2, eta_, so_, efin_));
+            VCHCHK(residual_trial(c, dt, inline_dmu, fused, fin_inside, guess2, eta_, so_, efin_, fin_pub));
             VCHCHK(sync_state(c, false));
             if (++tguard > ARMIJO_TRIALS + 2) return vch_fail(VCH_ERR_STATE, "newton_level: Armijo loop did not terminate");
         } while (any_trial());
     }
+    if (unfit && c->mass_done) LAUNCH(k_mass, c->grid, dim3(NTH), c->G, c->st, c->slot_stride, c->phi_s, c->wts_mass, 1, c->part_mass, 0);
     {
         int solves = 1, sweeps[4] = {1, 1, 1, 1}, chn[4] = {0, 0, 0, 0}, form[4] = {0, 0, 0, 0}, longest = 1, bound = 1, chmax = 0,
             form_any = 0;
@@ -1187,7 +1243,7 @@
     const long hs = hist_stride(c);
     HIPCHK(hipMemsetAsync(c->w, 0, sizeof(double) * c->B * c->G.plane, c->stream));
     LAUNCH(k_init_mu, c->grid, dim3(NTH), c->G, c->P, c->phi_s, c->w, c->mu_s);
-    LAUNCH(k_mass, c->grid, dim3(NTH), c->G, c->st, c->slot_stride, c->phi_s, c->wts_mass, 0, c->part);
+    LAUNCH(k_mass, c->grid, dim3(NTH), c->G, c->st, c->slot_stride, c->phi_s, c->wts_mass, 0, c->part, 0);
     LAUNCH(k_fin_mass, dim3(c->B), dim3(64), c->st, c->part, c->nblk, 1);
     c->post_pending = false;
     const bool fold_post = c->post_fold && c->fused_on && c->use_fft && !c->half_f && !c->half_s;
@@ -1257,7 +1313,8 @@
             }
         }
         VCHCHK(newton_level(c, dt[step], un, unp1, hs, nullptr, true));
-        LAUNCH(k_mass, c->grid, dim3(NTH), c->G, c->st, c->slot_stride, c->phi_s, c->wts_mass, 1, c->part_mass);
+        if (!c->mass_done) LAUNCH(k_mass, c->grid, dim3(NTH), c->G, c->st, c->slot_stride, c->phi_s, c->wts_mass, 1, c->part_mass, 0);
+        c->mass_done = false;
         double *const lvl = hist_out ? hist_out + (long)(step + 1) * c->G.plane : (double *)nullptr;
         if (fold_post && step + 1 < M) {
             c->post_pending = true;
diff --git a/sparse-optimal-control-of-viscous-chan-hilliard-via-gradient-descent--1d-2d_amd/csrc/vch_fft.h b/sparse-optimal-control-of-viscous-chan-hilliard-via-gradient-descent--1d-2d_amd/csrc/vch_fft.h
--- a/sparse-optimal-control-of-viscous-chan-hilliard-via-gradient-descent--1d-2d_amd/csrc/vch_fft.h
+++ b/sparse-optimal-control-of-viscous-chan-hilliard-via-gradient-descent--1d-2d_amd/csrc/vch_fft.h
@@ -598,6 +598,7 @@
     const double *phi_s;
     double *cmin;
     double *keep1, *keep2;
+    unsigned long long *cell;
 };
 
 #ifndef CHEB_MINW
@@ -767,7 +768,10 @@
                 mn = fmin(mn, sred[T / 64 + w]);
             }
             if (need_norm) a.gpart[(long)b * gridDim.x + blockIdx.x] = tot;
-            if (last) a.cmin[(long)b * gridDim.x + blockIdx.x] = mn;
+            if (last) {
+                if (a.cell) CeilCell::fold(a.cell + b * CeilCell::STRIDE, mn);
+                else a.cmin[(long)b * gridDim.x + blockIdx.x] = mn;
+            }
         }
     }
 }
diff --git a/sparse-optimal-control-of-viscous-chan-hilliard-via-gradient-descent--1d-2d_amd/csrc/vch_kernels2d.h b/sparse-optimal-control-of-viscous-chan-hilliard-via-gradient-descent--1d-2d_amd/csrc/vch_kernels2d.h
--- a/sparse-optimal-control-of-viscous-chan-hilliard-via-gradient-descent--1d-2d_amd/csrc/vch_kernels2d.h
+++ b/sparse-optimal-control-of-viscous-chan-hilliard-via-gradient-descent--1d-2d_amd/csrc/vch_kernels2d.h
@@ -594,10 +594,11 @@
 
 __global__ __launch_bounds__(NTH) void k_mass(Geom G, const TrajState *__restrict__ st, long slot_stride,
                                               const double *__restrict__ phi_s, const double *__restrict__ wts,
-                                              int do_clip, double *__restrict__ part) {
+                                              int do_clip, double *__restrict__ part, int ended_only) {
     TILE_COORDS;
     __shared__ double sred[NPART * 4];
     if (st[b].frozen) return;
+    if (ended_only && st[b].newton_active) return;
     const int slot = st[b].slot;
     const double hi = 1.0 - DELTA_SEP;
     double acc[2] = {0.0, 0.0};
@@ -1055,7 +1056,35 @@
     int cheb_max;
     double scale_ratio;
     double eta1_factor;
+    unsigned long long *cell;
 };
+
+struct CeilCell {
+    static constexpr int STRIDE = 16;
+    static constexpr double FREE = 2.0;
+    static __device__ __forceinline__ unsigned long long key(double v) {
+        const unsigned long long u = (unsigned long long)__double_as_longlong(v);
+        return (u >> 63) ? ~u : (u | 0x8000000000000000ull);
+    }
+    static __device__ __forceinline__ double value(unsigned long long k) {
+        return __longlong_as_double((long long)((k >> 63) ? (k ^ 0x8000000000000000ull) : ~k));
+    }
+    static __device__ __forceinline__ void reset(unsigned long long *c) {
+        __hip_atomic_store(c, key(1e300), __ATOMIC_RELAXED, __HIP_MEMORY_SCOPE_AGENT);
+    }
+    static __device__ __forceinline__ void fold(unsigned long long *c, double v) {
+        if (v < FREE) __hip_atomic_fetch_min(c, key(v), __ATOMIC_RELAXED, __HIP_MEMORY_SCOPE_AGENT);
+    }
+    static __device__ __forceinline__ double load(const unsigned long long *c) {
+        return value(__hip_atomic_load(c, __ATOMIC_RELAXED, __HIP_MEMORY_SCOPE_AGENT));
+    }
+};
+__device__ __forceinline__ double ceiling_alpha(double vmin) {
+    double amax = 2.0;
+    if (vmin < 1e299) amax = fmin(amax, 0.9 * vmin);
+    if (!isfinite(amax) || amax <= 0.0) amax = 1.0;
+    return fmin(1.0, amax);
+}
 
 __device__ __forceinline__ double cg_weight(double D, double dbar, int scaled) {
     const double dl = D - dbar;
@@ -1093,6 +1122,49 @@
     return tkm1 / tk;
 }
 
+__device__ __forceinline__ double fin_sum1(const double *part, int n, int b, int stride, int k) {
+    double a = 0.0;
+    for (int t = threadIdx.x; t < n; t += 64) a += part[((long)b * n + t) * stride + k];
+    return wave_sum(a);
+}
+
+struct ChebFin {
+    int enq, gnblk;
+    const double *g0, *gn;
+    const double *cmin;
+};
+__device__ __forceinline__ double cheb_solve_rel(int cheb_n, const ChebFin &cheb, int b) {
+    if (cheb_n < 1) return 1.0;
+    const double g0 = fin_sum1(cheb.g0, cheb.gnblk, b, 1, 0), gn = fin_sum1(cheb.gn, cheb.gnblk, b, 1, 0);
+    return g0 > 0.0 ? sqrt(fmax(gn, 0.0) / g0) : 0.0;
+}
+__device__ __forceinline__ void cheb_close_books(TrajState &S, double rel) {
+    rel *= cheb_last_factor(S.cheb_theta, S.cheb_delta, S.cheb_n);
+    S.lin_rel = rel;
+    S.lin_it = S.cheb_n;
+    S.lin_total += S.cheb_n;
+    if (rel * S.lin_rscale > S.lin_maxrel) S.lin_maxrel = rel * S.lin_rscale;
+    S.lin_maxabs = fmax(S.lin_maxabs, rel * S.lin_r0);
+    if (S.cheb_n > S.step_lin_max) S.step_lin_max = S.cheb_n;
+    if (S.step_solves >= 1 && S.step_solves <= 4) S.step_lin[S.step_solves - 1] = S.cheb_n;
+}
+__device__ __forceinline__ void ceiling_arm(TrajState &S, double vmin, int lin_active) {
+    S.alpha = ceiling_alpha(vmin);
+    if (lin_active && S.lin_rel > S.lin_maxrel) S.lin_maxrel = S.lin_rel;
+    S.lin_active = 0;
+    S.need_trial = 1;
+    S.trial_no = 0;
+    S.force_accept = 0;
+    S.best_norm = 1e300;
+    S.best_alpha = S.alpha;
+}
+
+struct FinTail {
+    ChebFin cheb;
+    TrajState *pub;
+    unsigned long long *seq, val;
+};
+
 template <int MODE>
 __device__ __forceinline__ void fin_residual_update(TrajState &S, const double (&v)[NPART], bool primed, double *__restrict__ hist,
                                                     double kappa, double dt, double lin_tol, double eta, SolveOpts so);
@@ -1100,26 +1172,50 @@
 template <int MODE>
 __global__ void k_fin_residual(TrajState *st, const double *__restrict__ part, int nblk,
                                double *__restrict__ hist, double kappa, double dt, double lin_tol, double eta, int guess,
-                               SolveOpts so) {
+                               SolveOpts so, FinTail tail) {
     const int b = blockIdx.x;
     __shared__ TrajState S;
     traj_copy_in(S, st + b);
+    bool go = true;
     if (MODE == 2) {
-        if (S.frozen) return;
-        if (threadIdx.x == 0) {
+        go = !S.frozen;
+        if (go && threadIdx.x == 0) {
             newton_begin(S);
             S.slot = 1 - S.slot;
         }
         __syncthreads();
     }
-    if (!S.newton_active || !S.need_trial) return;
-    double v[NPART];
-    const int op[NPART] = {0, 0, 1, 2, 0, 0};
-    const bool primed = guess_bit((unsigned)guess, b) && (MODE != 1 || S.iters == 1);
-    fin_reduce(part, nblk, b, v, op, primed ? 5 : 4);
-    if (threadIdx.x == 0)
-        fin_residual_update<(MODE == 1 ? 1 : 0)>(S, v, primed, hist + (long)b * HIST_CAP, kappa, dt, lin_tol, eta, so);
-    traj_copy_out(st + b, S);
+    go = go && S.newton_active && S.need_trial;
+    if (MODE == 1 && !go && tail.cheb.enq >= 0 && S.newton_active && S.use_cheb && !(S.lin_active && S.cheb_n > tail.cheb.enq)) {
+        const int books = S.lin_active;
+        const double rel = books ? cheb_solve_rel(S.cheb_n, tail.cheb, b) : 1.0;
+        __syncthreads();
+        if (threadIdx.x == 0) {
+            if (books) cheb_close_books(S, rel);
+            ceiling_arm(S, CeilCell::load(so.cell + b * CeilCell::STRIDE), 0);
+        }
+        __syncthreads();
+        go = true;
+    }
+    if (go) {
+        double v[NPART];
+        const int op[NPART] = {0, 0, 1, 2, 0, 0};
+        const bool primed = guess_bit((unsigned)guess, b) && (MODE != 1 || S.iters == 1);
+        fin_reduce(part, nblk, b, v, op, primed ? 5 : 4);
+        if (so.cell) so.cell += b * CeilCell::STRIDE;
+        if (threadIdx.x == 0)
+            fin_residual_update<(MODE == 1 ? 1 : 0)>(S, v, primed, hist + (long)b * HIST_CAP, kappa, dt, lin_tol, eta, so);
+        traj_copy_out(st + b, S);
+    }
+    if (tail.pub) {
+        __syncthreads();
+        const unsigned *s = reinterpret_cast<const unsigned *>(&S);
+        unsigned *d = reinterpret_cast<unsigned *>(tail.pub + b);
+        for (int i = threadIdx.x; i < (int)(sizeof(TrajState) / 4); i += 64) d[i] = s[i];
+        __threadfence_system();
+        __syncthreads();
+        if (threadIdx.x == 0) __hip_atomic_store(tail.seq + b, tail.val, __ATOMIC_RELEASE, __HIP_MEMORY_SCOPE_SYSTEM);
+    }
 }
 
 template <int MODE>
@@ -1173,6 +1269,7 @@
         S.use_cheb = (so.cheb_max >= 0 && S.cheb_n <= so.cheb_max) ? 1 : 0;
         S.scaled = (!S.use_cheb && so.scale_ratio > 0.0 && S.Dmax > so.scale_ratio * S.Dmin) ? 1 : 0;
         S.lin_active = 1;
+        if (so.cell) CeilCell::reset(so.cell);
         S.lin_it = 0;
         S.lin_prev = 1e300;
         S.lin_rel = 1.0;
@@ -1209,6 +1306,7 @@
     double *hist;
     double kappa, lin_tol, eta;
     SolveOpts so;
+    int cheb_enq;
 };
 
 __device__ __forceinline__ void store_agent(double *p, double v) { __hip_atomic_store(p, v, __ATOMIC_RELAXED, __HIP_MEMORY_SCOPE_AGENT); }
@@ -1245,14 +1343,20 @@
                                               EvalFin fin, PostArgs post) {
     TILE_COORDS;
     const int S_slot = st[b].slot, S_iters = MODE == 0 ? 0 : st[b].iters;
-    const double S_alpha = MODE == 0 ? 0.0 : st[b].alpha;
+    double S_alpha = MODE == 0 ? 0.0 : st[b].alpha;
+    const bool use_cell = MODE == 2 && !FIN_INSIDE && fin.cheb_enq >= 0;
+    const double cell_min = use_cell ? CeilCell::load(fin.so.cell + b * CeilCell::STRIDE) : 1e300;
     if (MODE == 0) {
         if (st[b].frozen) {
             if (blk == 0 && threadIdx.x == 0) st[b].newton_active = st[b].need_trial = st[b].lin_active = 0;
             return;
         }
     } else {
-        if (!st[b].newton_active || !st[b].need_trial) return;
+        if (!st[b].newton_active) return;
+        if (!st[b].need_trial) {
+            if (!use_cell || !st[b].use_cheb || (st[b].lin_active && st[b].cheb_n > fin.cheb_enq)) return;
+            S_alpha = ceiling_alpha(cell_min);
+        }
     }
     __shared__ double sp[(TY + 4) * (TX + 4)];
     __shared__ double sd[MODE == 2 ? (TY + 4) * (TX + 4) : 1];
@@ -1561,12 +1665,6 @@
     }
 }
 
-__device__ __forceinline__ double fin_sum1(const double *part, int n, int b, int stride, int k) {
-    double a = 0.0;
-    for (int t = threadIdx.x; t < n; t += 64) a += part[((long)b * n + t) * stride + k];
-    return wave_sum(a);
-}
-
 __global__ void k_fin_cg_init(TrajState *st, const double *__restrict__ gpart, int gnblk) {
     const int b = blockIdx.x;
     TrajState &S = st[b];
@@ -1715,11 +1813,6 @@
     }
 }
 
-struct ChebFin {
-    int enq, gnblk;
-    const double *g0, *gn;
-    const double *cmin;
-};
 __global__ void k_fin_ceiling(TrajState *st, const double *__restrict__ part, int nblk, int strict, int fin_copy, ChebFin cheb) {
     const int b = blockIdx.x;
     __shared__ TrajState S;
@@ -1729,21 +1822,8 @@
     int lin_active = S.lin_active;
     if (cheb.enq >= 0 && lin_active) {
         if (S.cheb_n > cheb.enq) return;
-        double rel = 1.0;
-        if (S.cheb_n >= 1) {
-            const double g0 = fin_sum1(cheb.g0, cheb.gnblk, b, 1, 0), gn = fin_sum1(cheb.gn, cheb.gnblk, b, 1, 0);
-            rel = g0 > 0.0 ? sqrt(fmax(gn, 0.0) / g0) : 0.0;
-        }
-        if (threadIdx.x == 0) {
-            rel *= cheb_last_factor(S.cheb_theta, S.cheb_delta, S.cheb_n);
-            S.lin_rel = rel;
-            S.lin_it = S.cheb_n;
-            S.lin_total += S.cheb_n;
-            if (rel * S.lin_rscale > S.lin_maxrel) S.lin_maxrel = rel * S.lin_rscale;
-            S.lin_maxabs = fmax(S.lin_maxabs, rel * S.lin_r0);
-            if (S.cheb_n > S.step_lin_max) S.step_lin_max = S.cheb_n;
-            if (S.step_solves >= 1 && S.step_solves <= 4) S.step_lin[S.step_solves - 1] = S.cheb_n;
-        }
+        const double rel = cheb_solve_rel(S.cheb_n, cheb, b);
+        if (threadIdx.x == 0) cheb_close_books(S, rel);
         lin_active = 0;
     }
     if (fin_copy >= 0 && lin_active) {
@@ -1763,19 +1843,7 @@
     } else {
         fin_reduce(part, nblk, b, v, op, 1);
     }
-    if (threadIdx.x == 0) {
-        double amax = 2.0;
-        if (v[0] < 1e299) amax = fmin(amax, 0.9 * v[0]);
-        if (!isfinite(amax) || amax <= 0.0) amax = 1.0;
-        S.alpha = fmin(1.0, amax);
-        if (lin_active && S.lin_rel > S.lin_maxrel) S.lin_maxrel = S.lin_rel;
-        S.lin_active = 0;
-        S.need_trial = 1;
-        S.trial_no = 0;
-        S.force_accept = 0;
-        S.best_norm = 1e300;
-        S.best_alpha = S.alpha;
-    }
+    if (threadIdx.x == 0) ceiling_arm(S, v[0], lin_active);
     traj_copy_out(st + b, S);
 }
 
```
